# LilYau350/Variance-Aware-Weight

Hardware: AMD Instinct MI355X
Metric: training images/sec (higher is better)
Workload: dtype bf16; 1 GPU; DiT-B/4, 4x32x32 latents, 1000 classes; Trainer.train_step: q_sample + fwd + lambda-weighted MSE + bwd + AdamW + EMA; global batch 256 = 256 per GPU; global_batch=256, per_gpu_batch=256, parallelism=dp1, weight_type=lambda, hip_graph=False

## Files before the change

### include/vaw_hip.h

```cpp
#ifndef VAW_HIP_H
#define VAW_HIP_H
#include <stdint.h>

#ifdef __cplusplus
extern "C" {
#endif

typedef enum { VAW_OK = 0, VAW_ERR_INVALID = -1, VAW_ERR_LAUNCH = -2, VAW_ERR_UNSUPPORTED = -3 } vaw_status;
typedef enum { VAW_F32 = 0, VAW_BF16 = 1,
               VAW_FP8 = 2, VAW_BF8 = 3  } vaw_dtype;
typedef void* vaw_stream;

int vaw_version(void);
const char* vaw_last_error_string(void);


int vaw_qsample_fwd(const float* x0, const float* noise, const int64_t* t, const float* tab_a, const float* tab_s,
                    int num_timesteps, float* x_t, int B, int64_t per_sample, vaw_stream stream);

int vaw_mix_rows(const float* x, const float* y, const float* ca, const float* cb, float* out, int B,
                 int64_t per_sample, vaw_stream stream);

int vaw_wmse_fwd(const float* model_out, const float* x0, const float* noise, const float* ca, const float* cb,
                 const float* w, float* mse, int B, int64_t per_sample, vaw_stream stream);
int vaw_wmse_bwd(const float* model_out, const float* x0, const float* noise, const float* ca, const float* cb,
                 const float* w, const float* gmse, float* dout, int B, int64_t per_sample, vaw_stream stream);

int vaw_vb_fwd(const float* mean_out, const float* var_out, const float* x0, const float* x_t, const float* coef,
               int mean_mode, int var_mode, float scale, float* vb, int B, int64_t per_sample, vaw_stream stream);
int vaw_vb_bwd(const float* mean_out, const float* var_out, const float* x0, const float* x_t, const float* coef,
               int mean_mode, int var_mode, float scale, const float* gvb, float* d_mean, float* d_var, int B,
               int64_t per_sample, vaw_stream stream);

int vaw_sample_step(int kind, const float* mean_out, const float* var_out, const float* x, const float* noise,
                    const float* coef, int mean_mode, int var_mode, int clip_denoised, float eta, float* sample,
                    float* pred_xstart, float* mean, float* log_variance, int B, int64_t per_sample, vaw_stream stream);

int vaw_bpd_terms(const float* mean_out, const float* var_out, int64_t model_ld, const float* x0, const float* x_t,
                  const float* noise, const float* coef, int mean_mode, int var_mode, int clip_denoised, float* vb,
                  float* xstart_mse, float* mse, int64_t out_ld, int group, int B, int64_t per_sample, vaw_stream stream);

int vaw_prior_bpd(const float* x0, float sqrt_abar_last, float log_one_minus_abar_last, float* prior_bpd, int B,
                  int64_t per_sample, vaw_stream stream);

int vaw_ddim_reverse_step(const float* mean_out, int64_t model_ld, const float* x, const float* coef, int clip_denoised,
                          float* sample, float* pred_xstart, int B, int64_t per_sample, vaw_stream stream);

int vaw_guided_sample_step(int kind, const float* mean_cond, const float* mean_uncond, const float* var_cond,
                           const float* var_uncond, int64_t model_ld, float guidance_scale, const float* x, const float* noise,
                           const float* coef, int mean_mode, int var_mode, int clip_denoised, float eta, float* sample,
                           float* pred_xstart, float* mean, float* log_variance, int B, int64_t per_sample, vaw_stream stream);

int vaw_cfg_combine(const float* cond, const float* uncond, int64_t model_ld, float guidance_scale, float* out, int B,
                    int64_t per_sample, vaw_stream stream);

int vaw_finish_images(const void* src, int src_f64, uint8_t* dst, int B, int C, int H, int W, vaw_stream stream);


#define VAW_EDM_COLS 24
#define VAW_FLOW_COLS 16

int vaw_edm_input(const double* x, const double* noise, const double* coef, int row, int rows, double* x_hat, float* model_in,
                  float* model_in_dup, int B, int64_t per_sample, vaw_stream stream);

int vaw_edm_step(int kind, int pred_type, const float* cond, const float* uncond, int64_t model_ld, float guidance_scale,
                 const double* x_hat, double* d_cur, const double* coef, int row, int rows, double* x_out, float* model_in,
                 float* model_in_dup, int B, int64_t per_sample, vaw_stream stream);

int vaw_flow_step(int kind, int sde, int mean_type, const float* cond, const float* uncond, int64_t model_ld,
                  float guidance_scale, const float* x, const float* noise, const float* x_pred, float* f0, float* kick,
                  const float* coef, int row0, int row1, int rows, float* x_out, float* x_out_dup, int B, int64_t per_sample,
                  vaw_stream stream);


#define VAW_RESAMPLER_MAX_T 4096

int vaw_resampler_update(const int64_t* ts, const float* losses, int n, int T, int H, double* ring, int64_t* seen, int* bad,
                         vaw_stream stream);

// ... 82 lines not shown
    VAW_GV_GENERIC = 0,
    VAW_GV_T128_BK32 = 1,
    VAW_GV_T128_BK64 = 2,
    VAW_GV_RING256 = 3,
    VAW_GV_PERSISTENT = 4,
    VAW_GV_SMALL_M = 5,
    VAW_GV_PARKED_DRAIN = 6,
    VAW_GV_WARP_SPEC = 7
} vaw_gemm_variant;
typedef enum { VAW_GR_NONE = 0, VAW_GR_F32 = 1, VAW_GR_BF16 = 2, VAW_GR_F32_ROWSUM = 3 } vaw_gemm_reduce;
typedef enum { VAW_GS_NONE = 0, VAW_GS_FUSED = 1, VAW_GS_SEPARATE = 2 } vaw_gemm_rowsum_mode;
typedef enum { VAW_GC_NONE = 0, VAW_GC_FOLD = 1, VAW_GC_DEFERRED = 2, VAW_GC_SEPARATE = 3 } vaw_gemm_colsum_mode;
typedef struct {
    int variant;
    int ntw;
    int mb, nb, stages;
    int bkt;
    int epi_kind;
    int split;
    int xcd_parts;
    int grid_x, grid_y, grid_z, block;
    int64_t lds_bytes;
    int reduce;
    int rowsum_mode;
    int colsum_mode;
    int64_t colsum_rows;
    int64_t workspace_floats_used;
    int launches;
    int status;
} vaw_gemm_launch;
int vaw_gemm_plan(vaw_dtype dt, int a_kmajor, int b_kmajor, int64_t M, int64_t N, int64_t K, int64_t lda, int64_t ldb,
                  int64_t ldc, int64_t A, int64_t B, int64_t C, const vaw_epilogue* epi_host, int64_t workspace_floats,
                  const vaw_gemm_knobs* knobs, vaw_gemm_launch* out);

int64_t vaw_colsum_workspace_floats(int64_t M, int64_t N);
int vaw_colsum(vaw_dtype dt, const void* X, int64_t M, int64_t N, int64_t ldx, float* out, float beta,
               float* workspace, int64_t workspace_floats, vaw_stream stream);
int vaw_reduce_rows(const float* partial, int64_t R, int64_t N, float* out, float beta, vaw_stream stream);
typedef struct {
    const float* partial;
    float* out;
    int64_t R, N;
} vaw_reduce_job;
int64_t vaw_reduce_rows_batched_desc_bytes(int n_jobs);
int vaw_reduce_rows_batched(int n_jobs, const vaw_reduce_job* jobs, float beta, void* desc_dev, int upload, vaw_stream stream);


int vaw_ln_modulate_fwd(vaw_dtype dt, const float* x, const float* shift, const float* scale, int64_t mod_ld,
                        void* out, float* mean, float* rstd, int B, int T, int D, float eps, vaw_stream stream);
int vaw_ln_modulate_bwd(vaw_dtype dt, const void* dout, const float* x, const float* mean, const float* rstd,
                        const float* scale, int64_t mod_ld, const float* dres_in, float* dx, float* dshift,
                        float* dscale, int64_t dmod_ld, int B, int T, int D, float* workspace, int64_t workspace_floats,
                        vaw_stream stream);
int vaw_ln_modulate_fwd_fp8(const float* x, const float* shift, const float* scale, int64_t mod_ld, void* q_out, float* q_state,
                            vaw_dtype q_format, float* mean, float* rstd, int B, int T, int D, float eps, vaw_stream stream);
int vaw_gate_bwd_fp8(const float* dres, const void* y, const float* gate, int64_t mod_ld, void* dy_q, float* q_state,
                     vaw_dtype q_format, float* dgate, int64_t dmod_ld, float* dy_colsum_partial, int B, int T, int D,
                     float* workspace, int64_t workspace_floats, vaw_stream stream);
int64_t vaw_row_bwd_workspace_floats(int B, int T, int D);
typedef enum { VAW_ROW_LN_FWD = 0, VAW_ROW_LN_FWD_FP8 = 1, VAW_ROW_LN_BWD = 2, VAW_ROW_GATE_BWD = 3, VAW_ROW_GATE_BWD_FP8 = 4,
               VAW_ROW_LN_BWD_GATE = 5, VAW_ROW_LN_BWD_GATE_FP8 = 6, VAW_ROW_COLSUM = 7 } vaw_row_kind;
typedef enum {
    VAW_RV_LN_FWD = 0,
    VAW_RV_ROW_BWD = 1,
    VAW_RV_ROW_GATE = 2,
    VAW_RV_ROW_FUSE = 3,
    VAW_RV_ROW_FUSE8 = 4,
    VAW_RV_COLSUM_BF16X8 = 5, VAW_RV_COLSUM_VEC4 = 6, VAW_RV_COLSUM_SCALAR = 7
} vaw_row_variant;
typedef struct {
    int variant;
    int nv;
    int nc, rows_per_chunk;
    int grid_x, block;
    int64_t lds_bytes;
    int64_t workspace_floats;
} vaw_row_launch;
int vaw_row_plan(vaw_row_kind kind, vaw_dtype dt, int64_t B, int64_t T, int64_t D, int64_t ldx, int64_t base_addr,
                 int64_t workspace_floats, vaw_row_launch* out);
int vaw_gate_bwd(vaw_dtype dt, const float* dres, const void* y, const float* gate, int64_t mod_ld, void* dy,
                 float* dgate, int64_t dmod_ld, float* dy_colsum_partial, int B, int T, int D, float* workspace, int64_t workspace_floats, vaw_stream stream);
int vaw_ln_modulate_bwd_gate(vaw_dtype dt, const void* dout, const float* x, const float* mean, const float* rstd,
                             const float* scale, int64_t mod_ld, const float* dres_in, float* dx, float* dshift, float* dscale,
                             int64_t dmod_ld, const void* y_next, const float* gate_next, void* dy_next, float* dgate_next,
                             float* dy_colsum_partial, int B, int T, int D, float* workspace, int64_t workspace_floats, vaw_stream stream);
int vaw_ln_modulate_bwd_gate_fp8(const void* dout, const float* x, const float* mean, const float* rstd, const float* scale,
                                 int64_t mod_ld, const float* dres_in, float* dx, float* dshift, float* dscale, int64_t dmod_ld,
                                 const void* y_next, const float* gate_next, void* dy_q, float* q_state, vaw_dtype q_format,
                                 float* dgate_next, float* dy_colsum_partial, int B, int T, int D, float* workspace,
                                 int64_t workspace_floats, vaw_stream stream);

int vaw_patchify(vaw_dtype dt, const float* img, void* tok, int B, int C, int H, int W, int p, vaw_stream stream);
int vaw_patchify_bwd(const float* dtok, float* dimg, int B, int C, int H, int W, int p, vaw_stream stream);
int vaw_unpatchify(vaw_dtype dt, const float* tok, float* img, int B, int C, int H, int W, int p,
                   vaw_stream stream);
int vaw_unpatchify_bwd(vaw_dtype dt, const float* dimg, void* dtok, int B, int C, int H, int W, int p,
                       vaw_stream stream);

int vaw_timestep_embedding(vaw_dtype dt, const float* t, void* out, int B, int dim, float max_period,
                           vaw_stream stream);
int vaw_silu_fwd(vaw_dtype dt, const float* x, void* out, int64_t n, vaw_stream stream);
int vaw_silu_bwd(const float* x, const float* dy, float* dx, int64_t n, vaw_stream stream);
int vaw_add_embedding(const float* a, const float* table, const int64_t* idx, float* out, int B, int D,
                      int num_rows, vaw_stream stream);
int vaw_embedding_bwd(const float* dc, const int64_t* idx, float* dtable, int B, int D, int num_rows, float beta,
                      vaw_stream stream);

typedef struct {
    int B, H, T, hd;
    int64_t q_sb, q_sh, q_st, q_sd;
    int64_t o_sb, o_sh, o_st, o_sd;
    float scale;
} vaw_attn_desc;
int vaw_attn_fwd(vaw_dtype dt, const vaw_attn_desc* d_host, const void* q, const void* k, const void* v, void* o,
                 float* lse, vaw_stream stream);
int vaw_attn_bwd(vaw_dtype dt, const vaw_attn_desc* d_host, const void* q, const void* k, const void* v,
                 const void* o, const void* d_o, const float* lse, float* delta, void* dq, void* dk, void* dv,
                 vaw_stream stream);
int vaw_attn_bwd_colsum(vaw_dtype dt, const vaw_attn_desc* d, const void* q, const void* k, const void* v, const void* o,
                        const void* d_o, const float* lse, float* delta, void* dq, void* dk, void* dv, float* colsum_partial,
                        int64_t* rows_out, vaw_stream stream);

typedef enum { VAW_ATTN_DIR_FWD = 0, VAW_ATTN_DIR_BWD = 1, VAW_ATTN_DIR_BWD_COLSUM = 2 } vaw_attn_dir;
typedef enum {
    VAW_AV_ROWWISE = 0,
    VAW_AV_FWD_T64 = 1,
    VAW_AV_FWD_G1 = 2,
    VAW_AV_FWD_G2 = 3,
    VAW_AV_FWD_BIG = 4,
    VAW_AV_BWD_T64 = 5,
    VAW_AV_BWD_G1 = 6,
    VAW_AV_BWD_G2 = 7,
    VAW_AV_BWD_BIG_NT2 = 8,
    VAW_AV_BWD_BIG_NT4 = 9
} vaw_attn_variant;
typedef struct {
    int variant;
    int hd_image;
    int launches;
    int grid_x, grid_y, block;
    int64_t lds_bytes;
    int lds_cap_raised;
    int64_t colsum_rows;
    int status;
} vaw_attn_launch;
int vaw_attn_plan(int dir, vaw_dtype dt, const vaw_attn_desc* d, int64_t q, int64_t k, int64_t v, int64_t o_or_do, int64_t dq,
                  int64_t dk, int64_t dv, vaw_attn_launch* out);


int vaw_conv3x3_narrow(vaw_dtype dt, int mode, const void* in, const void* w, const float* bias, void* out, int B, int H,
                       int W, int Cn, int Cw, vaw_stream stream);

int64_t vaw_groupnorm_workspace_floats(int B, int HW, int C);
int vaw_groupnorm_fwd(vaw_dtype dt, const void* x, const float* gamma, const float* beta, const float* scale,
                      const float* shift, int64_t film_ld, int silu, void* y, float* mean, float* rstd, int B, int HW,
                      int C, int G, float eps, float* workspace, vaw_stream stream);
int vaw_groupnorm_apply(vaw_dtype dt, const void* x, const float* mean, const float* rstd, const float* gamma,
                        const float* beta, const float* scale, const float* shift, int64_t film_ld, int silu, void* y, int B,
                        int HW, int C, int G, vaw_stream stream);
int vaw_groupnorm_bwd(vaw_dtype dt, const void* dout, const void* x, const float* mean, const float* rstd,
                      const float* gamma, const float* beta, const float* scale, const float* shift, int64_t film_ld,
                      int silu, const void* dx_add, void* dx, float* dgamma, float* dbeta, float grad_beta, float* dscale,
                      float* dshift, int64_t dfilm_ld, int B, int HW, int C, int G, float* workspace, vaw_stream stream);
int vaw_im2col3x3(vaw_dtype dt, const void* x, void* col, int B, int H, int W, int C, vaw_stream stream);
int vaw_col2im3x3(vaw_dtype dt, const void* dcol, void* dx, int B, int H, int W, int C, vaw_stream stream);
int vaw_conv3x3(vaw_dtype dt, int mode, const void* act, const void* act2, const void* w, void* out, int B, int H, int W,
                int Ci, int Co, const vaw_epilogue* epi_host, float* workspace, int64_t workspace_floats, vaw_stream stream);
int64_t vaw_conv3x3_wgrad_small_workspace_floats(int B, int H, int W, int Ci, int Co);
int vaw_conv3x3_wgrad_small(vaw_dtype dt, const void* dy, const void* x, float* dw, float beta, int B, int H, int W, int Ci,
                            int Co, float* workspace, int64_t workspace_floats, vaw_stream stream);
int vaw_resample2(vaw_dtype dt, const void* in, void* out, int B, int Ho, int Wo, int C, int mode, float s,
                  vaw_stream stream);
int vaw_concat_channels(vaw_dtype dt, void* a, void* b, void* cat, int64_t M, int Ca, int Cb, int split,
                        vaw_stream stream);
int vaw_add_inplace(vaw_dtype dt, void* dst, const void* src, int64_t n, vaw_stream stream);
int vaw_mul(vaw_dtype dt, const void* a, const void* b, void* out, int64_t n, vaw_stream stream);
int vaw_subsample2(vaw_dtype dt, const void* in, void* out, int B, int Ho, int Wo, int C, int mode, vaw_stream stream);
int64_t vaw_dropout_bits_words(int64_t n);
int vaw_dropout_pack(vaw_dtype dt, const void* mask, void* bits, int64_t M, int C, vaw_stream stream);
int vaw_dropout_bits_fwd(vaw_dtype dt, const void* x, const void* bits, float keep_scale, void* y, int64_t n, vaw_stream stream);
int vaw_dropout_bits_bwd(vaw_dtype dt, const void* dy, const void* bits, float keep_scale, void* dx, int64_t n, vaw_stream stream);
int vaw_rowvec_add(vaw_dtype dt, void* h, const float* e, int64_t ld, int B, int HW, int C, vaw_stream stream);
int vaw_rowvec_sum(vaw_dtype dt, const void* dh, float* de, int64_t ld, int B, int HW, int C, float beta, vaw_stream stream);
int vaw_nchw_to_nhwc(vaw_dtype dt, const float* nchw, void* nhwc, int B, int C, int HW, vaw_stream stream);
int vaw_nhwc_to_nchw(vaw_dtype dt, const void* nhwc, float* nchw, int B, int C, int HW, vaw_stream stream);


int64_t vaw_sumsq_workspace_floats(void);
int vaw_sumsq(const float* g, int64_t n, float* sumsq_out, int accumulate, float* workspace, vaw_stream stream);
int vaw_adamw_ema_step(float* p, float* g, float* m, float* v, float* ema, void* shadow_bf16, int64_t n, float lr,
                       float beta1, float beta2, float eps, float weight_decay, float bc1, float bc2,
                       float ema_decay, const float* sumsq, float clip_max_norm, int zero_grad, vaw_stream stream);
int vaw_adamw_ema_step_dev(float* p, float* g, float* m, float* v, float* ema, void* shadow_bf16, int64_t n,
                           const float* hyper, float beta1, float beta2, float eps, float weight_decay, float ema_decay,
                           const float* sumsq, float clip_max_norm, int zero_grad, vaw_stream stream);
int vaw_ema_update(float* ema, const float* src, int64_t n, float decay, vaw_stream stream);
int vaw_cast_bf16(const float* src, void* dst, int64_t n, vaw_stream stream);
int vaw_uncast_bf16(const void* src, float* dst, int64_t n, float scale, vaw_stream stream);

typedef struct {
    int records;
    int colsum_sets;
    int own_dy;
    int Bk;
    int64_t block_bytes;
    int64_t block_stat_bytes;
    int64_t shared_bytes;
    int64_t colsum_bytes;
    int64_t scratch_bytes;
    int64_t cond_bytes;
    int64_t total;
} vaw_dit_ws_plan_t;
int vaw_dit_ws_plan(int dtype, int B, int T, int D, int Dm, int depth, int heads, int Kp, int No, int defer_wgrad, int checkpoint,
                    vaw_dit_ws_plan_t* out);

int vaw_comm_unique_id(void* out128);
int vaw_comm_init(const void* id128, int rank, int world);
int vaw_comm_world(void);
int vaw_comm_destroy(void);
int vaw_allreduce_bucket_start(void* buf, int64_t count, vaw_dtype dt, vaw_stream stream);
int vaw_reduce_scatter_bucket_start(void* buf, int64_t count, vaw_dtype dt, vaw_stream stream);
int vaw_allgather_bucket_start(void* buf, int64_t count, vaw_dtype dt, vaw_stream stream);
int vaw_allreduce_bucket_wait(vaw_stream stream);

#ifdef __cplusplus
}
#endif
#endif
```

### variance-aware-weight_amd/_lib.py

```python
import ctypes as C
import os

import torch

_HERE = os.path.dirname(os.path.abspath(__file__))
LIB_PATH = os.environ.get("VAW_HIP_LIB") or os.path.join(_HERE, "libvaw_hip.so")

F32, BF16, FP8, BF8 = 0, 1, 2, 3
TORCH_DTYPE = {F32: torch.float32, BF16: torch.bfloat16}

_p, _i, _l, _f = C.c_void_p, C.c_int, C.c_int64, C.c_float


class Epilogue(C.Structure):
    _fields_ = [("bias", _p), ("act", _i), ("aux_in", _p), ("aux_out", _p), ("gate", _p), ("gate_ld", _l),
                ("resid", _p), ("rowadd", _p), ("rows_per_batch", _i), ("alpha", _f), ("beta", _f), ("out_f32", _i),
                ("colsum_out", _p), ("colsum_beta", _f), ("resid_is_act", _i), ("rowsum_a_out", _p), ("rowsum_a_beta", _f),
                ("colsum_partial_out", _p), ("colsum_rows_out", C.POINTER(C.c_int64))]


class AttnDesc(C.Structure):
    _fields_ = [("B", _i), ("H", _i), ("T", _i), ("hd", _i), ("q_sb", _l), ("q_sh", _l), ("q_st", _l), ("q_sd", _l),
                ("o_sb", _l), ("o_sh", _l), ("o_st", _l), ("o_sd", _l), ("scale", _f)]


class RowLaunch(C.Structure):
    _fields_ = [("variant", _i), ("nv", _i), ("nc", _i), ("rows_per_chunk", _i), ("grid_x", _i), ("block", _i), ("lds_bytes", _l),
                ("workspace_floats", _l)]


class AttnLaunch(C.Structure):
    _fields_ = [("variant", _i), ("hd_image", _i), ("launches", _i), ("grid_x", _i), ("grid_y", _i), ("block", _i), ("lds_bytes", _l),
                ("lds_cap_raised", _i), ("colsum_rows", _l), ("status", _i)]


class GemmKnobs(C.Structure):
    _fields_ = [(n, _i) for n in ("tile", "force_generic", "bk", "pd", "ws", "xcdsplit", "sm_max_m", "sm_wide_m", "sm_nb", "sm_stages",
                                  "ws_loaders", "epi", "debug", "p8_nt", "nt_aux", "cus")]


class GemmLaunch(C.Structure):
    _fields_ = [("variant", _i), ("ntw", _i), ("mb", _i), ("nb", _i), ("stages", _i), ("bkt", _i), ("epi_kind", _i), ("split", _i),
                ("xcd_parts", _i), ("grid_x", _i), ("grid_y", _i), ("grid_z", _i), ("block", _i), ("lds_bytes", _l), ("reduce", _i),
                ("rowsum_mode", _i), ("colsum_mode", _i), ("colsum_rows", _l), ("workspace_floats_used", _l), ("launches", _i),
                ("status", _i)]


class DitWsPlan(C.Structure):
    _fields_ = [("records", _i), ("colsum_sets", _i), ("own_dy", _i), ("Bk", _i), ("block_bytes", _l), ("block_stat_bytes", _l),
                ("shared_bytes", _l), ("colsum_bytes", _l), ("scratch_bytes", _l), ("cond_bytes", _l), ("total", _l)]


ATTN_FWD, ATTN_BWD, ATTN_BWD_COLSUM = range(3)
(AV_ROWWISE, AV_FWD_T64, AV_FWD_G1, AV_FWD_G2, AV_FWD_BIG, AV_BWD_T64, AV_BWD_G1, AV_BWD_G2, AV_BWD_BIG_NT2,
 AV_BWD_BIG_NT4) = range(10)
AV_NAMES = ("rowwise", "fwd_t64", "fwd_g1", "fwd_g2", "fwd_big", "bwd_t64", "bwd_g1", "bwd_g2", "bwd_big_nt2", "bwd_big_nt4")

GV_GENERIC, GV_T128_BK32, GV_T128_BK64, GV_RING256, GV_PERSISTENT, GV_SMALL_M, GV_PARKED_DRAIN, GV_WARP_SPEC = range(8)
GV_NAMES = ("generic", "t128_bk32", "t128_bk64", "ring256", "persistent", "small_m", "parked_drain", "warp_spec")
GR_NONE, GR_F32, GR_BF16, GR_F32_ROWSUM = range(4)
GS_NONE, GS_FUSED, GS_SEPARATE = range(3)
GC_NONE, GC_FOLD, GC_DEFERRED, GC_SEPARATE = range(4)
P8_STORE, P8_GELU, P8_DGELU, P8_GATE, P8_SLAB, P8_ANY, P8_WGRAD, P8_RESID = range(8)

RESAMPLER_MAX_T = 4096

ROW_LN_FWD, ROW_LN_FWD_FP8, ROW_LN_BWD, ROW_GATE_BWD, ROW_GATE_BWD_FP8, ROW_LN_BWD_GATE, ROW_LN_BWD_GATE_FP8, ROW_COLSUM = range(8)
RV_LN_FWD, RV_ROW_BWD, RV_ROW_GATE, RV_ROW_FUSE, RV_ROW_FUSE8, RV_COLSUM_BF16X8, RV_COLSUM_VEC4, RV_COLSUM_SCALAR = range(8)

_PROTOS = {
    "vaw_qsample_fwd": [_p, _p, _p, _p, _p, _i, _p, _i, _l, _p],
    "vaw_mix_rows": [_p, _p, _p, _p, _p, _i, _l, _p],
    "vaw_wmse_fwd": [_p, _p, _p, _p, _p, _p, _p, _i, _l, _p],
    "vaw_wmse_bwd": [_p, _p, _p, _p, _p, _p, _p, _p, _i, _l, _p],
    "vaw_gemm": [_i, _i, _i, _l, _l, _l, _p, _l, _p, _l, _p, _l, C.POINTER(Epilogue), _p, _l, _p],
    "vaw_gemm_uses_bf16_mfma": [_i, _l, _l, _l, _p, _l, _p, _l],
    "vaw_colsum": [_i, _p, _l, _l, _l, _p, _f, _p, _l, _p],
    "vaw_ln_modulate_fwd": [_i, _p, _p, _p, _l, _p, _p, _p, _i, _i, _i, _f, _p],
    "vaw_ln_modulate_bwd": [_i, _p, _p, _p, _p, _p, _l, _p, _p, _p, _p, _l, _i, _i, _i, _p, _l, _p],
    "vaw_gate_bwd": [_i, _p, _p, _p, _l, _p, _p, _l, _p, _i, _i, _i, _p, _l, _p],
    "vaw_reduce_rows": [_p, _l, _l, _p, _f, _p],
    "vaw_reduce_rows_batched": [_i, _p, _f, _p, _i, _p],
    "vaw_ln_modulate_bwd_gate": [_i, _p, _p, _p, _p, _p, _l, _p, _p, _p, _p, _l, _p, _p, _p, _p, _p, _i, _i, _i, _p, _l, _p],
    "vaw_ln_modulate_bwd_gate_fp8": [_p, _p, _p, _p, _p, _l, _p, _p, _p, _p, _l, _p, _p, _p, _p, _i, _p, _p, _i, _i, _i, _p, _l, _p],
    "vaw_patchify": [_i, _p, _p, _i, _i, _i, _i, _i, _p],
    "vaw_patchify_bwd": [_p, _p, _i, _i, _i, _i, _i, _p],
    "vaw_unpatchify": [_i, _p, _p, _i, _i, _i, _i, _i, _p],
    "vaw_unpatchify_bwd": [_i, _p, _p, _i, _i, _i, _i, _i, _p],
    "vaw_timestep_embedding": [_i, _p, _p, _i, _i, _f, _p],
    "vaw_silu_fwd": [_i, _p, _p, _l, _p],
    "vaw_silu_bwd": [_p, _p, _p, _l, _p],
    "vaw_add_embedding": [_p, _p, _p, _p, _i, _i, _i, _p],
    "vaw_embedding_bwd": [_p, _p, _p, _i, _i, _i, _f, _p],
    "vaw_attn_fwd": [_i, C.POINTER(AttnDesc), _p, _p, _p, _p, _p, _p],
    "vaw_attn_bwd": [_i, C.POINTER(AttnDesc), _p, _p, _p, _p, _p, _p, _p, _p, _p, _p, _p],
    "vaw_attn_bwd_colsum": [_i, C.POINTER(AttnDesc), _p, _p, _p, _p, _p, _p, _p, _p, _p, _p, _p, C.POINTER(C.c_int64), _p],
    "vaw_comm_unique_id": [_p],
    "vaw_comm_init": [_p, _i, _i],
    "vaw_comm_world": [],
    "vaw_comm_destroy": [],
    "vaw_allreduce_bucket_start": [_p, _l, _i, _p],
    "vaw_reduce_scatter_bucket_start": [_p, _l, _i, _p],
    "vaw_allgather_bucket_start": [_p, _l, _i, _p],
# ... 1 lines not shown
    "vaw_groupnorm_fwd": [_i, _p, _p, _p, _p, _p, _l, _i, _p, _p, _p, _i, _i, _i, _i, _f, _p, _p],
    "vaw_groupnorm_apply": [_i, _p, _p, _p, _p, _p, _p, _p, _l, _i, _p, _i, _i, _i, _i, _p],
    "vaw_groupnorm_bwd": [_i, _p, _p, _p, _p, _p, _p, _p, _p, _l, _i, _p, _p, _p, _p, _f, _p, _p, _l, _i, _i, _i, _i, _p, _p],
    "vaw_im2col3x3": [_i, _p, _p, _i, _i, _i, _i, _p],
    "vaw_col2im3x3": [_i, _p, _p, _i, _i, _i, _i, _p],
    "vaw_conv3x3": [_i, _i, _p, _p, _p, _p, _i, _i, _i, _i, _i, C.POINTER(Epilogue), _p, _l, _p],
    "vaw_vb_fwd": [_p, _p, _p, _p, _p, _i, _i, _f, _p, _i, _l, _p],
    "vaw_vb_bwd": [_p, _p, _p, _p, _p, _i, _i, _f, _p, _p, _p, _i, _l, _p],
    "vaw_sample_step": [_i, _p, _p, _p, _p, _p, _i, _i, _i, _f, _p, _p, _p, _p, _i, _l, _p],
    "vaw_bpd_terms": [_p, _p, _l, _p, _p, _p, _p, _i, _i, _i, _p, _p, _p, _l, _i, _i, _l, _p],
    "vaw_guided_sample_step": [_i, _p, _p, _p, _p, _l, _f, _p, _p, _p, _i, _i, _i, _f, _p, _p, _p, _p, _i, _l, _p],
    "vaw_cfg_combine": [_p, _p, _l, _f, _p, _i, _l, _p],
    "vaw_finish_images": [_p, _i, _p, _i, _i, _i, _i, _p],
    "vaw_edm_input": [_p, _p, _p, _i, _i, _p, _p, _p, _i, _l, _p],
    "vaw_edm_step": [_i, _i, _p, _p, _l, _f, _p, _p, _p, _i, _i, _p, _p, _p, _i, _l, _p],
    "vaw_flow_step": [_i, _i, _i, _p, _p, _l, _f, _p, _p, _p, _p, _p, _p, _i, _i, _i, _p, _p, _i, _l, _p],
    "vaw_prior_bpd": [_p, _f, _f, _p, _i, _l, _p],
    "vaw_ddim_reverse_step": [_p, _l, _p, _p, _i, _p, _p, _i, _l, _p],
    "vaw_resampler_update": [_p, _p, _i, _i, _i, _p, _p, _p, _p],
    "vaw_resampler_draw": [_p, _p, _i, _i, C.c_double, _p, _i, _p, _p, _p, _p],
    "vaw_conv3x3_narrow": [_i, _i, _p, _p, _p, _p, _i, _i, _i, _i, _i, _p],
    "vaw_conv3x3_wgrad_small": [_i, _p, _p, _p, _f, _i, _i, _i, _i, _i, _p, _l, _p],
    "vaw_resample2": [_i, _p, _p, _i, _i, _i, _i, _i, _f, _p],
    "vaw_concat_channels": [_i, _p, _p, _p, _l, _i, _i, _i, _p],
    "vaw_add_inplace": [_i, _p, _p, _l, _p],
    "vaw_mul": [_i, _p, _p, _p, _l, _p],
    "vaw_subsample2": [_i, _p, _p, _i, _i, _i, _i, _i, _p],
    "vaw_dropout_pack": [_i, _p, _p, _l, _i, _p],
    "vaw_dropout_bits_fwd": [_i, _p, _p, _f, _p, _l, _p],
    "vaw_dropout_bits_bwd": [_i, _p, _p, _f, _p, _l, _p],
    "vaw_rowvec_add": [_i, _p, _p, _l, _i, _i, _i, _p],
    "vaw_rowvec_sum": [_i, _p, _p, _l, _i, _i, _i, _f, _p],
    "vaw_nchw_to_nhwc": [_i, _p, _p, _i, _i, _i, _p],
    "vaw_nhwc_to_nchw": [_i, _p, _p, _i, _i, _i, _p],
    "vaw_sumsq": [_p, _l, _p, _i, _p, _p],
    "vaw_adamw_ema_step_dev": [_p, _p, _p, _p, _p, _p, _l, _p, _f, _f, _f, _f, _f, _p, _f, _i, _p],
    "vaw_adamw_ema_step": [_p, _p, _p, _p, _p, _p, _l, _f, _f, _f, _f, _f, _f, _f, _f, _p, _f, _i, _p],
    "vaw_ema_update": [_p, _p, _l, _f, _p],
    "vaw_cast_bf16": [_p, _p, _l, _p],
    "vaw_uncast_bf16": [_p, _p, _l, _f, _p],
    "vaw_wgrad_grouped": [_i, _i, _p, _l, _f, _p, _i, _p, _l, _p],
    "vaw_fp8_quantize": [_i, _i, _p, _l, _l, _l, _p, _l, _p, _l, _p, _p, _l, _p],
    "vaw_fp8_quantize_delayed": [_i, _i, _p, _l, _l, _l, _p, _l, _p, _l, _p, _p],
    "vaw_fp8_scale_update": [_p, _l, _p],
    "vaw_fp8_quantize_delayed_batched": [_i, _p, _p, _i, _p],
    "vaw_gemm_fp8": [_i, _l, _l, _l, _p, _l, _p, _p, _l, _p, _p, _l, C.POINTER(Epilogue), _p, _i, _p, _l, _p],
    "vaw_fp8_transpose": [_p, _l, _l, _l, _p, _l, _p],
    "vaw_ln_modulate_fwd_fp8": [_p, _p, _p, _l, _p, _p, _i, _p, _p, _i, _i, _i, _f, _p],
    "vaw_gate_bwd_fp8": [_p, _p, _p, _l, _p, _p, _i, _p, _l, _p, _i, _i, _i, _p, _l, _p],
    "vaw_row_plan": [_i, _i, _l, _l, _l, _l, _l, _l, C.POINTER(RowLaunch)],
    "vaw_attn_plan": [_i, _i, C.POINTER(AttnDesc), _l, _l, _l, _l, _l, _l, _l, C.POINTER(AttnLaunch)],
    "vaw_gemm_plan": [_i, _i, _i, _l, _l, _l, _l, _l, _l, _l, _l, _l, C.POINTER(Epilogue), _l, C.POINTER(GemmKnobs), C.POINTER(GemmLaunch)],
    "vaw_dit_ws_plan": [_i, _i, _i, _i, _i, _i, _i, _i, _i, _i, _i, C.POINTER(DitWsPlan)],
}

_lib = None


class VawError(RuntimeError):
    pass


def lib():
    global _lib
    if _lib is None:
        if not os.path.exists(LIB_PATH):
            raise VawError(f"{LIB_PATH} not found: build it with `python -c 'import __graft_entry__ as g; g.build()'` "
                           "(there is no CPU fallback for the HIP path)")
        L = C.CDLL(LIB_PATH)
        for name, args in _PROTOS.items():
            if not hasattr(L, name) and os.environ.get("VAW_HIP_LIB"):
                continue
            fn = getattr(L, name)
            fn.argtypes = args
            fn.restype = _i
        L.vaw_version.restype = _i
        L.vaw_last_error_string.restype = C.c_char_p
        L.vaw_colsum_workspace_floats.argtypes = [_l, _l]
        L.vaw_colsum_workspace_floats.restype = _l
        L.vaw_row_bwd_workspace_floats.argtypes = [_i, _i, _i]
        L.vaw_row_bwd_workspace_floats.restype = _l
        L.vaw_conv3x3_wgrad_small_workspace_floats.argtypes = [_i, _i, _i, _i, _i]
        L.vaw_conv3x3_wgrad_small_workspace_floats.restype = _l
        L.vaw_groupnorm_workspace_floats.argtypes = [_i, _i, _i]
        L.vaw_groupnorm_workspace_floats.restype = _l
        if hasattr(L, "vaw_dropout_bits_words"):
            L.vaw_dropout_bits_words.argtypes = [_l]
            L.vaw_dropout_bits_words.restype = _l
        L.vaw_wgrad_grouped_desc_bytes.argtypes = [_i]
        L.vaw_wgrad_grouped_desc_bytes.restype = _l
        L.vaw_reduce_rows_batched_desc_bytes.argtypes = [_i]
        L.vaw_reduce_rows_batched_desc_bytes.restype = _l
        L.vaw_fp8_quantize_batched_desc_bytes.argtypes = [_i]
        L.vaw_fp8_quantize_batched_desc_bytes.restype = _l
        L.vaw_fp8_quantize_workspace_floats.argtypes = []
        L.vaw_fp8_quantize_workspace_floats.restype = _l
        L.vaw_sumsq_workspace_floats.argtypes = []
        L.vaw_sumsq_workspace_floats.restype = _l
        L.vaw_debug_force_rowwise_attention.argtypes = [_i]
        L.vaw_debug_force_rowwise_attention.restype = None
        L.vaw_debug_force_generic_gemm.argtypes = [_i]
        L.vaw_debug_force_generic_gemm.restype = None
        L.vaw_debug_gemm_tile.argtypes = [_i]
        L.vaw_debug_gemm_tile.restype = None
        if hasattr(L, "vaw_gemm_default_knobs"):
            L.vaw_gemm_default_knobs.argtypes = [C.POINTER(GemmKnobs)]
            L.vaw_gemm_default_knobs.restype = None
        for dbg in ("vaw_debug_gn_coop", "vaw_debug_gn_flat"):
            if hasattr(L, dbg):
                getattr(L, dbg).argtypes = [_i]
                getattr(L, dbg).restype = None
        L.vaw_p8_set_reserved_cus.argtypes = [_i]
        L.vaw_p8_set_reserved_cus.restype = None
        L.vaw_debug_cu_hog.argtypes = [_i, _i, _p]
        L.vaw_debug_cu_hog.restype = _i
        _lib = L
    return _lib


def exported_symbols():
    return sorted(list(_PROTOS) + ["vaw_version", "vaw_last_error_string", "vaw_colsum_workspace_floats",
                                   "vaw_sumsq_workspace_floats", "vaw_groupnorm_workspace_floats", "vaw_wgrad_grouped_desc_bytes",
                                   "vaw_conv3x3_wgrad_small_workspace_floats", "vaw_row_bwd_workspace_floats",
                                   "vaw_fp8_quantize_workspace_floats", "vaw_p8_set_reserved_cus", "vaw_reduce_rows_batched_desc_bytes", "vaw_fp8_quantize_batched_desc_bytes",
                                   "vaw_gemm_default_knobs", "vaw_dropout_bits_words"])


def check(rc, what):
    if rc != 0:
        raise VawError(f"{what} failed ({rc}): {lib().vaw_last_error_string().decode()}")


def stream_ptr():
    return torch.cuda.current_stream().cuda_stream


def ptr(t):
    return 0 if t is None else t.data_ptr()


def need_cuda(*tensors):
    for t in tensors:
        if t is not None and not t.is_cuda:
            raise VawError("vaw_amd runs on the GPU only: got a CPU tensor (no CPU fallback exists by design)")
```

### variance-aware-weight_amd/csrc/elementwise.hip

```cpp
#include "common.h"

static inline int stream_grid(int64_t work_items, int block) {
    int64_t g = (work_items + block - 1) / block;
    const int64_t cap = 256 * 8;
    return (int)(g < 1 ? 1 : (g > cap ? cap : g));
}

template <bool GATHER>
__global__ void mix_rows_kernel(const float* __restrict__ x, const float* __restrict__ y, const float* __restrict__ ca,
                                const float* __restrict__ cb, const int64_t* __restrict__ t, int T,
                                float* __restrict__ out, int64_t n) {
    const int b = blockIdx.y;
    float a, c;
    if (GATHER) {
        const int64_t tt = t[b];
        const bool ok = tt >= 0 && tt < T;
        a = ok ? ca[tt] : __builtin_nanf("");
        c = ok ? cb[tt] : __builtin_nanf("");
    } else {
        a = ca[b];
        c = cb[b];
    }
    const float* xr = x + (int64_t)b * n;
    const float* yr = y + (int64_t)b * n;
    float* orow = out + (int64_t)b * n;
    const int64_t n4 = ((n & 3) == 0) ? n / 4 : 0;
    for (int64_t i = blockIdx.x * (int64_t)blockDim.x + threadIdx.x; i < n4; i += (int64_t)gridDim.x * blockDim.x) {
        f32x4 xv = load4(xr + 4 * i), yv = load4(yr + 4 * i);
        store4(orow + 4 * i, a * xv + c * yv);
    }
    for (int64_t i = n4 * 4 + blockIdx.x * (int64_t)blockDim.x + threadIdx.x; i < n; i += (int64_t)gridDim.x * blockDim.x)
        orow[i] = a * xr[i] + c * yr[i];
}

extern "C" int vaw_qsample_fwd(const float* x0, const float* noise, const int64_t* t, const float* tab_a,
                               const float* tab_s, int num_timesteps, float* x_t, int B, int64_t per_sample,
                               vaw_stream stream) {
    VAW_CHECK_ARG(B > 0 && per_sample > 0 && num_timesteps > 0, "qsample: bad sizes B=%d n=%ld", B, (long)per_sample);
    int gx = stream_grid(per_sample / 4 + 1, 256);
    dim3 grid(gx > 64 ? 64 : gx, B);
    mix_rows_kernel<true><<<grid, 256, 0, (hipStream_t)stream>>>(x0, noise, tab_a, tab_s, t, num_timesteps, x_t, per_sample);
    VAW_CHECK_LAUNCH("qsample");
    return VAW_OK;
}

extern "C" int vaw_mix_rows(const float* x, const float* y, const float* ca, const float* cb, float* out, int B,
                            int64_t per_sample, vaw_stream stream) {
    VAW_CHECK_ARG(B > 0 && per_sample > 0, "mix_rows: bad sizes");
    int gx = stream_grid(per_sample / 4 + 1, 256);
    dim3 grid(gx > 64 ? 64 : gx, B);
    mix_rows_kernel<false><<<grid, 256, 0, (hipStream_t)stream>>>(x, y, ca, cb, nullptr, 0, out, per_sample);
    VAW_CHECK_LAUNCH("mix_rows");
    return VAW_OK;
}

__global__ void wmse_fwd_kernel(const float* __restrict__ o, const float* __restrict__ x0, const float* __restrict__ nz,
                                const float* __restrict__ ca, const float* __restrict__ cb, const float* __restrict__ w,
                                float* __restrict__ mse, int64_t n) {
    __shared__ float scratch[16];
    const int b = blockIdx.x;
    const float a = ca[b], c = cb[b];
    const float* orow = o + (int64_t)b * n;
    const float* xr = x0 + (int64_t)b * n;
    const float* nr = nz + (int64_t)b * n;
    float acc = 0.f;
    const int64_t n4 = ((n & 3) == 0) ? n / 4 : 0;
    for (int64_t i = threadIdx.x; i < n4; i += blockDim.x) {
        f32x4 d = a * load4(xr + 4 * i) + c * load4(nr + 4 * i) - load4(orow + 4 * i);
        acc += d[0] * d[0] + d[1] * d[1] + d[2] * d[2] + d[3] * d[3];
    }
    for (int64_t i = n4 * 4 + threadIdx.x; i < n; i += blockDim.x) {
        float d = a * xr[i] + c * nr[i] - orow[i];
        acc += d * d;
    }
    float tot = block_sum(acc, scratch);
    if (threadIdx.x == 0) mse[b] = w[b] * (tot / (float)n);
}

__global__ void wmse_bwd_kernel(const float* __restrict__ o, const float* __restrict__ x0, const float* __restrict__ nz,
                                const float* __restrict__ ca, const float* __restrict__ cb, const float* __restrict__ w,
                                const float* __restrict__ gmse, float* __restrict__ dout, int64_t n) {
    const int b = blockIdx.y;
    const float a = ca[b], c = cb[b];
    const float k = gmse[b] * w[b] * 2.f / (float)n;
    const float* orow = o + (int64_t)b * n;
    const float* xr = x0 + (int64_t)b * n;
    const float* nr = nz + (int64_t)b * n;
    float* dr = dout + (int64_t)b * n;
    const int64_t n4 = ((n & 3) == 0) ? n / 4 : 0;
    for (int64_t i = blockIdx.x * (int64_t)blockDim.x + threadIdx.x; i < n4; i += (int64_t)gridDim.x * blockDim.x)
        store4(dr + 4 * i, k * (load4(orow + 4 * i) - a * load4(xr + 4 * i) - c * load4(nr + 4 * i)));
    for (int64_t i = n4 * 4 + blockIdx.x * (int64_t)blockDim.x + threadIdx.x; i < n; i += (int64_t)gridDim.x * blockDim.x)
        dr[i] = k * (orow[i] - a * xr[i] - c * nr[i]);
}

extern "C" int vaw_wmse_fwd(const float* model_out, const float* x0, const float* noise, const float* ca,
                            const float* cb, const float* w, float* mse, int B, int64_t per_sample,
                            vaw_stream stream) {
    VAW_CHECK_ARG(B > 0 && per_sample > 0, "wmse_fwd: bad sizes");
    wmse_fwd_kernel<<<B, 1024, 0, (hipStream_t)stream>>>(model_out, x0, noise, ca, cb, w, mse, per_sample);
    VAW_CHECK_LAUNCH("wmse_fwd");
    return VAW_OK;
}

extern "C" int vaw_wmse_bwd(const float* model_out, const float* x0, const float* noise, const float* ca,
                            const float* cb, const float* w, const float* gmse, float* dout, int B,
                            int64_t per_sample, vaw_stream stream) {
    VAW_CHECK_ARG(B > 0 && per_sample > 0, "wmse_bwd: bad sizes");
    int gx = stream_grid(per_sample / 4 + 1, 256);
    dim3 grid(gx > 64 ? 64 : gx, B);
    wmse_bwd_kernel<<<grid, 256, 0, (hipStream_t)stream>>>(model_out, x0, noise, ca, cb, w, gmse, dout, per_sample);
    VAW_CHECK_LAUNCH("wmse_bwd");
    return VAW_OK;
}

#define VB_NCOEF 8
struct VbElem {
    float val;
    float d_lv;
    float d_mean;
};
__device__ __forceinline__ float vb_cdf(float z, float& dcdf) {
    const float k = 0.7978845608028654f;
    const float th = tanhf(k * (z + 0.044715f * (z * z * z)));
    dcdf = 0.5f * (1.f - th * th) * k * (1.f + 3.f * 0.044715f * z * z);
    return 0.5f * (1.f + th);
}
__device__ __forceinline__ VbElem vb_elem(float x0, float true_mean, float true_lv, float mean, float lv, bool t0) {
    VbElem r;
    if (!t0) {
        const float e2 = expf(-lv), d = true_mean - mean, ratio = expf(true_lv - lv);
        r.val = 0.5f * (-1.0f + lv - true_lv + ratio + (d * d) * e2);
        r.d_lv = 0.5f * (1.f - ratio - (d * d) * e2);
        r.d_mean = -d * e2;
        return r;
    }
    const float cx = x0 - mean, inv = expf(-(0.5f * lv));
    const float pin = inv * (cx + 1.0f / 255.0f), mnn = inv * (cx - 1.0f / 255.0f);
    float dp, dm;
    const float cp = vb_cdf(pin, dp), cm = vb_cdf(mnn, dm);
    float lp, g_pin = 0.f, g_min = 0.f;
    if (x0 < -0.999f) {
        lp = logf(fmaxf(cp, 1e-12f));
        if (cp >= 1e-12f) g_pin = dp / cp;
    } else if (x0 > 0.999f) {
        const float q = 1.f - cm;
        lp = logf(fmaxf(q, 1e-12f));
        if (q >= 1e-12f) g_min = -dm / q;
    } else {
        const float dl = cp - cm;
        lp = logf(fmaxf(dl, 1e-12f));
        if (dl >= 1e-12f) { g_pin = dp / dl; g_min = -dm / dl; }
    }
    r.val = -lp;
    r.d_lv = 0.5f * (g_pin * pin + g_min * mnn);
    r.d_mean = inv * (g_pin + g_min);
    return r;
}
__device__ __forceinline__ void vb_model(const float* c, int mean_mode, int var_mode, float xt, float m, float v, float& mean,
                                         float& lv) {
    mean = mean_mode == 1 ? m : c[0] * (c[4] * xt + c[5] * m) + c[1] * xt;
    if (var_mode == 1) lv = v;
    else if (var_mode == 2) { const float frac = (v + 1.f) / 2.f; lv = frac * c[3] + (1.f - frac) * c[2]; }
    else lv = c[3];
// ... 511 lines not shown

extern "C" int vaw_finish_images(const void* src, int src_f64, uint8_t* dst, int B, int C, int H, int W, vaw_stream stream) {
    VAW_CHECK_ARG(B > 0 && C > 0 && H > 0 && W > 0, "finish_images: bad sizes B=%d C=%d H=%d W=%d", B, C, H, W);
    VAW_CHECK_ARG(src && dst, "finish_images: null pointer");
    VAW_CHECK_ARG(src_f64 == 0 || src_f64 == 1, "finish_images: src_f64 must be 0 (f32) or 1 (f64), got %d", src_f64);
    VAW_CHECK_ARG(((uintptr_t)src & (src_f64 ? 7 : 3)) == 0, "finish_images: source not aligned to its element size");
    const int64_t HW = (int64_t)H * W;
    if (src_f64) finish_images_launch(static_cast<const double*>(src), dst, B, C, HW, (hipStream_t)stream);
    else finish_images_launch(static_cast<const float*>(src), dst, B, C, HW, (hipStream_t)stream);
    VAW_CHECK_LAUNCH("finish_images");
    return VAW_OK;
}

template <typename T>
__global__ void timestep_embedding_kernel(const float* __restrict__ t, T* __restrict__ out, int B, int dim,
                                          float neg_log_period) {
    const int half = dim / 2;
    for (int64_t idx = blockIdx.x * (int64_t)blockDim.x + threadIdx.x; idx < (int64_t)B * dim;
         idx += (int64_t)gridDim.x * blockDim.x) {
        const int b = (int)(idx / dim), j = (int)(idx % dim);
        float v = 0.f;
        if (j < 2 * half) {
            const int i = j < half ? j : j - half;
            const float f = expf(neg_log_period * (float)i / (float)half);
            const float ang = t[b] * f;
            v = j < half ? cosf(ang) : sinf(ang);
        }
        out[idx] = from_f32<T>(v);
    }
}

extern "C" int vaw_timestep_embedding(vaw_dtype dt, const float* t, void* out, int B, int dim, float max_period,
                                      vaw_stream stream) {
    VAW_CHECK_ARG(B > 0 && dim > 0, "timestep_embedding: bad sizes");
    const float nl = -logf(max_period);
    int grid = stream_grid((int64_t)B * dim, 256);
    if (dt == VAW_F32)
        timestep_embedding_kernel<float><<<grid, 256, 0, (hipStream_t)stream>>>(t, (float*)out, B, dim, nl);
    else
        timestep_embedding_kernel<bf16_t><<<grid, 256, 0, (hipStream_t)stream>>>(t, (bf16_t*)out, B, dim, nl);
    VAW_CHECK_LAUNCH("timestep_embedding");
    return VAW_OK;
}

template <typename T>
__global__ void silu_fwd_kernel(const float* __restrict__ x, T* __restrict__ out, int64_t n) {
    for (int64_t i = blockIdx.x * (int64_t)blockDim.x + threadIdx.x; i < n; i += (int64_t)gridDim.x * blockDim.x)
        out[i] = from_f32<T>(silu_f(x[i]));
}
__global__ void silu_bwd_kernel(const float* __restrict__ x, const float* __restrict__ dy, float* __restrict__ dx, int64_t n) {
    for (int64_t i = blockIdx.x * (int64_t)blockDim.x + threadIdx.x; i < n; i += (int64_t)gridDim.x * blockDim.x)
        dx[i] = dy[i] * silu_grad_f(x[i]);
}
extern "C" int vaw_silu_fwd(vaw_dtype dt, const float* x, void* out, int64_t n, vaw_stream stream) {
    VAW_CHECK_ARG(n > 0, "silu_fwd: n<=0");
    int grid = stream_grid(n, 256);
    if (dt == VAW_F32) silu_fwd_kernel<float><<<grid, 256, 0, (hipStream_t)stream>>>(x, (float*)out, n);
    else silu_fwd_kernel<bf16_t><<<grid, 256, 0, (hipStream_t)stream>>>(x, (bf16_t*)out, n);
    VAW_CHECK_LAUNCH("silu_fwd");
    return VAW_OK;
}
extern "C" int vaw_silu_bwd(const float* x, const float* dy, float* dx, int64_t n, vaw_stream stream) {
    VAW_CHECK_ARG(n > 0, "silu_bwd: n<=0");
    silu_bwd_kernel<<<stream_grid(n, 256), 256, 0, (hipStream_t)stream>>>(x, dy, dx, n);
    VAW_CHECK_LAUNCH("silu_bwd");
    return VAW_OK;
}

__global__ void add_embedding_kernel(const float* __restrict__ a, const float* __restrict__ table,
                                     const int64_t* __restrict__ idx, float* __restrict__ out, int B, int D, int rows) {
    for (int64_t i = blockIdx.x * (int64_t)blockDim.x + threadIdx.x; i < (int64_t)B * D; i += (int64_t)gridDim.x * blockDim.x) {
        const int b = (int)(i / D), d = (int)(i % D);
        const int64_t r = idx[b];
        out[i] = a[i] + ((r >= 0 && r < rows) ? table[r * D + d] : __builtin_nanf(""));
    }
}
__global__ void __launch_bounds__(256)
embedding_bwd_kernel(const float* __restrict__ dc, const int64_t* __restrict__ idx, float* __restrict__ dtable, int B, int D,
                     int rows, float beta) {
    __shared__ int s_idx[1024];
    const int r = blockIdx.x;
    constexpr int MAXC = 8;
    for (int d0 = 0; d0 < D; d0 += 256 * MAXC) {
        float acc[MAXC];
#pragma unroll
        for (int j = 0; j < MAXC; ++j) acc[j] = 0.f;
        for (int b0 = 0; b0 < B; b0 += 1024) {
            const int nb = B - b0 < 1024 ? B - b0 : 1024;
            __syncthreads();
            for (int i = threadIdx.x; i < nb; i += 256) s_idx[i] = (int)idx[b0 + i];
            __syncthreads();
            for (int i = 0; i < nb; ++i) {
                if (s_idx[i] != r) continue;
                const float* src = dc + (int64_t)(b0 + i) * D + d0;
#pragma unroll
                for (int j = 0; j < MAXC; ++j) {
                    const int d = threadIdx.x + 256 * j;
                    if (d0 + d < D) acc[j] += src[d];
                }
            }
        }
#pragma unroll
        for (int j = 0; j < MAXC; ++j) {
            const int d = d0 + threadIdx.x + 256 * j;
            if (d < D) {
                float* o = dtable + (int64_t)r * D + d;
                *o = (beta != 0.f ? beta * *o : 0.f) + acc[j];
            }
        }
    }
}
extern "C" int vaw_add_embedding(const float* a, const float* table, const int64_t* idx, float* out, int B, int D,
                                 int num_rows, vaw_stream stream) {
    VAW_CHECK_ARG(B > 0 && D > 0 && num_rows > 0, "add_embedding: bad sizes");
    add_embedding_kernel<<<stream_grid((int64_t)B * D, 256), 256, 0, (hipStream_t)stream>>>(a, table, idx, out, B, D, num_rows);
    VAW_CHECK_LAUNCH("add_embedding");
    return VAW_OK;
}
extern "C" int vaw_embedding_bwd(const float* dc, const int64_t* idx, float* dtable, int B, int D, int num_rows,
                                 float beta, vaw_stream stream) {
    VAW_CHECK_ARG(B > 0 && D > 0 && num_rows > 0, "embedding_bwd: bad sizes");
    embedding_bwd_kernel<<<num_rows, 256, 0, (hipStream_t)stream>>>(dc, idx, dtable, B, D, num_rows, beta);
    VAW_CHECK_LAUNCH("embedding_bwd");
    return VAW_OK;
}

template <typename T, bool CONV_ORDER, bool TO_TOKENS>
__global__ void patch_shuffle_kernel(const float* __restrict__ img_in, float* __restrict__ img_out,
                                     const float* __restrict__ tok_in_f32, T* __restrict__ tok_out, int B, int C, int H,
                                     int W, int p) {
    const int hp = H / p, wp = W / p;
    const int64_t total = (int64_t)B * C * H * W;
    const int K = C * p * p;
    for (int64_t e = blockIdx.x * (int64_t)blockDim.x + threadIdx.x; e < total; e += (int64_t)gridDim.x * blockDim.x) {
        int x = (int)(e % W);
        int64_t r = e / W;
        int y = (int)(r % H);
        r /= H;
        int c = (int)(r % C);
        int b = (int)(r / C);
        const int ty = y / p, i = y % p, tx = x / p, j = x % p;
        const int64_t row = ((int64_t)b * hp + ty) * wp + tx;
        const int col = CONV_ORDER ? (c * p + i) * p + j : (i * p + j) * C + c;
        if (TO_TOKENS) tok_out[row * K + col] = from_f32<T>(img_in[e]);
        else img_out[e] = tok_in_f32[row * K + col];
    }
}

extern "C" int vaw_patchify(vaw_dtype dt, const float* img, void* tok, int B, int C, int H, int W, int p,
                            vaw_stream stream) {
    VAW_CHECK_ARG(B > 0 && C > 0 && p > 0 && H % p == 0 && W % p == 0, "patchify: bad sizes");
    int grid = stream_grid((int64_t)B * C * H * W, 256);
    if (dt == VAW_F32)
        patch_shuffle_kernel<float, true, true><<<grid, 256, 0, (hipStream_t)stream>>>(img, nullptr, nullptr, (float*)tok, B, C, H, W, p);
    else
        patch_shuffle_kernel<bf16_t, true, true><<<grid, 256, 0, (hipStream_t)stream>>>(img, nullptr, nullptr, (bf16_t*)tok, B, C, H, W, p);
    VAW_CHECK_LAUNCH("patchify");
    return VAW_OK;
}
extern "C" int vaw_patchify_bwd(const float* dtok, float* dimg, int B, int C, int H, int W, int p, vaw_stream stream) {
    VAW_CHECK_ARG(B > 0 && C > 0 && p > 0 && H % p == 0 && W % p == 0, "patchify_bwd: bad sizes");
    int grid = stream_grid((int64_t)B * C * H * W, 256);
    patch_shuffle_kernel<float, true, false><<<grid, 256, 0, (hipStream_t)stream>>>(nullptr, dimg, dtok, nullptr, B, C, H, W, p);
    VAW_CHECK_LAUNCH("patchify_bwd");
// ... 165 lines not shown
                                      vaw_stream stream) {
    VAW_CHECK_ARG(n > 0 && hyper, "adamw_dev: n<=0 or no hyper buffer");
    VAW_CHECK_ARG((((uintptr_t)p | (uintptr_t)g | (uintptr_t)m | (uintptr_t)v | (uintptr_t)ema) & 15) == 0 &&
                      ((uintptr_t)shadow_bf16 & 7) == 0, "adamw_dev: buffers must be 16-byte aligned");
    VAW_CHECK_ARG(clip_max_norm <= 0.f || sumsq != nullptr, "adamw_dev: clip needs sumsq");
    AdamArgs a{0.f, beta1, beta2, eps, weight_decay, 1.f, 1.f, ema_decay, clip_max_norm, zero_grad};
    adamw_ema_kernel<<<adam_grid(n), 256, 0, (hipStream_t)stream>>>(p, g, m, v, ema, (bf16_t*)shadow_bf16, n, sumsq, a, hyper);
    VAW_CHECK_LAUNCH("adamw_ema_dev");
    return VAW_OK;
}

__global__ void ema_kernel(float* __restrict__ ema, const float* __restrict__ src, int64_t n, float d) {
    for (int64_t i = blockIdx.x * (int64_t)blockDim.x + threadIdx.x; i < n; i += (int64_t)gridDim.x * blockDim.x)
        ema[i] = ema[i] * d + src[i] * (1.f - d);
}
extern "C" int vaw_ema_update(float* ema, const float* src, int64_t n, float decay, vaw_stream stream) {
    VAW_CHECK_ARG(n > 0, "ema: n<=0");
    ema_kernel<<<stream_grid(n, 256), 256, 0, (hipStream_t)stream>>>(ema, src, n, decay);
    VAW_CHECK_LAUNCH("ema");
    return VAW_OK;
}

__global__ void cast_bf16_kernel(const float* __restrict__ src, bf16_t* __restrict__ dst, int64_t n) {
    const int64_t n4 = n / 4;
    for (int64_t i = blockIdx.x * (int64_t)blockDim.x + threadIdx.x; i < n4; i += (int64_t)gridDim.x * blockDim.x)
        store4(dst + 4 * i, load4(src + 4 * i));
    for (int64_t i = n4 * 4 + blockIdx.x * (int64_t)blockDim.x + threadIdx.x; i < n; i += (int64_t)gridDim.x * blockDim.x)
        dst[i] = (bf16_t)src[i];
}
extern "C" int vaw_cast_bf16(const float* src, void* dst, int64_t n, vaw_stream stream) {
    VAW_CHECK_ARG(n > 0 && ((uintptr_t)src & 15) == 0 && ((uintptr_t)dst & 7) == 0, "cast_bf16: n<=0 or unaligned");
    cast_bf16_kernel<<<stream_grid(n / 4 + 1, 256), 256, 0, (hipStream_t)stream>>>(src, (bf16_t*)dst, n);
    VAW_CHECK_LAUNCH("cast_bf16");
    return VAW_OK;
}

__global__ void uncast_bf16_kernel(const bf16_t* __restrict__ src, float* __restrict__ dst, int64_t n, float scale) {
    const int64_t n8 = n / 8;
    for (int64_t i = blockIdx.x * (int64_t)blockDim.x + threadIdx.x; i < n8; i += (int64_t)gridDim.x * blockDim.x) {
        const bf16x8 v = reinterpret_cast<const bf16x8*>(src)[i];
        f32x4 a = {(float)v[0], (float)v[1], (float)v[2], (float)v[3]}, b = {(float)v[4], (float)v[5], (float)v[6], (float)v[7]};
        reinterpret_cast<f32x4*>(dst)[2 * i] = a * scale;
        reinterpret_cast<f32x4*>(dst)[2 * i + 1] = b * scale;
    }
    for (int64_t i = n8 * 8 + blockIdx.x * (int64_t)blockDim.x + threadIdx.x; i < n; i += (int64_t)gridDim.x * blockDim.x)
        dst[i] = scale * (float)src[i];
}
extern "C" int vaw_uncast_bf16(const void* src, float* dst, int64_t n, float scale, vaw_stream stream) {
    VAW_CHECK_ARG(n > 0 && ((uintptr_t)src & 15) == 0 && ((uintptr_t)dst & 15) == 0, "uncast_bf16: n<=0 or unaligned");
    uncast_bf16_kernel<<<stream_grid(n / 8 + 1, 256), 256, 0, (hipStream_t)stream>>>((const bf16_t*)src, dst, n, scale);
    VAW_CHECK_LAUNCH("uncast_bf16");
    return VAW_OK;
}
```

### variance-aware-weight_amd/csrc/gemm.hip

```cpp
#include "common.h"
#include <type_traits>

#include "gemm_plan.h"

#define BM 128
#define BN 128
#define BK 64
#define CS_LD 132
#define CS_BYTES (64 * CS_LD * 4)
#define CP_BYTES (4 * 128 * 4)

template <int BKT> struct FastCfg {
    static constexpr int tile_bytes = 128 * BKT * 2;
    static constexpr int stage_bytes = 2 * tile_bytes;
    static constexpr int main_bytes = 2 * stage_bytes;
    static constexpr int lds_bytes = (main_bytes > CS_BYTES ? main_bytes : CS_BYTES) + CP_BYTES;
};

typedef __attribute__((address_space(3))) void* lds_ptr_t;
typedef const __attribute__((address_space(1))) void* gbl_ptr_t;

template <int BKT>
__device__ __forceinline__ int kmaj_swz(int row) { return BKT == 64 ? ((row >> 1) & 7) : ((-(row >> 2)) & 3); }
template <int BKT>
// ... 443 lines not shown
            for (int i = 0; i < 4; ++i)
#pragma unroll
                for (int j = 0; j < 4; ++j)
#pragma unroll
                    for (int r = 0; r < 4; ++r)
                        cs[(16 * i + 4 * (lane >> 4) + r) * BIG_CS_LD + 64 * wx + 16 * j + (lane & 15)] =
                            acc[4 * (quarter & 1) + i][j][r];
        }
        __syncthreads();
#pragma unroll
        for (int pass = 0; pass < 4; ++pass) {
            const int row = pass * 16 + r0;
            if (!col_ok || 64 * quarter + row >= mvalid) continue;
            const float* src = cs + row * BIG_CS_LD + c8;
            const int64_t m = m0 + 64 * quarter + row;
            if (n_split > 1) {
                float* dst = e.slab + (int64_t)blockIdx.y * e.M * e.N + m * e.N + n0 + c8;
                store4(dst, load4(src));
                store4(dst + 4, load4(src + 4));
            } else {
                f32x4 v0 = load4(src), v1 = load4(src + 4);
                epi_row8(e, (unsigned)m, n0 + c8, v0, v1, b0, b1);
                s0 += v0;
                s1 += v1;
            }
        }
    }
    if (e.colpart && n_split == 1) {
#pragma unroll
        for (int j = 0; j < 4; ++j) {
            s0[j] += __shfl_xor(s0[j], 32, 64);
            s1[j] += __shfl_xor(s1[j], 32, 64);
        }
        float* cp = reinterpret_cast<float*>(smem + BIG_NSTAGE * BIG_STAGE);
        if (lane < 32) {
            store4(cp + wid * 256 + c8, s0);
            store4(cp + wid * 256 + c8 + 4, s1);
        }
        __syncthreads();
        if ((int)threadIdx.x < nvalid && threadIdx.x < 256) {
            float t = 0.f;
#pragma unroll
            for (int w8 = 0; w8 < 8; ++w8) t += cp[w8 * 256 + threadIdx.x];
            e.colpart[(int64_t)tm * e.N + n0 + threadIdx.x] = t;
        }
    }
}

template <typename TO>
__global__ void splitk_reduce_kernel(const float* __restrict__ slab, int S, int64_t M, int64_t N, int64_t ldc,
                                     void* __restrict__ C, float alpha, float beta, int out_f32,
                                     const float* __restrict__ rowpart = nullptr, float* __restrict__ rowsum_out = nullptr,
                                     float rowsum_beta = 0.f) {
    if (rowpart && blockIdx.x == gridDim.x - 1) {
        for (int64_t m = threadIdx.x; m < M; m += blockDim.x) {
            float t = 0.f;
            for (int sidx = 0; sidx < S; ++sidx) t += rowpart[(int64_t)sidx * M + m];
            rowsum_out[m] = (rowsum_beta != 0.f ? rowsum_beta * rowsum_out[m] : 0.f) + t;
        }
    }
    const int64_t total4 = M * N / 4;
    for (int64_t i = blockIdx.x * (int64_t)blockDim.x + threadIdx.x; i < total4; i += (int64_t)gridDim.x * blockDim.x) {
        const int64_t m = (4 * i) / N, n = (4 * i) % N;
        f32x4 acc = {0, 0, 0, 0};
        int sidx = 0;
        for (; sidx + 8 <= S; sidx += 8) {
            f32x4 v[8];
#pragma unroll
            for (int u = 0; u < 8; ++u) v[u] = load4(slab + (int64_t)(sidx + u) * M * N + 4 * i);
#pragma unroll
            for (int u = 0; u < 8; ++u) acc += v[u];
        }
        for (; sidx < S; ++sidx) acc += load4(slab + (int64_t)sidx * M * N + 4 * i);
        acc *= alpha;
        const int64_t off = m * ldc + n;
        if (out_f32) {
            float* c = (float*)C + off;
            if (beta != 0.f) acc += beta * load4(c);
            store4(c, acc);
        } else {
            store4((TO*)C + off, acc);
        }
    }
}

#define GBM 128
#define GBN 128
#define GBK 16
#define GLD 144

template <typename T, bool KMAJOR>
__device__ __forceinline__ void generic_stage(const T* __restrict__ g, int64_t ld, int64_t r0, int64_t rows, int64_t k0,
                                              int64_t K, float* tile, int tid) {
#pragma unroll
    for (int i = 0; i < (GBM * GBK) / 256; ++i) {
        const int e = tid + 256 * i;
        int r, k;
        if (KMAJOR) { r = e / GBK; k = e % GBK; } else { k = e / GBM; r = e % GBM; }
        const int64_t gr = r0 + r, gk = k0 + k;
        float v = 0.f;
        if (gr < rows && gk < K) v = to_f32(KMAJOR ? g[gr * ld + gk] : g[gk * ld + gr]);
        tile[k * GLD + r] = v;
    }
}

template <typename T, bool AK, bool BKM>
__global__ void __launch_bounds__(256)
gemm_generic_kernel(const T* __restrict__ A, int64_t lda, const T* __restrict__ B, int64_t ldb, int64_t K, int64_t kchunk,
                    EpiDev e) {
    __shared__ float As[GBK * GLD];
// ... 261 lines not shown
```

### variance-aware-weight_amd/csrc/layernorm.hip

```cpp
#include <stdio.h>
#include <stdlib.h>

#include "common.h"

template <typename T, int NV>
__global__ void __launch_bounds__(256)
ln_modulate_fwd_kernel(const float* __restrict__ x, const float* __restrict__ shift, const float* __restrict__ scale,
                       int64_t mod_ld, T* __restrict__ out, float* __restrict__ mean_out, float* __restrict__ rstd_out,
                       int64_t M, int Tt, int D, float eps, unsigned char* __restrict__ q_out = nullptr,
                       float* __restrict__ q_state = nullptr, int q_e5m2 = 0) {
    const int lane = threadIdx.x & 63;
    const float q_inv = q_out ? 1.f / q_state[0] : 1.f;
    float am = 0.f;
    const int wave = __builtin_amdgcn_readfirstlane(threadIdx.x >> 6);
    const int64_t row0 = (int64_t)blockIdx.x * 4 + wave, rstep = (int64_t)gridDim.x * 4;
    unsigned colc[NV];
#pragma unroll
    for (int i = 0; i < NV; ++i) {
        const unsigned c = (unsigned)(i * 64 + lane) * 4u;
        colc[i] = c < (unsigned)D ? c : 0u;
    }
    f32x4 nx[NV];
    if (row0 < M) {
#pragma unroll
// ... 19 lines not shown
        for (int i = 0; i < NV; ++i) {
            const int c = (i * 64 + lane) * 4;
            if (c < D) {
                f32x4 d = v[i] - mean;
                q += d[0] * d[0] + d[1] * d[1] + d[2] * d[2] + d[3] * d[3];
            }
        }
        const float rstd = rsqrtf(wave_sum(q) / (float)D + eps);
        if (lane == 0) {
            mean_out[row] = mean;
            rstd_out[row] = rstd;
        }
        const float* sh = shift + (int64_t)b * mod_ld;
        const float* sc = scale + (int64_t)b * mod_ld;
        if (q_out) {
#pragma unroll
            for (int i = 0; i < NV; ++i) {
                const int c = (i * 64 + lane) * 4;
                if (c < D) {
                    f32x4 xh = (v[i] - mean) * rstd;
                    *reinterpret_cast<unsigned*>(q_out + row * D + c) = fp8_word_of_bf16(xh * (1.f + load4(sc + c)) + load4(sh + c), q_inv, q_e5m2, am);
                }
            }
            continue;
        }
        T* orow = out + row * D;
#pragma unroll
        for (int i = 0; i < NV; ++i) {
            const int c = (i * 64 + lane) * 4;
            if (c < D) {
                f32x4 xh = (v[i] - mean) * rstd;
                store4(orow + c, xh * (1.f + load4(sc + c)) + load4(sh + c));
            }
        }
    }
    if (q_out) {
        __shared__ float wmax[4];
        am = wave_max(am);
        if (lane == 0) wmax[threadIdx.x >> 6] = am;
        __syncthreads();
        if (threadIdx.x < 64) fp8_amax_commit(fmaxf(fmaxf(wmax[0], wmax[1]), fmaxf(wmax[2], wmax[3])), q_state + 1, lane);
    }
}

template <typename T, int NV, bool GATE_ONLY, bool QOUT = false, bool FUSE = false>
__global__ void __launch_bounds__((FUSE && NV > 3) ? 512 : 1024)
row_bwd_kernel(const T* __restrict__ dout, const float* __restrict__ x, const float* __restrict__ mean,
               const float* __restrict__ rstd, const float* __restrict__ scale, int64_t mod_ld,
               const float* __restrict__ dres_in, float* __restrict__ dx, float* __restrict__ dshift,
               float* __restrict__ dscale, int64_t dmod_ld, int Tt, int D,
               const float* __restrict__ dres, const T* __restrict__ y, const float* __restrict__ gate,
               T* __restrict__ dy, float* __restrict__ dgate, float* __restrict__ dy_colpart,
               int rows_per_chunk, float* __restrict__ part,
               unsigned char* __restrict__ q_out = nullptr, float* __restrict__ q_state = nullptr, int q_e5m2 = 0) {
    static_assert(!(FUSE && GATE_ONLY), "FUSE extends the LayerNorm mode");
    constexpr int NQ = FUSE ? 4 : 2;
    extern __shared__ __attribute__((aligned(16))) float lds[];
    const float q_inv = ((GATE_ONLY || FUSE) && QOUT) ? 1.f / q_state[0] : 1.f;
    float q_am = 0.f;
    const int lane = threadIdx.x & 63, wid = threadIdx.x >> 6, nw = blockDim.x >> 6;
    const int b = blockIdx.x;
    const int t_begin = blockIdx.y * rows_per_chunk;
    const int t_end = t_begin + rows_per_chunk < Tt ? t_begin + rows_per_chunk : Tt;
    f32x4 acc0[NV], acc1[NV], sc[NV];
    f32x4 acc2[FUSE ? NV : 1], acc3[FUSE ? NV : 1];
    float* const sc_lds = lds + NQ * D;
    float* const gsc_lds = sc_lds + D;
#pragma unroll
    for (int i = 0; i < NV; ++i) {
        acc0[i] = f32x4{0, 0, 0, 0};
        acc1[i] = f32x4{0, 0, 0, 0};
        const int c = (i * 64 + lane) * 4;
        const float* src = GATE_ONLY ? gate : scale;
        sc[i] = c < D ? load4(src + (int64_t)b * mod_ld + c) : f32x4{0, 0, 0, 0};
        if (FUSE) {
            acc2[i] = acc3[i] = f32x4{0, 0, 0, 0};
            if (wid == 0 && c < D) {
                store4(sc_lds + c, 1.f + sc[i]);
                store4(gsc_lds + c, load4(gate + (int64_t)b * mod_ld + c));
            }
        }
    }
    if (FUSE) __syncthreads();
    for (int t = t_begin + wid; t < t_end; t += nw) {
        const int64_t row = (int64_t)b * Tt + t;
        if (GATE_ONLY) {
#pragma unroll
            for (int i = 0; i < NV; ++i) {
                const int c = (i * 64 + lane) * 4;
                if (c < D) {
                    f32x4 g = load4(dres + row * D + c);
                    f32x4 yv = load4(y + row * D + c);
                    f32x4 d = g * sc[i];
                    if (QOUT) *reinterpret_cast<unsigned*>(q_out + row * D + c) = fp8_word_of_bf16(d, q_inv, q_e5m2, q_am);
                    else store4(dy + row * D + c, d);
                    acc0[i] += g * yv;
                    f32x4 dr = {to_f32(from_f32<T>(d[0])), to_f32(from_f32<T>(d[1])), to_f32(from_f32<T>(d[2])), to_f32(from_f32<T>(d[3]))};
                    acc1[i] += dr;
                }
            }
        } else {
            const float mu = mean[row], rs = rstd[row];
            f32x4 g[NV], xh[NV];
            float s1 = 0.f, s2 = 0.f;
#pragma unroll
            for (int i = 0; i < NV; ++i) {
                const int c = (i * 64 + lane) * 4;
                if (c < D) {
                    f32x4 d = load4(dout + row * D + c);
                    xh[i] = (load4(x + row * D + c) - mu) * rs;
                    acc0[i] += d;
                    acc1[i] += d * xh[i];
                    g[i] = d * (FUSE ? load4(sc_lds + c) : 1.f + sc[i]);
                    s1 += g[i][0] + g[i][1] + g[i][2] + g[i][3];
                    f32x4 gx = g[i] * xh[i];
                    s2 += gx[0] + gx[1] + gx[2] + gx[3];
                } else {
                    g[i] = xh[i] = f32x4{0, 0, 0, 0};
                }
            }
            const float c1 = wave_sum(s1) / (float)D, c2 = wave_sum(s2) / (float)D;
#pragma unroll
            for (int i = 0; i < NV; ++i) {
                const int c = (i * 64 + lane) * 4;
                if (c < D) {
                    f32x4 r = (g[i] - c1 - xh[i] * c2) * rs;
                    if (dres_in) r += load4(dres_in + row * D + c);
                    store4(dx + row * D + c, r);
                    if (FUSE) {
                        const f32x4 yv = load4(y + row * D + c);
                        const f32x4 d = r * load4(gsc_lds + c);
                        if (QOUT) *reinterpret_cast<unsigned*>(q_out + row * D + c) = fp8_word_of_bf16(d, q_inv, q_e5m2, q_am);
                        else store4(dy + row * D + c, d);
                        acc2[i] += r * yv;
                        f32x4 dr = {to_f32(from_f32<T>(d[0])), to_f32(from_f32<T>(d[1])), to_f32(from_f32<T>(d[2])), to_f32(from_f32<T>(d[3]))};
                        acc3[i] += dr;
                    }
                }
            }
        }
    }
    if ((GATE_ONLY || FUSE) && QOUT) fp8_amax_commit(q_am, q_state + 1, lane);
    float* s0 = lds;
    float* s1p = lds + D;
    for (int i = threadIdx.x; i < NQ * D; i += blockDim.x) lds[i] = 0.f;
    __syncthreads();
    for (int w = 0; w < nw; ++w) {
        if (wid == w) {
#pragma unroll
            for (int i = 0; i < NV; ++i) {
                const int c = (i * 64 + lane) * 4;
                if (c < D) {
                    store4(s0 + c, load4(s0 + c) + acc0[i]);
                    store4(s1p + c, load4(s1p + c) + acc1[i]);
                    if (FUSE) {
                        store4(lds + 2 * D + c, load4(lds + 2 * D + c) + acc2[i]);
                        store4(lds + 3 * D + c, load4(lds + 3 * D + c) + acc3[i]);
                    }
                }
            }
        }
        __syncthreads();
    }
    if (part) {
        float* dst = part + ((int64_t)blockIdx.y * gridDim.x + b) * NQ * D;
        for (int c = threadIdx.x; c < NQ * D; c += blockDim.x) dst[c] = lds[c];
        return;
    }
    for (int c = threadIdx.x; c < D; c += blockDim.x) {
        if (GATE_ONLY) {
            dgate[(int64_t)b * dmod_ld + c] = s0[c];
            if (dy_colpart) dy_colpart[(int64_t)b * D + c] = s1p[c];
        } else {
            dshift[(int64_t)b * dmod_ld + c] = s0[c];
            dscale[(int64_t)b * dmod_ld + c] = s1p[c];
            if (FUSE) {
                dgate[(int64_t)b * dmod_ld + c] = lds[2 * D + c];
                if (dy_colpart) dy_colpart[(int64_t)b * D + c] = lds[3 * D + c];
            }
        }
    }
// ... 249 lines not shown
        case 6: { constexpr int NV = 6; CALL; } break;              \
        default: { constexpr int NV = 8; CALL; } break;             \
    }

#define ROW_PLAN(kind, dt, B, T, D, ldx, base, wsf)                                      \
    vaw_row_launch plan;                                                               \
    {                                                                                  \
        const int rc_ = vaw_row_plan(kind, dt, B, T, D, ldx, base, wsf, &plan);        \
        if (rc_ != VAW_OK) return rc_;                                                 \
    }

extern "C" int vaw_ln_modulate_fwd(vaw_dtype dt, const float* x, const float* shift, const float* scale, int64_t mod_ld,
                                   void* out, float* mean, float* rstd, int B, int T, int D, float eps,
                                   vaw_stream stream) {
    VAW_CHECK_ARG(B > 0 && T > 0 && D > 0 && D % 4 == 0 && D <= 2048 && mod_ld % 4 == 0,
                  "ln_modulate_fwd: need D%%4==0, D<=2048, mod_ld%%4==0 (D=%d)", D);
    ROW_PLAN(VAW_ROW_LN_FWD, dt, B, T, D, 0, 0, 0);
    const int64_t M = (int64_t)B * T;
    static int per_cu[2][9] = {};
    const int nvk = plan.nv, ti = dt == VAW_F32 ? 0 : 1;
    if (!per_cu[ti][nvk]) {
        int nb = 0;
        if (dt == VAW_F32) { DISPATCH_NV(nvk, (void)hipOccupancyMaxActiveBlocksPerMultiprocessor(&nb, ln_modulate_fwd_kernel<float, NV>, 256, 0)); }
        else { DISPATCH_NV(nvk, (void)hipOccupancyMaxActiveBlocksPerMultiprocessor(&nb, ln_modulate_fwd_kernel<bf16_t, NV>, 256, 0)); }
        per_cu[ti][nvk] = nb > 0 && nb <= 8 ? nb : 8;
    }
    const int64_t cap = 256LL * per_cu[ti][nvk];
    const int grid = (int)(plan.grid_x < cap ? plan.grid_x : cap);
    hipStream_t s = (hipStream_t)stream;
    if (dt == VAW_F32) {
        DISPATCH_NV(nvk, (ln_modulate_fwd_kernel<float, NV><<<grid, plan.block, 0, s>>>(x, shift, scale, mod_ld, (float*)out, mean, rstd, M, T, D, eps)));
    } else {
        DISPATCH_NV(nvk, (ln_modulate_fwd_kernel<bf16_t, NV><<<grid, plan.block, 0, s>>>(x, shift, scale, mod_ld, (bf16_t*)out, mean, rstd, M, T, D, eps)));
    }
    VAW_CHECK_LAUNCH("ln_modulate_fwd");
    return VAW_OK;
}

extern "C" int vaw_ln_modulate_fwd_fp8(const float* x, const float* shift, const float* scale, int64_t mod_ld, void* q_out,
                                       float* q_state, vaw_dtype q_format, float* mean, float* rstd, int B, int T, int D, float eps,
                                       vaw_stream stream) {
    VAW_CHECK_ARG(B > 0 && T > 0 && D > 0 && D % 4 == 0 && D <= 2048 && mod_ld % 4 == 0 && q_out && q_state,
                  "ln_modulate_fwd_fp8: need D%%4==0, D<=2048, mod_ld%%4==0 (D=%d)", D);
    VAW_CHECK_ARG(q_format == VAW_FP8 || q_format == VAW_BF8, "ln_modulate_fwd_fp8: q_format");
    ROW_PLAN(VAW_ROW_LN_FWD_FP8, VAW_BF16, B, T, D, 0, 0, 0);
    const int64_t M = (int64_t)B * T;
    hipStream_t s = (hipStream_t)stream;
    DISPATCH_NV(plan.nv, (ln_modulate_fwd_kernel<bf16_t, NV><<<plan.grid_x, plan.block, 0, s>>>(x, shift, scale, mod_ld, nullptr, mean, rstd, M, T, D, eps,
                                                                                             (unsigned char*)q_out, q_state, q_format == VAW_BF8)));
    VAW_CHECK_LAUNCH("ln_modulate_fwd_fp8");
    return VAW_OK;
}

extern "C" int vaw_ln_modulate_bwd(vaw_dtype dt, const void* dout, const float* x, const float* mean, const float* rstd,
                                   const float* scale, int64_t mod_ld, const float* dres_in, float* dx, float* dshift,
                                   float* dscale, int64_t dmod_ld, int B, int T, int D, float* workspace,
                                   int64_t workspace_floats, vaw_stream stream) {
    VAW_CHECK_ARG(B > 0 && T > 0 && D > 0 && D % 4 == 0 && D <= 2048 && mod_ld % 4 == 0,
                  "ln_modulate_bwd: need D%%4==0, D<=2048, mod_ld%%4==0 (D=%d)", D);
    ROW_PLAN(VAW_ROW_LN_BWD, dt, B, T, D, 0, 0, workspace ? workspace_floats : 0);
    hipStream_t s = (hipStream_t)stream;
    const int nc = plan.nc, rpc = plan.rows_per_chunk, block = plan.block;
    float* part = nc > 1 ? workspace : nullptr;
    const size_t lds = plan.lds_bytes;
    dim3 grid(B, nc);
    if (dt == VAW_F32) {
        DISPATCH_NV(plan.nv, (row_bwd_kernel<float, NV, false><<<grid, block, lds, s>>>((const float*)dout, x, mean, rstd, scale, mod_ld, dres_in, dx, dshift, dscale, dmod_ld, T, D, nullptr, nullptr, nullptr, nullptr, nullptr, nullptr, rpc, part)));
    } else {
        DISPATCH_NV(plan.nv, (row_bwd_kernel<bf16_t, NV, false><<<grid, block, lds, s>>>((const bf16_t*)dout, x, mean, rstd, scale, mod_ld, dres_in, dx, dshift, dscale, dmod_ld, T, D, nullptr, nullptr, nullptr, nullptr, nullptr, nullptr, rpc, part)));
    }
    if (nc > 1) row_bwd_finish_kernel<<<ceil_div((int64_t)B * D, 256), 256, 0, s>>>(part, nc, B, D, dshift, dmod_ld, dscale, dmod_ld);
    VAW_CHECK_LAUNCH("ln_modulate_bwd");
    return VAW_OK;
}

extern "C" int vaw_ln_modulate_bwd_gate(vaw_dtype dt, const void* dout, const float* x, const float* mean, const float* rstd,
                                        const float* scale, int64_t mod_ld, const float* dres_in, float* dx, float* dshift,
                                        float* dscale, int64_t dmod_ld, const void* y_next, const float* gate_next, void* dy_next,
                                        float* dgate_next, float* dy_colsum_partial, int B, int T, int D, float* workspace,
                                        int64_t workspace_floats, vaw_stream stream) {
    VAW_CHECK_ARG(B > 0 && T > 0 && D > 0 && D % 4 == 0 && D <= 2048 && mod_ld % 4 == 0,
                  "ln_modulate_bwd_gate: need D%%4==0, D<=2048, mod_ld%%4==0 (D=%d)", D);
    VAW_CHECK_ARG(y_next && gate_next && dy_next && dgate_next, "ln_modulate_bwd_gate: the gate operands are required");
    ROW_PLAN(VAW_ROW_LN_BWD_GATE, dt, B, T, D, 0, 0, workspace ? workspace_floats : 0);
    hipStream_t s = (hipStream_t)stream;
    const int nc = plan.nc, rpc = plan.rows_per_chunk, block = plan.block;
    float* part = nc > 1 ? workspace : nullptr;
    const size_t lds = plan.lds_bytes;
    dim3 grid(B, nc);
    if (plan.variant == VAW_RV_ROW_FUSE8) {
#define LAUNCH_FUSE8(NVv)                                                                                                              \
    row_bwd_fuse8_kernel<NVv, false><<<grid, block, row_fuse8_lds<NVv, false>(D, block), s>>>(                                          \
        (const bf16_t*)dout, x, mean, rstd, scale, mod_ld, dres_in, dx, dshift, dscale, dmod_ld, T, D, (const bf16_t*)y_next, gate_next, \
        (bf16_t*)dy_next, dgate_next, dy_colsum_partial, rpc, part, nullptr, nullptr, 0)
        const int nv = plan.nv;
        if (nv == 1) LAUNCH_FUSE8(1); else if (nv == 2) LAUNCH_FUSE8(2); else if (nv == 3) LAUNCH_FUSE8(3); else if (nv == 4) LAUNCH_FUSE8(4); else LAUNCH_FUSE8(5);
    } else if (dt == VAW_F32) {
        DISPATCH_NV(plan.nv, (row_bwd_kernel<float, NV, false, false, true><<<grid, block, lds, s>>>((const float*)dout, x, mean, rstd, scale, mod_ld, dres_in, dx, dshift, dscale, dmod_ld, T, D, nullptr, (const float*)y_next, gate_next, (float*)dy_next, dgate_next, dy_colsum_partial, rpc, part)));
    } else {
        DISPATCH_NV(plan.nv, (row_bwd_kernel<bf16_t, NV, false, false, true><<<grid, block, lds, s>>>((const bf16_t*)dout, x, mean, rstd, scale, mod_ld, dres_in, dx, dshift, dscale, dmod_ld, T, D, nullptr, (const bf16_t*)y_next, gate_next, (bf16_t*)dy_next, dgate_next, dy_colsum_partial, rpc, part)));
    }
    if (nc > 1)
        row_bwd_finish_kernel<<<ceil_div((int64_t)B * D, 256), 256, 0, s>>>(part, nc, B, D, dshift, dmod_ld, dscale, dmod_ld, 4, dgate_next, dmod_ld,
                                                                             dy_colsum_partial, D);
    VAW_CHECK_LAUNCH("ln_modulate_bwd_gate");
    return VAW_OK;
}

extern "C" int vaw_ln_modulate_bwd_gate_fp8(const void* dout, const float* x, const float* mean, const float* rstd, const float* scale,
                                            int64_t mod_ld, const float* dres_in, float* dx, float* dshift, float* dscale, int64_t dmod_ld,
                                            const void* y_next, const float* gate_next, void* dy_q, float* q_state, vaw_dtype q_format,
                                            float* dgate_next, float* dy_colsum_partial, int B, int T, int D, float* workspace,
                                            int64_t workspace_floats, vaw_stream stream) {
    VAW_CHECK_ARG(B > 0 && T > 0 && D > 0 && D % 4 == 0 && D <= 2048 && mod_ld % 4 == 0,
                  "ln_modulate_bwd_gate_fp8: need D%%4==0, D<=2048, mod_ld%%4==0 (D=%d)", D);
    VAW_CHECK_ARG(y_next && gate_next && dy_q && q_state && dgate_next, "ln_modulate_bwd_gate_fp8: the gate operands are required");
    VAW_CHECK_ARG(q_format == VAW_FP8 || q_format == VAW_BF8, "ln_modulate_bwd_gate_fp8: q_format");
    ROW_PLAN(VAW_ROW_LN_BWD_GATE_FP8, VAW_BF16, B, T, D, 0, 0, workspace ? workspace_floats : 0);
    hipStream_t s = (hipStream_t)stream;
    const int nc = plan.nc, rpc = plan.rows_per_chunk, block = plan.block;
    float* part = nc > 1 ? workspace : nullptr;
    const size_t lds = plan.lds_bytes;
    dim3 grid(B, nc);
    if (plan.variant == VAW_RV_ROW_FUSE8) {
#define LAUNCH_FUSE8Q(NVv)                                                                                                             \
    row_bwd_fuse8_kernel<NVv, true><<<grid, block, row_fuse8_lds<NVv, true>(D, block), s>>>(                                            \
// ... 221 lines not shown
```

### variance-aware-weight_amd/dit.py

```python
import os

import numpy as np
import torch
import torch.nn as nn

from . import _lib as L
from . import ops
from ._lib import BF16, F32, ptr
from .flat import FlatModule

__all__ = ["DiT", "DiT_S", "DiT_B", "DiT_L", "DiT_XL", "DiT_models"]


def _sincos_1d(dim, pos):
    omega = 1.0 / 10000 ** (np.arange(dim // 2, dtype=np.float64) / (dim / 2.0))
    ang = np.einsum("m,d->md", pos.reshape(-1), omega)
    return np.concatenate([np.sin(ang), np.cos(ang)], axis=1)


def get_2d_sincos_pos_embed(dim, grid_size):
    gh = np.arange(grid_size, dtype=np.float32)
    gw = np.arange(grid_size, dtype=np.float32)
    grid = np.stack(np.meshgrid(gw, gh), axis=0).reshape([2, 1, grid_size, grid_size])
    return np.concatenate([_sincos_1d(dim // 2, grid[0]), _sincos_1d(dim // 2, grid[1])], axis=1)
# ... 115 lines not shown
            fmts = [L.FP8] * 4 + [gf] * 4
            self.fp8_states = ops.fp8_states(fmts * Lyr, dev, m.fp8_margin)
            self.calib_fwd = self.calib_bwd = False
            self.d_fwd = self.d_bwd = False
            for l, b in enumerate(self.blk):
                F = lambda i, cols: ops.Fp8(M, cols, dev, transposed=True, plain=False, fmt=fmts[i], state=self.fp8_states[8 * l + i])
                b.update(f_xm=F(0, D), f_ao=F(1, D), f_xm2=F(2, D), f_a=F(3, m.Dm), f_dy2=F(4, D), f_dhid=F(5, m.Dm), f_dy1=F(6, D),
                         f_dqkv=F(7, 3 * D))
        elif plan.own_dy:
            for b in self.blk[:plan.records]:
                b.update(dy2=e(M, D), dDm=e(M, m.Dm), dy1=e(M, D), dqkv=e(M, 3 * D))
        self.wgrad_groups = {}
        self.bias_groups = {}

        def cp_set():
            cps = dict(fc2=ops.ColsumPartial(B, D, dev), proj=ops.ColsumPartial(B, D, dev),
                       fc1=ops.ColsumPartial((M + 63) // 64, m.Dm, dev), qkv=ops.ColsumPartial(max(B, M // 64), 3 * D, dev))
            cps["fc2"].rows.value = cps["proj"].rows.value = B
            self._bufs += [c.buf for c in cps.values()]
            return cps

        self.cp = [cp_set()] * Lyr if ckpt else [cp_set() for _ in range(Lyr)]
        if not (ckpt and plan.own_dy):
            self.dyb = e(M, D)
        self.delta = e(B * m.num_heads * T, dtype=f32)
        self.dmod, self.dmod_a = e(B, m.mod_cols, dtype=f32), z(m.mod_cols)
        self.dcs, self.dc, self.dc_a = e(B, D, dtype=f32), e(B, D, dtype=f32), z(D)
        self.dh1s, self.dh1, self.dh1_a = e(B, D, dtype=f32), e(B, D, dtype=f32), z(D)
        self.dxp = e(M, m.Kp, dtype=f32)
        if not self.fp8 and self.nbytes() != plan.total:
            raise L.VawError(f"DiT workspace: allocated {self.nbytes()} bytes, vaw_dit_ws_plan says {plan.total}")

    def nbytes(self):
        return sum(t.numel() * t.element_size() for t in self._bufs)


class _DiTFn(torch.autograd.Function):
    @staticmethod
    def forward(ctx, anchor, model, x, t, y):
        out = model._forward_impl(x, t, y)
        ctx.model, ctx.gen, ctx.need_dx = model, model._ws_cur.gen, x.requires_grad
        ctx.x_shape = x.shape
        return out

    @staticmethod
    def backward(ctx, dout):
        m = ctx.model
        if m._ws_cur.gen != ctx.gen:
            raise L.VawError("DiT backward: activations were overwritten by a later forward of the same batch size")
        if m._ws_cur.ckpt != bool(m.activation_checkpointing):
            raise L.VawError("DiT backward: activation_checkpointing was switched between this forward and its backward "
                             "(the workspace of the forward was laid out for the other mode)")
        dx = m._backward_impl(dout.contiguous(), ctx.need_dx)
        return torch.zeros_like(m._anchor), None, dx, None, None


class DiT(FlatModule):
    def __init__(self, image_size=32, patch_size=2, in_channels=4, hidden_size=1152, depth=28, num_heads=16,
                 mlp_ratio=4.0, class_dropout_prob=0.1, num_classes=1000, learn_sigma=False, learn_align=False,
                 encoder_depth=8, z_dims=768, projector_dim=2048, compute_dtype="bf16", activation_checkpointing=False):
        super().__init__()
        if learn_align:
            raise NotImplementedError("learn_align (REPA feature alignment) is outside the hot path (SURVEY §2.1 row 12)")
        assert hidden_size % num_heads == 0 and hidden_size % 4 == 0
        self.learn_sigma, self.learn_align = learn_sigma, learn_align
        self.in_channels = in_channels
        self.out_channels = in_channels * 2 if learn_sigma else in_channels
        self.patch_size, self.num_heads, self.depth = patch_size, num_heads, depth
        self.image_size = image_size
        self.encoder_depth = encoder_depth
        self.x_embedder = _PatchEmbed(image_size, patch_size, in_channels, hidden_size)
        self.t_embedder = _TimestepEmbedder(hidden_size)
        self.y_embedder = _LabelEmbedder(num_classes, hidden_size, class_dropout_prob)
        self.pos_embed = nn.Parameter(torch.zeros(1, self.x_embedder.num_patches, hidden_size), requires_grad=False)
        self.blocks = nn.ModuleList([_Block(hidden_size, num_heads, mlp_ratio) for _ in range(depth)])
        self.projectors = None
        self.final_layer = _FinalLayer(hidden_size, patch_size, self.out_channels)
        self.initialize_weights()
        self.D, self.T = hidden_size, self.x_embedder.num_patches
        self.Dm = int(hidden_size * mlp_ratio)
        self.Kp = in_channels * patch_size * patch_size
        self.No = patch_size * patch_size * self.out_channels
        self.mod_cols = (6 * depth + 2) * hidden_size
        self.fp8_grad_format = "e5m2"
        self.fp8_scaling, self.fp8_margin = "delayed", 2.0
        self.fp8_fuse_epilogue = os.environ.get("VAW_FP8_FUSE", "1") != "0"
        self.fp8_fuse_rows = os.environ.get("VAW_FP8_FUSE_ROWS", "1") != "0"
        self._fp8_w, self._fp8_epoch, self._fp8_wstates, self._fp8_wgroup = {}, None, None, None
        self.activation_checkpointing = False
        self.set_compute_dtype(compute_dtype)
        self._anchor = torch.zeros(1, requires_grad=True)
        self._ws, self._ws_cur = {}, None
        self.set_activation_checkpointing(activation_checkpointing)
        self._ckpt_debug_hook = None
        self.grad_ready_hook = None
        self.defer_wgrad = True

    def initialize_weights(self):
        def basic(mod):
            if isinstance(mod, nn.Linear):
                nn.init.xavier_uniform_(mod.weight)
                if mod.bias is not None:
                    nn.init.constant_(mod.bias, 0)
        self.apply(basic)
        pe = get_2d_sincos_pos_embed(self.pos_embed.shape[-1], int(self.x_embedder.num_patches ** 0.5))
        self.pos_embed.data.copy_(torch.from_numpy(pe).float().unsqueeze(0))
        w = self.x_embedder.proj.weight.data
# ... 212 lines not shown
        mo = ptr(ws.mod) + 4 * (6 * l * D)
        xin, xmid = ptr(ws.xres[2 * l]), ptr(ws.xres[2 * l + 1])
        if xout is None:
            xout = ptr(ws.xres[2 * l + 2])
        fuse_rows = ws.fp8 and ws.d_fwd and self.fp8_fuse_epilogue and self.fp8_fuse_rows and M % 64 == 0 and D % 128 == 0
        if fuse_rows:
            ops.ln_modulate_fwd_fp8(xin, mo, mo + 4 * D, ld, b["f_xm"], ptr(b["mean1"]), ptr(b["rstd1"]), B, T, D)
        else:
            ops.ln_modulate_fwd(dt, xin, mo, mo + 4 * D, ld, ptr(b["xm"]), ptr(b["mean1"]), ptr(b["rstd1"]), B, T, D)
        self._linear_fwd(ws, b, "f_xm", None if fuse_rows else b["xm"], pre + "attn.qkv.", M, 3 * D, D, ptr(b["qkv"]), 3 * D)
        q = ptr(b["qkv"])
        es = self._wsize
        ops.attn_fwd(dt, self._attn_desc(B), q, q + es * D, q + 2 * es * D, ptr(b["ao"]), ptr(b["lse"]))
        self._linear_fwd(ws, b, "f_ao", b["ao"], pre + "attn.proj.", M, D, D, xmid, D, aux_out=ptr(b["y1"]), gate=mo + 4 * 2 * D,
                         gate_ld=ld, resid=xin, rows_per_batch=T, out_f32=True)
        if fuse_rows:
            ops.ln_modulate_fwd_fp8(xmid, mo + 4 * 3 * D, mo + 4 * 4 * D, ld, b["f_xm2"], ptr(b["mean2"]), ptr(b["rstd2"]), B, T, D)
        else:
            ops.ln_modulate_fwd(dt, xmid, mo + 4 * 3 * D, mo + 4 * 4 * D, ld, ptr(b["xm2"]), ptr(b["mean2"]), ptr(b["rstd2"]), B, T, D)
        fuse_a = ws.fp8 and ws.d_fwd and self.fp8_fuse_epilogue and M % 64 == 0
        self._linear_fwd(ws, b, "f_xm2", None if fuse_rows else b["xm2"], pre + "mlp.fc1.", M, Dm, D, b["f_a"].epilogue_target() if fuse_a else ptr(b["a"]), Dm,
                         act=1, aux_out=ptr(b["hpre"]), **({"out_fp8": b["f_a"]} if fuse_a else {}))
        self._linear_fwd(ws, b, "f_a", None if fuse_a else b["a"], pre + "mlp.fc2.", M, D, Dm, xout, D, aux_out=ptr(b["y2"]),
                         gate=mo + 4 * 5 * D, gate_ld=ld, resid=xmid, rows_per_batch=T, out_f32=True)

    def _linear_fwd(self, ws, b, fkey, x, name, M, N, K, out, ldc, **epi):
        if not ws.fp8:
            ops.gemm(self._dt, 1, 1, M, N, K, ptr(x), K, self._w(name + "weight"), K, out, ldc, bias=self._p32(name + "bias"), **epi)
            return
        f = b[fkey].quantize(x, delayed=ws.d_fwd) if x is not None else b[fkey].transpose_from_q()
        w = self._fp8_w[name + "weight"]
        ops.gemm_fp8(M, N, K, f.last_q, K, ptr(f.scale), ptr(w.q), K, ptr(w.scale), out, ldc, bias=self._p32(name + "bias"), **epi)

    def _linear_dgrad(self, ws, b, fkey, dy, name, M, N, K, out, **epi):
        if not ws.fp8:
            ops.gemm(self._dt, 1, 0, M, K, N, ptr(dy) if isinstance(dy, torch.Tensor) else dy, N, self._w(name + "weight"), K, out, K, **epi)
            return
        f = b[fkey].quantize(dy, src_dt=BF16, delayed=ws.d_bwd) if dy is not None else b[fkey].transpose_from_q()
        w = self._fp8_w[name + "weight"]
        ops.gemm_fp8(M, K, N, f.last_q, N, ptr(f.scale), ptr(w.qt), N, ptr(w.scale), out, K, a_format=f.fmt, **epi)

    def _attn_desc(self, B):
        d = getattr(self, "_adesc", None)
        if d is None or d.B != B:
            d = self._adesc = ops.attn_desc_token_major(B, self.num_heads, self.T, self.D // self.num_heads)
        return d

    def _wgrad(self, dt, name, dy, x, Nw, Kw, M, beta, bias=True):
        ops.gemm(dt, 0, 0, Nw, Kw, M, dy, Nw, x, Kw, self._g(name + "weight"), Kw, beta=beta, out_f32=True,
                 rowsum_a_out=self._g(name + "bias") if bias else None, rowsum_a_beta=beta)

    def _adaln_wgrad(self, dt, ws, r0, nrows, B, beta):
        D, ld = self.D, self.mod_cols
        if dt == BF16:
            ops.cast_bf16(ws.dmod, ws.dmod_a)
            dmod_a, es = ptr(ws.dmod_a), 2
        else:
            dmod_a, es = ptr(ws.dmod), 4
        ops.gemm(dt, 0, 0, nrows, D, ws.Bk, dmod_a + es * r0, ld, ptr(ws.cs), D, self._g("blocks.0.adaLN_modulation.1.weight") + 4 * r0 * D,
                 D, beta=beta, out_f32=True)
        ops.colsum(dt, dmod_a + es * r0, B, nrows, ld, self._g("blocks.0.adaLN_modulation.1.bias") + 4 * r0, beta)
        return dmod_a

    def _backward_impl(self, dout, need_dx):
        ws = self._ws_cur
        B = ws.B
        dt, D, T, Dm, Lyr, ld = self._dt, self.D, self.T, self.Dm, self.depth, self.mod_cols
        M, lib, st = B * T, L.lib(), L.stream_ptr()
        H = W = self.image_size
        beta = 1.0 if self.grads_live() else 0.0
        self._gbase = self.flat_grads().data_ptr()
        hook = self.grad_ready_hook
        ada_half = self._ada_split_block() if hook else None
        dres, dD, dDm, dmod = ptr(ws.dres), ptr(ws.dD), ptr(ws.dDm), ptr(ws.dmod)
        mod = ptr(ws.mod)
        es = self._wsize
        defer = ws.defer and dt == BF16
        fp8 = ws.fp8
        own_dy = defer and not fp8
        ckpt = ws.ckpt
        fuse_rows = fp8 and ws.d_bwd and self.fp8_fuse_epilogue and self.fp8_fuse_rows and M % 64 == 0 and D % 128 == 0

        def ln_bwd_and_gate(dout_p, x_p, mean_p, rstd_p, scale_p, dres_in, dsh, dsc, nxt):
            if nxt is None:
                ops.ln_modulate_bwd(dt, dout_p, x_p, mean_p, rstd_p, scale_p, ld, dres_in, dres, dsh, dsc, ld, B, T, D)
                return
            l2, which = nxt
            nb = ws.blk[l2]
            mo2, dmo2 = mod + 4 * (6 * l2 * D), dmod + 4 * (6 * l2 * D)
            gcol = 5 if which == "mlp" else 2
            y, cp = (nb["y2"], ws.cp[l2]["fc2"]) if which == "mlp" else (nb["y1"], ws.cp[l2]["proj"])
            if fuse_rows:
                ops.ln_modulate_bwd_gate_fp8(dout_p, x_p, mean_p, rstd_p, scale_p, ld, dres_in, dres, dsh, dsc, ld, ptr(y),
                                             mo2 + 4 * gcol * D, nb["f_dy2" if which == "mlp" else "f_dy1"], dmo2 + 4 * gcol * D,
                                             B, T, D, cp.buf.data_ptr())
            else:
                dy = ptr(nb["dy2" if which == "mlp" else "dy1"]) if own_dy else ptr(ws.dyb)
                ops.ln_modulate_bwd_gate(dt, dout_p, x_p, mean_p, rstd_p, scale_p, ld, dres_in, dres, dsh, dsc, ld, ptr(y),
                                         mo2 + 4 * gcol * D, dy, dmo2 + 4 * gcol * D, B, T, D, cp.buf.data_ptr())

        L.check(lib.vaw_unpatchify_bwd(dt, ptr(dout), ptr(ws.dotok), B, self.out_channels, H, W, self.patch_size, st), "unpatchify_bwd")
        self._wgrad(dt, "final_layer.linear.", ptr(ws.dotok), ptr(ws.xf), self.No, D, M, beta)
        ops.gemm(dt, 1, 0, M, D, self.No, ptr(ws.dotok), self.No, self._w("final_layer.linear.weight"), D, dD, D)
        mo, dmo = mod + 4 * (6 * Lyr * D), dmod + 4 * (6 * Lyr * D)
        ln_bwd_and_gate(dD, ptr(ws.xres[2 * Lyr]), ptr(ws.meanf), ptr(ws.rstdf), mo + 4 * D, 0, dmo, dmo + 4 * D,
                        (Lyr - 1, "mlp") if (Lyr and not ckpt) else None)
        if hook:
            hook(Lyr + 1)
        pending = []
        group_cut = Lyr // 2 if (hook and Lyr >= 4) else 0

        def fold_bias(blocks, qkv_too):
            key = (blocks[0], blocks[-1], self._gbase, qkv_too)
            cps = []
            for l in blocks:
                cp, pre = ws.cp[l], f"blocks.{l}."
                names = [("fc2", "mlp.fc2."), ("fc1", "mlp.fc1."), ("proj", "attn.proj.")] + ([("qkv", "attn.qkv.")] if qkv_too else [])
                cps += [(cp[key_cp], pre + nm) for key_cp, nm in names]
            rows = tuple(int(cp.rows.value) for cp, _ in cps)
            ent = ws.bias_groups.get(key)
            if ent is None or ent[1] != rows:
                jobs = [(cp.buf.data_ptr(), self._g(nm + "bias"), r, cp.N) for (cp, nm), r in zip(cps, rows)]
                ent = ws.bias_groups[key] = (ops.ReduceGroup(jobs, dout.device), rows)
            grp = ent[0]
            grp.launch(beta)

        def flush():
            if not pending:
                return
            key = (pending[0], pending[-1], self._gbase)
            grp = ws.wgrad_groups.get(key)
            if grp is None:
                probs = []
                for l in pending:
                    b, pre = ws.blk[l], f"blocks.{l}."
                    if fp8:
                        for name, fdy, fx, Nw, Kw in ((pre + "mlp.fc2.", b["f_dy2"], b["f_a"], D, Dm), (pre + "mlp.fc1.", b["f_dhid"], b["f_xm2"], Dm, D),
                                                      (pre + "attn.proj.", b["f_dy1"], b["f_ao"], D, D), (pre + "attn.qkv.", b["f_dqkv"], b["f_xm"], 3 * D, D)):
                            probs.append((ptr(fdy.qt), ptr(fx.qt), self._g(name + "weight"), Nw, Kw, M, M, Kw, 0.0, 0, ptr(fdy.scale), ptr(fx.scale)))
                        continue
                    for name, dy, x, Nw, Kw in ((pre + "mlp.fc2.", b["dy2"], b["a"], D, Dm), (pre + "mlp.fc1.", b["dDm"], b["xm2"], Dm, D),
                                                (pre + "attn.proj.", b["dy1"], b["ao"], D, D), (pre + "attn.qkv.", b["dqkv"], b["xm"], 3 * D, D)):
                        probs.append((ptr(dy), ptr(x), self._g(name + "weight"), Nw, Kw, Nw, Kw, Kw))
                grp = ws.wgrad_groups[key] = ops.WgradGroup(probs, M, dout.device)
            grp.launch((L.BF8 if self.fp8_grad_format == "e5m2" else L.FP8) if fp8 else dt, beta)
            fold_bias(list(pending), True)
            if hook:
                for l in pending:
                    hook(l + 1)
            pending.clear()

        for l in reversed(range(Lyr)):
            b, cp, pre = ws.blk[l], ws.cp[l], f"blocks.{l}."
            mo, dmo = mod + 4 * (6 * l * D), dmod + 4 * (6 * l * D)
            xin, xmid = ptr(ws.xres[2 * l]), ptr(ws.xres[2 * l + 1])
            dy2, dhid, dy1, dq = ((ptr(b["dy2"]), ptr(b["dDm"]), ptr(b["dy1"]), ptr(b["dqkv"])) if own_dy
                                  else (ptr(ws.dyb), dDm, ptr(ws.dyb), ptr(ws.dqkv)))
            if ckpt:
                self._block_fwd(ws, l, xout=ptr(ws.xscr))
                if self._ckpt_debug_hook is not None:
                    self._ckpt_debug_hook(l, b)
                ops.gate_bwd(dt, dres, ptr(b["y2"]), mo + 4 * 5 * D, ld, dy2, dmo + 4 * 5 * D, ld, B, T, D, cp["fc2"].buf.data_ptr())
            if not defer:
                self._wgrad(dt, pre + "mlp.fc2.", dy2, ptr(b["a"]), D, Dm, M, beta, bias=False)
            fuse_dh = fp8 and ws.d_bwd and self.fp8_fuse_epilogue and M % 64 == 0
            self._linear_dgrad(ws, b, "f_dy2", None if fuse_rows else dy2, pre + "mlp.fc2.", M, D, Dm, b["f_dhid"].epilogue_target() if fuse_dh else dhid, act=2,
                               aux_in=ptr(b["hpre"]), colsum_partial=cp["fc1"], **({"out_fp8": b["f_dhid"]} if fuse_dh else {}))
            if not defer:
                self._wgrad(dt, pre + "mlp.fc1.", dhid, ptr(b["xm2"]), Dm, D, M, beta, bias=False)
            self._linear_dgrad(ws, b, "f_dhid", None if (fp8 and fuse_dh) else dhid, pre + "mlp.fc1.", M, Dm, D, dD)
            ln_bwd_and_gate(dD, xmid, ptr(b["mean2"]), ptr(b["rstd2"]), mo + 4 * 4 * D, dres, dmo + 4 * 3 * D, dmo + 4 * 4 * D, (l, "attn"))
            if not defer:
                self._wgrad(dt, pre + "attn.proj.", dy1, ptr(b["ao"]), D, D, M, beta, bias=False)
            self._linear_dgrad(ws, b, "f_dy1", None if fuse_rows else dy1, pre + "attn.proj.", M, D, D, ptr(ws.dao))
            q = ptr(b["qkv"])
            qkv_bias_folded = False
            if defer:
                qkv_bias_folded = ops.attn_bwd_colsum(dt, self._attn_desc(B), q, q + es * D, q + 2 * es * D, ptr(b["ao"]), ptr(ws.dao),
                                                      ptr(b["lse"]), ptr(ws.delta), dq, dq + es * D, dq + 2 * es * D, cp["qkv"])
            if not qkv_bias_folded:
                ops.attn_bwd(dt, self._attn_desc(B), q, q + es * D, q + 2 * es * D, ptr(b["ao"]), ptr(ws.dao), ptr(b["lse"]),
                             ptr(ws.delta), dq, dq + es * D, dq + 2 * es * D)
                if defer:
                    ops.colsum(dt, dq, M, 3 * D, 3 * D, cp["qkv"].buf.data_ptr(), 0.0, device=dout.device)
                    cp["qkv"].rows.value = 1
                else:
                    self._wgrad(dt, pre + "attn.qkv.", dq, ptr(b["xm"]), 3 * D, D, M, beta)
            self._linear_dgrad(ws, b, "f_dqkv", dq, pre + "attn.qkv.", M, 3 * D, D, dD)
            ln_bwd_and_gate(dD, xin, ptr(b["mean1"]), ptr(b["rstd1"]), mo + 4 * D, dres, dmo, dmo + 4 * D,
                            (l - 1, "mlp") if (l and not ckpt) else None)
            if defer:
                pending.append(l)
                if ckpt or l == group_cut:
                    pending.reverse()
                    flush()
            else:
                fold_bias([l], False)
            if hook:
                if not defer:
                    hook(l + 1)
                if l == ada_half:
                    r0 = 6 * l * D
                    self._adaln_wgrad(dt, ws, r0, ld - r0, B, beta)
                    hook("ada_hi")
        pending.reverse()
        flush()
        if dt == BF16:
            ops.cast_bf16(ws.dres, ws.dD)
            dx0 = dD
        else:
            dx0 = dres
        self._wgrad(dt, "x_embedder.proj.", dx0, ptr(ws.xp), D, self.Kp, M, beta)
        dx = None
        if need_dx:
            ops.gemm(dt, 1, 0, M, self.Kp, D, dx0, D, self._w("x_embedder.proj.weight"), self.Kp, ptr(ws.dxp), self.Kp, out_f32=True)
            dx = torch.empty(B, self.in_channels, H, W, device=dout.device, dtype=torch.float32)
            L.check(lib.vaw_patchify_bwd(ptr(ws.dxp), ptr(dx), B, self.in_channels, H, W, self.patch_size, st), "patchify_bwd")
        rows = ld if ada_half is None else 6 * ada_half * D
        dmod_a = self._adaln_wgrad(dt, ws, 0, rows, B, beta)
        ops.gemm(dt, 1, 0, B, D, ld, dmod_a, ld, self._w("blocks.0.adaLN_modulation.1.weight"), D, ptr(ws.dcs), D, out_f32=True)
        L.check(lib.vaw_silu_bwd(ptr(ws.c), ptr(ws.dcs), ptr(ws.dc), B * D, st), "silu_bwd")
        ye = self.y_embedder.embedding_table
        L.check(lib.vaw_embedding_bwd(ptr(ws.dc), ptr(ws.y), self._g("y_embedder.embedding_table.weight"), B, D,
                                      ye.num_embeddings, beta, st), "embedding_bwd")
        if dt == BF16:
            ops.cast_bf16(ws.dc, ws.dc_a)
            dc_a = ptr(ws.dc_a)
        else:
            dc_a = ptr(ws.dc)
        self._wgrad(dt, "t_embedder.mlp.2.", dc_a, ptr(ws.h1s), D, D, ws.Bk, beta)
        ops.gemm(dt, 1, 0, B, D, D, dc_a, D, self._w("t_embedder.mlp.2.weight"), D, ptr(ws.dh1s), D, out_f32=True)
        L.check(lib.vaw_silu_bwd(ptr(ws.h1), ptr(ws.dh1s), ptr(ws.dh1), B * D, st), "silu_bwd")
        if dt == BF16:
            ops.cast_bf16(ws.dh1, ws.dh1_a)
            dh1_a = ptr(ws.dh1_a)
        else:
            dh1_a = ptr(ws.dh1)
        self._wgrad(dt, "t_embedder.mlp.0.", dh1_a, ptr(ws.tfreq), D, 256, ws.Bk, beta)
        self.attach_grads()
        if fp8:
            ws.calib_bwd = True
        if hook:
            hook(0)
        return dx


_PRESETS = {"DiT-S": (384, 12, 6), "DiT-B": (768, 12, 12), "DiT-L": (1024, 24, 16), "DiT-XL": (1152, 28, 16)}


def _make(name):
    hidden, depth, heads = _PRESETS[name]

    def build(image_size, patch_size, in_channels, class_dropout_prob, num_classes, learn_sigma, **kwargs):
        return DiT(image_size=image_size, patch_size=patch_size, in_channels=in_channels, hidden_size=hidden,
                   depth=depth, num_heads=heads, class_dropout_prob=class_dropout_prob, num_classes=num_classes,
                   learn_sigma=learn_sigma, **kwargs)
    build.__name__ = name.replace("-", "_")
    return build


DiT_S, DiT_B, DiT_L, DiT_XL = (_make(n) for n in ("DiT-S", "DiT-B", "DiT-L", "DiT-XL"))
DiT_models = {"DiT-S": DiT_S, "DiT-B": DiT_B, "DiT-L": DiT_L, "DiT-XL": DiT_XL}
```

### variance-aware-weight_amd/gaussian_diffusion.py

```python
import enum
import math

import numpy as np
import torch

from . import ops


class ModelMeanType(enum.Enum):
    PREVIOUS_X = enum.auto()
    START_X = enum.auto()
    EPSILON = enum.auto()
    VELOCITY = enum.auto()
    VECTOR = enum.auto()
    SCORE = enum.auto()


class ModelVarType(enum.Enum):
    LEARNED = enum.auto()
    FIXED_SMALL = enum.auto()
    FIXED_LARGE = enum.auto()
    LEARNED_RANGE = enum.auto()


# ... 406 lines not shown
        return self._reverse_step(3, model, x, t, clip_denoised, denoised_fn, None, model_kwargs)

    def ddim_reverse_sample_loop_progressive(self, model, x_start, clip_denoised=True, model_kwargs=None, progress=False):
        indices = list(range(self.num_timesteps))
        if progress:
            from tqdm.auto import tqdm
            indices = tqdm(indices)
        x = x_start
        for i in indices:
            t = torch.full((x.shape[0],), i, device=x.device, dtype=torch.long)
            with torch.no_grad():
                out = self.ddim_reverse_sample(model, x, t, clip_denoised=clip_denoised, model_kwargs=model_kwargs)
                yield out
                x = out["sample"]

    def ddim_reverse_sample_loop(self, model, x_start, clip_denoised=True, model_kwargs=None, progress=False):
        final = None
        for final in self.ddim_reverse_sample_loop_progressive(model, x_start, clip_denoised, model_kwargs, progress):
            pass
        return final["sample"]

    def _vb_terms_bpd(self, mean_out, var_out, x_start, x_t, t, scale=1.0):
        self._refuse_unsupported_mean_type()
        mt, vt = self.model_mean_type, self.model_var_type
        var_mode = {ModelVarType.LEARNED: 1, ModelVarType.LEARNED_RANGE: 2}.get(vt, 0)
        coef = self._tables(x_start.device)["vb"][t]
        return ops.vb_terms(mean_out, var_out, x_start, x_t, coef, 1 if mt == ModelMeanType.PREVIOUS_X else 0, var_mode, scale)

    def _scale_timesteps(self, t):
        if self.rescale_timesteps:
            return t.float() * (1000.0 / self.num_timesteps)
        return t

    def q_sample(self, x_start, t, noise=None):
        if noise is None:
            noise = torch.randn_like(x_start)
        assert noise.shape == x_start.shape
        tb = self._tables(x_start.device)
        return ops.qsample(x_start.contiguous(), noise.contiguous(), t, tb["a"], tb["s"])

    def sample_t(self, x_start):
        if self.args.time_dist[0] == "uniform":
            return torch.randint(0, self.num_timesteps, (x_start.shape[0],), device=x_start.device)
        raise NotImplementedError(f"Unknown time_dist: {self.args.time_dist}")

    def compute_target(self, x_start, noise, t, alpha=None, sigma=None):
        tb = self._tables(x_start.device)
        if self.model_mean_type == ModelMeanType.START_X:
            return x_start
        if self.model_mean_type == ModelMeanType.EPSILON:
            return noise
        return ops.mix_rows(x_start.contiguous(), noise.contiguous(), tb["ca"][t], tb["cb"][t])

    def training_losses(self, model, x_start, features=None, t=None, model_kwargs=None, noise=None):
        if model_kwargs is None:
            model_kwargs = {}
        if noise is None:
            noise = torch.randn_like(x_start)
        if t is None:
            t = self.sample_t(x_start)
        kl_loss = self.loss_type in (LossType.KL, LossType.RESCALED_KL)
        if not kl_loss and self.loss_type not in (LossType.MSE, LossType.RESCALED_MSE):
            raise NotImplementedError(self.loss_type)
        if getattr(self.args, "learn_align", False):
            raise NotImplementedError("learn_align: feature-alignment teachers are out of scope (SURVEY.md §2.1 row 12)")
        x_start = x_start.contiguous()
        noise = noise.contiguous()
        tb = self._tables(x_start.device)
        x_t = ops.qsample(x_start, noise, t, tb["a"], tb["s"])
        raw_output = model(x_t, self._scale_timesteps(t), **model_kwargs)
        model_output = raw_output[0] if isinstance(raw_output, tuple) else raw_output
        learned = self.model_var_type in (ModelVarType.LEARNED, ModelVarType.LEARNED_RANGE)
        var_values = None
        if learned:
            B, C = x_t.shape[:2]
            assert model_output.shape == (B, C * 2, *x_t.shape[2:])
            model_output, var_values = torch.split(model_output, C, dim=1)
        if kl_loss:
            scale = float(self.num_timesteps) if self.loss_type == LossType.RESCALED_KL else 1.0
            return {"loss": self._vb_terms_bpd(model_output, var_values, x_start, x_t, t, scale)}
        terms = {}
        if learned:
            scale = self.num_timesteps / 1000.0 if self.loss_type == LossType.RESCALED_MSE else 1.0
            terms["vb"] = self._vb_terms_bpd(model_output.detach(), var_values, x_start, x_t, t, scale)
        assert model_output.shape == x_start.shape
        terms["mse"] = ops.weighted_mse(model_output, x_start, noise, tb["ca"][t], tb["cb"][t], tb["w"][t])
        terms["loss"] = terms["mse"] + terms["vb"] if "vb" in terms else terms["mse"]
        return terms


class FlowMatching:

    def __init__(self, *, args, model_mean_type, device="cuda"):
        self.args = args
        self.model_mean_type = model_mean_type
        self.mse_loss_weight_type = args.weight_type
        self.path_type = args.path_type
        self.sampler_type = getattr(args, "sampler_type", "ode")
        self.p2_gamma = args.p2_gamma
        self.p2_k = args.p2_k
        self.gamma = args.gamma
        self.learn_sigma = args.learn_sigma

    def expand_t_like_x(self, t, x):
        if t.dim() == 0:
            t = t.expand(x.shape[0])
        return t.view(t.size(0), *([1] * (len(x.size()) - 1))).to(x)

    def interpolant(self, t):
        if self.path_type == "linear":
            return 1 - t, t, torch.full_like(t, -1.0), torch.full_like(t, 1.0)
        if self.path_type == "cosine":
            return (torch.cos(t * np.pi / 2), torch.sin(t * np.pi / 2), -np.pi / 2 * torch.sin(t * np.pi / 2),
                    np.pi / 2 * torch.cos(t * np.pi / 2))
        if self.path_type == "linear_logsnr":
            lam = 10 + t * (-10.0 - 10)
            alpha_t, sigma_t = torch.sigmoid(0.5 * lam), torch.sigmoid(-0.5 * lam)
            d_alpha_t = -10.0 * alpha_t * sigma_t
            return alpha_t, sigma_t, d_alpha_t, -d_alpha_t
        raise NotImplementedError()

    def sample_t(self, x_start):
        td = self.args.time_dist
        if td[0] == "uniform":
            return torch.rand(x_start.shape[0], device=x_start.device)
        if td[0] == "lognorm":
            mu, sigma = float(td[-2]), float(td[-1])
            return torch.sigmoid(torch.randn(x_start.shape[0], device=x_start.device) * sigma + mu)
        raise NotImplementedError(f"Unknown time_dist: {td}")

    def q_sample(self, x_start, noise, t):
        alpha_t, sigma_t, _, _ = self.interpolant(t.float())
        return ops.mix_rows(x_start.contiguous(), noise.contiguous(), alpha_t.contiguous(), sigma_t.contiguous())

    def _target_coefs(self, alpha_t, sigma_t, d_alpha_t, d_sigma_t):
        mt = self.model_mean_type
        one, zero = torch.ones_like(alpha_t), torch.zeros_like(alpha_t)
        if mt == ModelMeanType.START_X:
            return one, zero
        if mt == ModelMeanType.EPSILON:
            return zero, one
        if mt == ModelMeanType.VELOCITY:
            return -sigma_t, alpha_t
        if mt == ModelMeanType.VECTOR:
            return d_alpha_t, d_sigma_t
        if mt == ModelMeanType.SCORE:
            return zero, -1.0 / sigma_t
        raise KeyError(mt)

    def compute_target(self, x_start, noise, t, alpha_t=None, sigma_t=None, d_alpha_t=None, d_sigma_t=None):
        if alpha_t is None or sigma_t is None or d_alpha_t is None or d_sigma_t is None:
            alpha_t, sigma_t, d_alpha_t, d_sigma_t = self.interpolant(t)
        ca, cb = self._target_coefs(alpha_t, sigma_t, d_alpha_t, d_sigma_t)
        return ops.mix_rows(x_start.contiguous(), noise.contiguous(), ca.float().contiguous(), cb.float().contiguous())

    def training_losses(self, model, x_start, features=None, t=None, model_kwargs=None, noise=None):
        if model_kwargs is None:
            model_kwargs = {}
        if noise is None:
            noise = torch.randn_like(x_start)
        if t is None:
            t = self.sample_t(x_start)
        if getattr(self.args, "learn_align", False):
            raise NotImplementedError("learn_align: feature-alignment teachers are out of scope (SURVEY.md §2.1 row 12)")
        x_start, noise = x_start.contiguous(), noise.contiguous()
        alpha_t, sigma_t, d_alpha_t, d_sigma_t = self.interpolant(t)
        x_t = ops.mix_rows(x_start, noise, alpha_t.contiguous(), sigma_t.contiguous())
        ca, cb = self._target_coefs(alpha_t, sigma_t.clone(), d_alpha_t, d_sigma_t)
        w = compute_mse_loss_weight(self.model_mean_type, self.mse_loss_weight_type, t, alpha_t, sigma_t, self.p2_k,
                                    self.p2_gamma)
        raw_output = model(x_t, t, **model_kwargs)
        model_output = raw_output[0] if isinstance(raw_output, tuple) else raw_output
        assert model_output.shape == x_start.shape
        terms = {"mse": ops.weighted_mse(model_output, x_start, noise, ca.float().contiguous(), cb.float().contiguous(),
                                         w.float().contiguous())}
        terms["loss"] = terms["mse"]
        return terms
```

### variance-aware-weight_amd/ops.py

```python
import ctypes as C

import torch

from . import _lib as L
from ._lib import BF16, F32, AttnDesc, Epilogue, check, need_cuda, ptr, stream_ptr


def dt_of(t):
    if t.dtype == torch.float32:
        return F32
    if t.dtype == torch.bfloat16:
        return BF16
    raise L.VawError(f"unsupported activation dtype {t.dtype}")


def _f32c(*ts):
    for t in ts:
        if t is not None and (t.dtype != torch.float32 or not t.is_contiguous()):
            raise L.VawError(f"expected a contiguous float32 tensor, got {t.dtype} contiguous={t.is_contiguous()}")


def qsample(x0, noise, t, tab_a, tab_s):
    need_cuda(x0, noise, t, tab_a, tab_s)
    _f32c(x0, noise, tab_a, tab_s)
    assert noise.shape == x0.shape and t.dtype == torch.int64 and t.shape == (x0.shape[0],)
    out = torch.empty_like(x0)
    B = x0.shape[0]
    check(L.lib().vaw_qsample_fwd(ptr(x0), ptr(noise), ptr(t), ptr(tab_a), ptr(tab_s), tab_a.numel(), ptr(out), B,
                                  x0.numel() // B, stream_ptr()), "vaw_qsample_fwd")
    return out


def mix_rows(x, y, ca, cb):
    need_cuda(x, y, ca, cb)
    _f32c(x, y, ca, cb)
    assert x.shape == y.shape and ca.shape == cb.shape == (x.shape[0],)
    out = torch.empty_like(x)
    B = x.shape[0]
    check(L.lib().vaw_mix_rows(ptr(x), ptr(y), ptr(ca), ptr(cb), ptr(out), B, x.numel() // B, stream_ptr()), "vaw_mix_rows")
    return out


class _WeightedMSE(torch.autograd.Function):
    @staticmethod
    def forward(ctx, model_out, x0, noise, ca, cb, w):
        need_cuda(model_out, x0, noise, ca, cb, w)
        model_out = model_out.contiguous()
        _f32c(model_out, x0, noise, ca, cb, w)
        B = x0.shape[0]
        assert model_out.shape == x0.shape == noise.shape and ca.shape == cb.shape == w.shape == (B,)
        mse = torch.empty(B, device=x0.device, dtype=torch.float32)
        check(L.lib().vaw_wmse_fwd(ptr(model_out), ptr(x0), ptr(noise), ptr(ca), ptr(cb), ptr(w), ptr(mse), B,
                                   x0.numel() // B, stream_ptr()), "vaw_wmse_fwd")
        ctx.save_for_backward(model_out, x0, noise, ca, cb, w)
        return mse

    @staticmethod
    def backward(ctx, gmse):
        model_out, x0, noise, ca, cb, w = ctx.saved_tensors
        gmse = gmse.contiguous().float()
        dout = torch.empty_like(model_out)
        B = x0.shape[0]
        check(L.lib().vaw_wmse_bwd(ptr(model_out), ptr(x0), ptr(noise), ptr(ca), ptr(cb), ptr(w), ptr(gmse), ptr(dout),
                                   B, x0.numel() // B, stream_ptr()), "vaw_wmse_bwd")
        return dout, None, None, None, None, None


def weighted_mse(model_out, x0, noise, ca, cb, w):
    return _WeightedMSE.apply(model_out, x0, noise, ca, cb, w)


class _VbTerms(torch.autograd.Function):

    @staticmethod
    def forward(ctx, mean_out, var_out, x0, x_t, coef, mean_mode, var_mode, scale):
        need_cuda(mean_out, x0, x_t, coef)
        _f32c(mean_out, x0, x_t, coef)
        B = x0.shape[0]
        assert mean_out.shape == x0.shape == x_t.shape and coef.shape == (B, 8)
        if var_out is not None:
            need_cuda(var_out)
            _f32c(var_out)
            assert var_out.shape == x0.shape
        vb = torch.empty(B, device=x0.device, dtype=torch.float32)
        check(L.lib().vaw_vb_fwd(ptr(mean_out), ptr(var_out) if var_out is not None else None, ptr(x0), ptr(x_t), ptr(coef),
                                 mean_mode, var_mode, scale, ptr(vb), B, x0.numel() // B, stream_ptr()), "vaw_vb_fwd")
        ctx.save_for_backward(mean_out, var_out, x0, x_t, coef)
        ctx.modes = (mean_mode, var_mode, scale)
        return vb

    @staticmethod
    def backward(ctx, gvb):
        mean_out, var_out, x0, x_t, coef = ctx.saved_tensors
        mean_mode, var_mode, scale = ctx.modes
        gvb = gvb.contiguous().float()
        d_mean = torch.empty_like(mean_out) if ctx.needs_input_grad[0] else None
        d_var = torch.empty_like(var_out) if (var_out is not None and ctx.needs_input_grad[1]) else None
        B = x0.shape[0]
        if d_mean is not None or d_var is not None:
            check(L.lib().vaw_vb_bwd(ptr(mean_out), ptr(var_out) if var_out is not None else None, ptr(x0), ptr(x_t), ptr(coef),
                                     mean_mode, var_mode, scale, ptr(gvb), ptr(d_mean) if d_mean is not None else None,
                                     ptr(d_var) if d_var is not None else None, B, x0.numel() // B, stream_ptr()), "vaw_vb_bwd")
        return d_mean, d_var, None, None, None, None, None, None


def vb_terms(mean_out, var_out, x0, x_t, coef, mean_mode, var_mode, scale=1.0):
    return _VbTerms.apply(mean_out.contiguous(), None if var_out is None else var_out.contiguous(), x0, x_t, coef,
                          int(mean_mode), int(var_mode), float(scale))


def _step_outputs(kind, x, want_all):
    res = {"pred_xstart": torch.empty_like(x)}
    if kind:
        res["sample"] = torch.empty_like(x)
    if want_all:
        res["mean"], res["log_variance"] = torch.empty_like(x), torch.empty_like(x)
    return res


def sample_step(kind, mean_out, var_out, x, noise, coef, mean_mode, var_mode, clip_denoised, eta=0.0, want_all=False):
    need_cuda(mean_out, x, coef)
    x = x.contiguous().float()
# ... 517 lines not shown
    _f32c(bias, gate, resid, rowadd)
    gemm(dt, a_kmajor, b_kmajor, M, N, K, ptr(A), A.shape[1], ptr(B), B.shape[1], ptr(out), N, bias=ptr(bias), act=act,
         aux_in=ptr(aux_in), aux_out=ptr(aux), gate=ptr(gate), gate_ld=(gate.shape[-1] if gate is not None else 0),
         resid=ptr(resid), rowadd=ptr(rowadd), rows_per_batch=rows_per_batch, alpha=alpha, beta=beta,
         out_f32=(out.dtype == torch.float32), colsum_out=ptr(colsum_out), colsum_beta=colsum_beta,
         rowsum_a_out=ptr(rowsum_a_out), rowsum_a_beta=rowsum_a_beta)
    return (out, aux) if want_aux else out


_scratch = {}


def scratch_f32(device, n):
    t = _scratch.get(device)
    if t is None or t.numel() < n:
        t = _scratch[device] = torch.empty(max(n, 1 << 26), device=device, dtype=torch.float32)
    return t


def colsum(dt, X, M, N, ldx, out, beta=0.0, device=None):
    need = L.lib().vaw_colsum_workspace_floats(M, N)
    ws = scratch_f32(device or torch.device("cuda", torch.cuda.current_device()), need)
    check(L.lib().vaw_colsum(dt, X, M, N, ldx, out, beta, ptr(ws), ws.numel(), stream_ptr()), "vaw_colsum")


def ln_modulate_fwd(dt, x, shift, scale, mod_ld, out, mean, rstd, B, T, D, eps=1e-6):
    check(L.lib().vaw_ln_modulate_fwd(dt, x, shift, scale, mod_ld, out, mean, rstd, B, T, D, eps, stream_ptr()),
          "vaw_ln_modulate_fwd")


def ln_modulate_fwd_fp8(x, shift, scale, mod_ld, f8, mean, rstd, B, T, D, eps=1e-6, pool=2):
    q = f8.epilogue_target(pool)
    check(L.lib().vaw_ln_modulate_fwd_fp8(x, shift, scale, mod_ld, q, f8.state.data_ptr(), f8.fmt, mean, rstd, B, T, D, eps, stream_ptr()),
          "vaw_ln_modulate_fwd_fp8")


def gate_bwd_fp8(dres, y, gate, mod_ld, f8, dgate, dmod_ld, B, T, D, dy_colpart=0, pool=2):
    ws = _row_ws(B, T, D)
    q = f8.epilogue_target(pool)
    check(L.lib().vaw_gate_bwd_fp8(dres, y, gate, mod_ld, q, f8.state.data_ptr(), f8.fmt, dgate, dmod_ld, dy_colpart or None, B, T, D,
                                   ws.data_ptr(), ws.numel(), stream_ptr()), "vaw_gate_bwd_fp8")


def row_plan(kind, dt, B, T, D, workspace_floats=0, ldx=0, base_addr=0):
    p = L.RowLaunch()
    check(L.lib().vaw_row_plan(kind, dt, B, T, D, ldx, base_addr, workspace_floats, C.byref(p)), "vaw_row_plan")
    return p


def _row_ws(B, T, D):
    return scratch_f32(torch.device("cuda", torch.cuda.current_device()), L.lib().vaw_row_bwd_workspace_floats(B, T, D))


def ln_modulate_bwd(dt, dout, x, mean, rstd, scale, mod_ld, dres_in, dx, dshift, dscale, dmod_ld, B, T, D):
    ws = _row_ws(B, T, D)
    check(L.lib().vaw_ln_modulate_bwd(dt, dout, x, mean, rstd, scale, mod_ld, dres_in or None, dx, dshift, dscale,
                                      dmod_ld, B, T, D, ws.data_ptr(), ws.numel(), stream_ptr()), "vaw_ln_modulate_bwd")


def ln_modulate_bwd_gate(dt, dout, x, mean, rstd, scale, mod_ld, dres_in, dx, dshift, dscale, dmod_ld, y_next, gate_next, dy_next,
                         dgate_next, B, T, D, dy_colpart=0):
    if D > 1280:
        ln_modulate_bwd(dt, dout, x, mean, rstd, scale, mod_ld, dres_in, dx, dshift, dscale, dmod_ld, B, T, D)
        gate_bwd(dt, dx, y_next, gate_next, mod_ld, dy_next, dgate_next, dmod_ld, B, T, D, dy_colpart)
        return
    ws = _row_ws(B, T, D)
    check(L.lib().vaw_ln_modulate_bwd_gate(dt, dout, x, mean, rstd, scale, mod_ld, dres_in or None, dx, dshift, dscale, dmod_ld,
                                           y_next, gate_next, dy_next, dgate_next, dy_colpart or None, B, T, D, ws.data_ptr(),
                                           ws.numel(), stream_ptr()), "vaw_ln_modulate_bwd_gate")


def ln_modulate_bwd_gate_fp8(dout, x, mean, rstd, scale, mod_ld, dres_in, dx, dshift, dscale, dmod_ld, y_next, gate_next, f8,
                             dgate_next, B, T, D, dy_colpart=0, pool=2):
    if D > 1280:
        ln_modulate_bwd(BF16, dout, x, mean, rstd, scale, mod_ld, dres_in, dx, dshift, dscale, dmod_ld, B, T, D)
        gate_bwd_fp8(dx, y_next, gate_next, mod_ld, f8, dgate_next, dmod_ld, B, T, D, dy_colpart, pool)
        return
    ws = _row_ws(B, T, D)
    q = f8.epilogue_target(pool)
    check(L.lib().vaw_ln_modulate_bwd_gate_fp8(dout, x, mean, rstd, scale, mod_ld, dres_in or None, dx, dshift, dscale, dmod_ld,
                                               y_next, gate_next, q, f8.state.data_ptr(), f8.fmt, dgate_next, dy_colpart or None,
                                               B, T, D, ws.data_ptr(), ws.numel(), stream_ptr()), "vaw_ln_modulate_bwd_gate_fp8")


class ColsumPartial:

    def __init__(self, max_rows, N, device):
        self.buf = torch.empty(max_rows, N, device=device, dtype=torch.float32)
        self.N = int(N)
        self.rows = C.c_int64(0)


class ReduceJob(C.Structure):
    _fields_ = [("partial", C.c_void_p), ("out", C.c_void_p), ("R", C.c_int64), ("N", C.c_int64)]


class ReduceGroup:

    def __init__(self, jobs, device):
        self.n = len(jobs)
        self.table = (ReduceJob * self.n)(*[ReduceJob(*j) for j in jobs])
        self.desc = torch.empty(L.lib().vaw_reduce_rows_batched_desc_bytes(self.n), device=device, dtype=torch.uint8)
        self.uploaded = False

    def launch(self, beta):
        check(L.lib().vaw_reduce_rows_batched(self.n, C.cast(self.table, C.c_void_p), float(beta), self.desc.data_ptr(),
                                              0 if self.uploaded else 1, stream_ptr()), "vaw_reduce_rows_batched")
        self.uploaded = True
# ... 38 lines not shown
def attn_fwd(dt, desc, q, k, v, o, lse):
    check(L.lib().vaw_attn_fwd(dt, C.byref(desc), q, k, v, o, lse, stream_ptr()), "vaw_attn_fwd")


def attn_bwd(dt, desc, q, k, v, o, d_o, lse, delta, dq, dk, dv):
    check(L.lib().vaw_attn_bwd(dt, C.byref(desc), q, k, v, o, d_o, lse, delta, dq, dk, dv, stream_ptr()), "vaw_attn_bwd")


def attn_bwd_colsum(dt, desc, q, k, v, o, d_o, lse, delta, dq, dk, dv, partial):
    partial.rows.value = partial.buf.shape[0]
    rc = L.lib().vaw_attn_bwd_colsum(dt, C.byref(desc), q, k, v, o, d_o, lse, delta, dq, dk, dv, partial.buf.data_ptr(),
                                     C.byref(partial.rows), stream_ptr())
    if rc == -3:
        return False
    check(rc, "vaw_attn_bwd_colsum")
    return True


def timestep_embedding(t, dim, dtype=torch.float32, max_period=10000.0):
    need_cuda(t)
    t = t.float().contiguous()
    out = torch.empty(t.shape[0], dim, device=t.device, dtype=dtype)
    check(L.lib().vaw_timestep_embedding(dt_of(out), ptr(t), ptr(out), t.shape[0], dim, max_period, stream_ptr()),
          "vaw_timestep_embedding")
    return out


def sumsq(g, out, accumulate=False):
    ws = scratch_f32(g.device, L.lib().vaw_sumsq_workspace_floats())
    check(L.lib().vaw_sumsq(ptr(g), g.numel(), ptr(out), 1 if accumulate else 0, ptr(ws), stream_ptr()), "vaw_sumsq")


def adamw_ema_step(p, g, m, v, ema, shadow, lr, beta1, beta2, eps, wd, step, ema_decay, sumsq_t, clip, zero_grad, hyper=None):
    if hyper is not None:
        check(L.lib().vaw_adamw_ema_step_dev(ptr(p), ptr(g), ptr(m), ptr(v), ptr(ema), ptr(shadow), p.numel(), ptr(hyper), beta1,
                                             beta2, eps, wd, ema_decay, ptr(sumsq_t), clip or 0.0, 1 if zero_grad else 0,
                                             stream_ptr()), "vaw_adamw_ema_step_dev")
        return
    bc1 = 1.0 - beta1 ** step
    bc2 = 1.0 - beta2 ** step
    check(L.lib().vaw_adamw_ema_step(ptr(p), ptr(g), ptr(m), ptr(v), ptr(ema), ptr(shadow), p.numel(), lr, beta1, beta2,
                                     eps, wd, bc1, bc2, ema_decay, ptr(sumsq_t), clip or 0.0, 1 if zero_grad else 0,
                                     stream_ptr()), "vaw_adamw_ema_step")


def ema_update(ema, src, decay):
    check(L.lib().vaw_ema_update(ptr(ema), ptr(src), ema.numel(), decay, stream_ptr()), "vaw_ema_update")


def cast_bf16(src, dst):
    check(L.lib().vaw_cast_bf16(ptr(src), ptr(dst), src.numel(), stream_ptr()), "vaw_cast_bf16")


def uncast_bf16(src, dst, scale=1.0):
    check(L.lib().vaw_uncast_bf16(ptr(src), ptr(dst), src.numel(), float(scale), stream_ptr()), "vaw_uncast_bf16")


def groupnorm_apply(dt, x, mean, rstd, gamma, beta, scale, shift, film_ld, silu, y, B, HW, C, G=32):
    check(L.lib().vaw_groupnorm_apply(dt, x, mean, rstd, gamma, beta, scale or None, shift or None, film_ld, 1 if silu else 0, y,
                                      B, HW, C, G, stream_ptr()), "vaw_groupnorm_apply")


def dropout_pack(dt, mask, M, C):
    bits = torch.empty(L.lib().vaw_dropout_bits_words(M * C), device=mask.device, dtype=torch.int32)
    check(L.lib().vaw_dropout_pack(dt, ptr(mask), ptr(bits), M, C, stream_ptr()), "vaw_dropout_pack")
    return bits


def dropout_bits(dt, x, bits, keep_scale, y, n, backward=False):
    fn = L.lib().vaw_dropout_bits_bwd if backward else L.lib().vaw_dropout_bits_fwd
    check(fn(dt, x, ptr(bits), keep_scale, y, n, stream_ptr()), "vaw_dropout_bits_bwd" if backward else "vaw_dropout_bits_fwd")
```

### variance-aware-weight_amd/respace.py

```python
import numpy as np
import torch

from .gaussian_diffusion import GaussianDiffusion


def _ddim_stride(num_timesteps, count):
    stride = -(-num_timesteps // count) if count > 0 else 0
    if not (1 <= stride < num_timesteps) or -(-num_timesteps // stride) != count:
        raise ValueError(f"cannot create exactly {num_timesteps} steps with an integer stride")
    return stride


def space_timesteps(num_timesteps, section_counts):
    if isinstance(section_counts, str):
        if section_counts.startswith("ddim"):
            return set(range(0, num_timesteps, _ddim_stride(num_timesteps, int(section_counts[4:]))))
        section_counts = [int(tok) for tok in section_counts.split(",")]
    counts = np.asarray(section_counts, dtype=np.int64)
    sizes = np.full(len(counts), num_timesteps // len(counts), dtype=np.int64)
    sizes[: num_timesteps % len(counts)] += 1
    short = np.nonzero(sizes < counts)[0]
    if short.size:
        raise ValueError(f"cannot divide section of {int(sizes[short[0]])} steps into {int(counts[short[0]])}")
    firsts = np.cumsum(sizes) - sizes
    kept = set()
    for first, size, count in zip(firsts.tolist(), sizes.tolist(), counts.tolist()):
        if count <= 0:
            continue
        step = 1.0 if count == 1 else (size - 1) / (count - 1)
        offsets = np.concatenate(([0.0], np.cumsum(np.full(count - 1, step, dtype=np.float64))))
        kept.update((first + np.rint(offsets).astype(np.int64)).tolist())
    return kept


class SpacedDiffusion(GaussianDiffusion):

    def __init__(self, use_timesteps, **kwargs):
        base_betas = np.asarray(kwargs["betas"], dtype=np.float64)
        self.original_num_steps = int(base_betas.shape[0])
        self.use_timesteps = set(use_timesteps)
        keep = np.array(sorted(k for k in self.use_timesteps if 0 <= k < self.original_num_steps), dtype=np.int64)
        self.timestep_map = keep.tolist()
        abar = np.cumprod(1.0 - base_betas, axis=0)[keep]
        kwargs["betas"] = 1 - abar / np.concatenate(([1.0], abar[:-1]))
        super().__init__(**kwargs)

    def _reverse_step(self, kind, model, *args, **kwargs):
        return super()._reverse_step(kind, self._respaced(model), *args, **kwargs)

    def training_losses(self, model, *args, **kwargs):
        return super().training_losses(self._respaced(model), *args, **kwargs)

    def calc_bpd_loop(self, model, *args, **kwargs):
        return super().calc_bpd_loop(self._respaced(model), *args, **kwargs)

    def _scale_timesteps(self, t):
        return t

    def _host_model_time(self, i):
        k = self.timestep_map[i]
        return float(np.float32(k) * np.float32(1000.0 / self.original_num_steps)) if self.rescale_timesteps else float(k)

    def _kept_steps_on(self, like):
        cache = self.__dict__.setdefault("_kept_cache", {})
        key = (like.device, like.dtype)
        if key not in cache:
            cache[key] = torch.as_tensor(self.timestep_map, device=like.device, dtype=like.dtype)
        return cache[key]

    def _respaced(self, model):
        if getattr(model, "_vaw_respaced_by", None) is self:
            return model
        factor = 1000.0 / self.original_num_steps if self.rescale_timesteps else None

        def original(j):
            k = self._kept_steps_on(j).index_select(0, j.reshape(-1)).reshape(j.shape)
            return k.float() * factor if factor is not None else k

        def call(x, j, **kwargs):
            return model(x, original(j), **kwargs)

        call._vaw_respaced_by = self
        if hasattr(model, "guided_halves"):
            call.guided_halves = lambda x, j, t_mean=None, **kwargs: model.guided_halves(x, original(j), t_mean=t_mean, **kwargs)
            call.unguided = lambda x, j, **kwargs: model.unguided(x, original(j), **kwargs)
            call.combine, call.guidance_scale = model.combine, model.guidance_scale
        if hasattr(model, "parameters"):
            call.parameters = model.parameters
        return call
```

### variance-aware-weight_amd/trainer.py

```python
from contextlib import nullcontext

import torch
import torch.nn as nn

from . import dist_util, ops
from .flat import FlatModule
from .optim import FusedAdamW


def ema(source, target, decay):
    s, t = getattr(source, "module", source), getattr(target, "module", target)
    with torch.no_grad():
        if isinstance(s, FlatModule) and isinstance(t, FlatModule):
            s.ensure_flat(); t.ensure_flat()
            if s._flat_offsets == t._flat_offsets and s._flat.is_cuda and not list(s.buffers()):
                ops.ema_update(t._flat, s._flat, decay)
                t.mark_weights_changed()
                return
        src, dst = source.state_dict(), target.state_dict()
        for k in src:
            dst[k].data.copy_(dst[k].data * decay + src[k].data * (1 - decay))
        if isinstance(t, FlatModule) and getattr(t, "_flat", None) is not None:
            t.mark_weights_changed()


def sample_from_latent(latent, latent_scale=1.0, cpu_rng=False):
    mean, std = torch.chunk(latent, 2, dim=1)
    eps = torch.randn(mean.shape).to(mean.device) if cpu_rng else torch.randn_like(mean)
    return (mean + std * eps) * latent_scale


class Trainer:
    def __init__(self, args, device, model, ema_model, optimizer, scheduler, diffusion, train_loader, pbar=None):
        if getattr(args, "learn_align", False):
            raise NotImplementedError("learn_align needs network-fetched teacher encoders: out of scope (SURVEY.md §2.1 row 12)")
        self.args, self.device = args, device
        self.model, self.ema_model = model, ema_model
        self.optimizer, self.scheduler, self.diffusion = optimizer, scheduler, diffusion
        self.train_loader = train_loader
        self.datalooper = iter(train_loader)
        self.pbar = pbar
        self.scaler = None
        inner = getattr(model, "module", model)
        if hasattr(inner, "set_compute_dtype"):
            low = getattr(args, "amp_dtype", None) or (inner.compute_dtype if inner.compute_dtype in ("bf16", "fp8") else "bf16")
            want = low if args.amp else "fp32"
            if inner.compute_dtype != want:
                inner.set_compute_dtype(want)
        ckpt = getattr(args, "activation_checkpointing", None)
        if ckpt is not None and hasattr(inner, "set_activation_checkpointing"):
            if inner.activation_checkpointing != bool(ckpt):
                inner.set_activation_checkpointing(ckpt)
        elif ckpt:
            raise ValueError(f"args.activation_checkpointing: {type(inner).__name__} has no activation recomputation (the DiT and UNet models do)")
        if hasattr(inner, "host_dropout_rng"):
            inner.host_dropout_rng = bool(getattr(args, "cpu_rng", False))
        self._fused = isinstance(optimizer, FusedAdamW)
        self._zero = self._fused and getattr(optimizer, "zero", None) is not None
        if getattr(inner, "_zero", None) is not None and not self._zero:
            raise ValueError("the model was wrapped with shard_optimizer=True: it needs a vaw_amd.FusedAdamW built after the wrap "
                             f"(got {type(optimizer).__name__}{' built before the wrap' if self._fused else ''})")
        if self._zero:
            if getattr(args, "ema_decay", None) is not None:
                optimizer.attach_ema_sharded(args.ema_decay, ema_model)
        elif self._fused and ema_model is not None and dist_util.is_main_process():
            optimizer.attach_ema(ema_model, args.ema_decay)
        self.last_mse = None
        self._cpu_rng = bool(getattr(args, "cpu_rng", False))
        self.schedule_sampler, self._device_sampler = None, False
        name = getattr(args, "schedule_sampler", None)
        if name and name != "uniform":
            from .resample import create_named_schedule_sampler
            self.schedule_sampler = create_named_schedule_sampler(name, diffusion, device=device)
            self._device_sampler = hasattr(self.schedule_sampler, "ring")
            if getattr(args, "hip_graph", False) and not self._device_sampler:
                raise ValueError("args.schedule_sampler updates its history on the host every step: not with args.hip_graph")
        self._graph, self._graph_calls, self._gin, self._gout = None, 0, None, None
        hg = getattr(args, "hip_graph", False)
        self._graph_auto = hg == "auto"
        self._use_graph = bool(hg)
        if self._use_graph:
            why = ("needs vaw_amd.FusedAdamW" if not self._fused else "not with DDP (args.parallel)" if args.parallel else
                   "not with grad_accumulation > 1" if max(1, args.grad_accumulation) > 1 else
                   "not with args.cpu_rng" if self._cpu_rng else "needs a CUDA device" if torch.device(device).type != "cuda" else
                   "the model draws its label-drop mask on the host every step (UNet drop_label_prob > 0)"
                   if getattr(inner, "host_rng_in_forward", False) else None)
            if why and self._graph_auto:
                self._use_graph = False
            elif why:
                raise ValueError(f"args.hip_graph: {why}")
            else:
                optimizer.enable_device_hyper()

    def _get_next_batch(self):
        try:
            images, labels = next(self.datalooper)
        except StopIteration:
            self.datalooper = iter(self.train_loader)
            return self._get_next_batch()
        return (images.to(self.device, non_blocking=True),
                labels.to(self.device, non_blocking=True) if self.args.class_cond else None)

    def _compute_loss(self, images, labels, features):
        model_kwargs = {"y": labels} if self.args.class_cond else {}
        if self._cpu_rng and not self._device_sampler:
            noise = torch.randn(images.shape).to(images.device)
            t = torch.randint(0, self.diffusion.num_timesteps, (images.shape[0],)).to(images.device)
            return self.diffusion.training_losses(self.model, images, features, t=t, model_kwargs=model_kwargs, noise=noise)
        if self.schedule_sampler is not None:
            noise = torch.randn(images.shape).to(images.device) if self._cpu_rng else None
            t, w = self.schedule_sampler.sample(images.shape[0], images.device)
            terms = self.diffusion.training_losses(self.model, images, features, t=t, model_kwargs=model_kwargs, noise=noise)
            self.schedule_sampler.update_with_local_losses(t, terms["loss"].detach())
            terms = dict(terms)
            terms["loss"] = terms["loss"] * w
            return terms
        return self.diffusion.training_losses(self.model, images, features, model_kwargs=model_kwargs)

    def _apply_gradient_clipping(self):
        if self.args.grad_clip:
            if self._fused:
                self.optimizer.max_grad_norm = float(self.args.grad_clip)
            else:
                nn.utils.clip_grad_norm_(self.model.parameters(), self.args.grad_clip)

    def consolidate(self):
        if self._zero:
            self.optimizer.consolidate()
            if getattr(self.optimizer, "_ema_shard", None) is not None:
                self.optimizer.consolidate_ema(self.ema_model)

    def _update_ema(self):
        if self._zero:
            return
        if dist_util.is_main_process() and self.ema_model is not None:
            if self._fused and getattr(self.optimizer, "ema_done_in_step", False):
                return
            ema(self.model, self.ema_model, self.args.ema_decay)

    def _graph_body(self, images, labels):
        a = self.args
        if a.in_chans == 4:
            images = sample_from_latent(images, a.latent_scale, False)
        loss_dict = self._compute_loss(images, labels, None)
        loss = loss_dict["loss"].mean()
        loss.backward()
        self._apply_gradient_clipping()
        self.optimizer.step()
        self.optimizer.zero_grad()
        return loss.detach(), (loss_dict["mse"].detach().mean() if "mse" in loss_dict else torch.zeros_like(loss.detach()))

    def eager_from_now_on(self):
        if self._use_graph:
            self._graph, self._gin, self._gout = None, None, None
            self._graph_calls = -(1 << 60)

    def _train_step_graph(self, step):
        a = self.args
        self.model.train()
        images, labels = self._get_next_batch()
        self.optimizer.prepare_step()
        self._graph_calls += 1
        if self._graph is None and self._graph_calls <= 2:
            if self._graph_auto and self._graph_calls == 2:
                import time
                e0, e1 = torch.cuda.Event(enable_timing=True), torch.cuda.Event(enable_timing=True)
                torch.cuda.synchronize()
                t0 = time.perf_counter()
                e0.record()
                total, mse = self._graph_body(images, labels)
                e1.record()
                host_ms = 1e3 * (time.perf_counter() - t0)
                torch.cuda.synchronize()
                self.graph_decision = dict(host_ms=host_ms, gpu_ms=e0.elapsed_time(e1))
                if host_ms < 0.7 * self.graph_decision["gpu_ms"]:
                    self._graph_calls = -(1 << 60)
            else:
                total, mse = self._graph_body(images, labels)
        elif self._graph_calls < 0:
            total, mse = self._graph_body(images, labels)
        else:
            if self._graph is None:
                self._gin = (images.clone(), None if labels is None else labels.clone())
                torch.cuda.synchronize()
                g = torch.cuda.CUDAGraph()
                with torch.cuda.graph(g):
                    self._gout = self._graph_body(*self._gin)
                self._graph = g
            else:
                self._gin[0].copy_(images, non_blocking=True)
                if labels is not None:
                    self._gin[1].copy_(labels, non_blocking=True)
            self._graph.replay()
            total, mse = self._gout
        self.scheduler.step()
        if dist_util.is_main_process():
            self._update_ema()
        self.last_mse = mse
        if dist_util.is_main_process() and self.pbar is not None:
            self.pbar.update(1)
        if getattr(a, "defer_loss_sync", False):
            return total
        total_f = float(total.item())
        if dist_util.is_main_process() and self.pbar is not None:
            self.pbar.set_postfix(mse=f"{float(mse.item()):.4f}")
        return total_f

    def train_step(self, step):
        if self._use_graph:
            return self._train_step_graph(step)
        a = self.args
        self.model.train()
        if a.parallel:
            self.train_loader.sampler.set_epoch(step)
        accum = max(1, a.grad_accumulation)
        total, mse_avg = None, None
        for i in range(accum):
            images, labels = self._get_next_batch()
            if a.in_chans == 4:
                images = sample_from_latent(images, a.latent_scale, self._cpu_rng)
            if a.parallel and accum > 1 and i < accum - 1:
                ctx = self.model.no_sync()
            else:
                ctx = nullcontext()
            with ctx:
                loss_dict = self._compute_loss(images, labels, None)
                loss = loss_dict["loss"].mean() / accum
                loss.backward()
            ld = loss.detach()
            md = loss_dict["mse"].detach().mean() / accum if "mse" in loss_dict else torch.zeros_like(ld)
            total = ld if total is None else total + ld
            mse_avg = md if mse_avg is None else mse_avg + md
            if (i + 1) % accum == 0:
                self._apply_gradient_clipping()
                self.optimizer.step()
                self.optimizer.zero_grad()
        self.scheduler.step()
        if dist_util.is_main_process():
            self._update_ema()
        self.last_mse = mse_avg
        if getattr(a, "defer_loss_sync", False):
            if dist_util.is_main_process() and self.pbar is not None:
                self.pbar.update(1)
            return total
        total_f = float(total.item())
        if dist_util.is_main_process() and self.pbar is not None:
            self.pbar.update(1)
            self.pbar.set_postfix(mse=f"{float(mse_avg.item()):.4f}")
        return total_f
```

Before: 20410 images/sec.

## Fuse latent sampling, q_sample, weighted MSE and mean into step-level kernels

Adds a fused training-step path, on by default through an environment flag. Latent sampling and q_sample become one kernel, and the weighted MSE gathers its coefficients by timestep on the device and produces the batch mean directly, which removes several small elementwise launches and extra passes over memory. It also adds backward kernels that write a bf16 copy alongside the fp32 result (SiLU bwd, LN-modulate bwd, cast+colsum), and it rewrites the embedding backward to find matching rows with ballot masks instead of a serial scan. The trade-off is more code paths and dispatch logic in the trainer, and some of the new kernels may only be wired up in parts of the code that are not shown.

```diff
diff --git a/include/vaw_hip.h b/include/vaw_hip.h
--- a/include/vaw_hip.h
+++ b/include/vaw_hip.h
@@ -25,6 +25,16 @@
                  const float* w, float* mse, int B, int64_t per_sample, vaw_stream stream);
 int vaw_wmse_bwd(const float* model_out, const float* x0, const float* noise, const float* ca, const float* cb,
                  const float* w, const float* gmse, float* dout, int B, int64_t per_sample, vaw_stream stream);
+
+int vaw_latent_qsample(const float* latent, const float* eps, const float* noise, const int64_t* t, const float* tab_a,
+                       const float* tab_s, int num_timesteps, float latent_scale, float t_scale, float* x0, float* x_t,
+                       float* t_float, int B, int64_t per_sample, vaw_stream stream);
+int vaw_wmse_fwd_t(const float* model_out, const float* x0, const float* noise, const int64_t* t, const float* ca, const float* cb,
+                   const float* w, int num_timesteps, float* mse, float* mean_out, float accum, int B, int64_t per_sample,
+                   vaw_stream stream);
+int vaw_wmse_bwd_t(const float* model_out, const float* x0, const float* noise, const int64_t* t, const float* ca, const float* cb,
+                   const float* w, int num_timesteps, const float* g, float inv_count, float* dout, int B, int64_t per_sample,
+                   vaw_stream stream);
 
 int vaw_vb_fwd(const float* mean_out, const float* var_out, const float* x0, const float* x_t, const float* coef,
                int mean_mode, int var_mode, float scale, float* vb, int B, int64_t per_sample, vaw_stream stream);
@@ -213,6 +223,10 @@
                         const float* scale, int64_t mod_ld, const float* dres_in, float* dx, float* dshift,
                         float* dscale, int64_t dmod_ld, int B, int T, int D, float* workspace, int64_t workspace_floats,
                         vaw_stream stream);
+int vaw_ln_modulate_bwd_cast(vaw_dtype dt, const void* dout, const float* x, const float* mean, const float* rstd,
+                             const float* scale, int64_t mod_ld, const float* dres_in, float* dx, float* dshift,
+                             float* dscale, int64_t dmod_ld, int B, int T, int D, float* workspace, int64_t workspace_floats,
+                             void* dx_act, vaw_stream stream);
 int vaw_ln_modulate_fwd_fp8(const float* x, const float* shift, const float* scale, int64_t mod_ld, void* q_out, float* q_state,
                             vaw_dtype q_format, float* mean, float* rstd, int B, int T, int D, float eps, vaw_stream stream);
 int vaw_gate_bwd_fp8(const float* dres, const void* y, const float* gate, int64_t mod_ld, void* dy_q, float* q_state,
@@ -262,6 +276,7 @@
                            vaw_stream stream);
 int vaw_silu_fwd(vaw_dtype dt, const float* x, void* out, int64_t n, vaw_stream stream);
 int vaw_silu_bwd(const float* x, const float* dy, float* dx, int64_t n, vaw_stream stream);
+int vaw_silu_bwd_cast(const float* x, const float* dy, float* dx, void* dx_bf16, int64_t n, vaw_stream stream);
 int vaw_add_embedding(const float* a, const float* table, const int64_t* idx, float* out, int B, int D,
                       int num_rows, vaw_stream stream);
 int vaw_embedding_bwd(const float* dc, const int64_t* idx, float* dtable, int B, int D, int num_rows, float beta,
@@ -357,6 +372,15 @@
                            const float* sumsq, float clip_max_norm, int zero_grad, vaw_stream stream);
 int vaw_ema_update(float* ema, const float* src, int64_t n, float decay, vaw_stream stream);
 int vaw_cast_bf16(const float* src, void* dst, int64_t n, vaw_stream stream);
+typedef struct {
+    int grid_x, block;
+    int rows_per_lane;
+    int64_t bytes_read, bytes_written;
+} vaw_cast_colsum_launch;
+int vaw_cast_colsum_plan(int64_t M, int64_t N, int64_t ld_src, int64_t ld_dst, int64_t src_addr, int64_t dst_addr,
+                         int64_t colsum_addr, vaw_cast_colsum_launch* out);
+int vaw_cast_colsum_bf16(const float* src, int64_t ld_src, void* dst, int64_t ld_dst, int64_t M, int64_t N, float* colsum,
+                         float beta, vaw_stream stream);
 int vaw_uncast_bf16(const void* src, float* dst, int64_t n, float scale, vaw_stream stream);
 
 typedef struct {
diff --git a/variance-aware-weight_amd/_lib.py b/variance-aware-weight_amd/_lib.py
--- a/variance-aware-weight_amd/_lib.py
+++ b/variance-aware-weight_amd/_lib.py
@@ -49,6 +49,10 @@
 class DitWsPlan(C.Structure):
     _fields_ = [("records", _i), ("colsum_sets", _i), ("own_dy", _i), ("Bk", _i), ("block_bytes", _l), ("block_stat_bytes", _l),
                 ("shared_bytes", _l), ("colsum_bytes", _l), ("scratch_bytes", _l), ("cond_bytes", _l), ("total", _l)]
+
+
+class CastColsumLaunch(C.Structure):
+    _fields_ = [("grid_x", _i), ("block", _i), ("rows_per_lane", _i), ("bytes_read", _l), ("bytes_written", _l)]
 
 
 ATTN_FWD, ATTN_BWD, ATTN_BWD_COLSUM = range(3)
@@ -156,6 +160,13 @@
     "vaw_attn_plan": [_i, _i, C.POINTER(AttnDesc), _l, _l, _l, _l, _l, _l, _l, C.POINTER(AttnLaunch)],
     "vaw_gemm_plan": [_i, _i, _i, _l, _l, _l, _l, _l, _l, _l, _l, _l, C.POINTER(Epilogue), _l, C.POINTER(GemmKnobs), C.POINTER(GemmLaunch)],
     "vaw_dit_ws_plan": [_i, _i, _i, _i, _i, _i, _i, _i, _i, _i, _i, C.POINTER(DitWsPlan)],
+    "vaw_latent_qsample": [_p, _p, _p, _p, _p, _p, _i, _f, _f, _p, _p, _p, _i, _l, _p],
+    "vaw_wmse_fwd_t": [_p, _p, _p, _p, _p, _p, _p, _i, _p, _p, _f, _i, _l, _p],
+    "vaw_wmse_bwd_t": [_p, _p, _p, _p, _p, _p, _p, _i, _p, _f, _p, _i, _l, _p],
+    "vaw_ln_modulate_bwd_cast": [_i, _p, _p, _p, _p, _p, _l, _p, _p, _p, _p, _l, _i, _i, _i, _p, _l, _p, _p],
+    "vaw_silu_bwd_cast": [_p, _p, _p, _p, _l, _p],
+    "vaw_cast_colsum_plan": [_l, _l, _l, _l, _l, _l, _l, C.POINTER(CastColsumLaunch)],
+    "vaw_cast_colsum_bf16": [_p, _l, _p, _l, _l, _l, _p, _f, _p],
 }
 
 _lib = None
@@ -230,6 +241,9 @@
                                    "vaw_gemm_default_knobs", "vaw_dropout_bits_words"])
 
 
+STEP_FUSED = os.environ.get("VAW_STEP_FUSED", "1") != "0"
+
+
 def check(rc, what):
     if rc != 0:
         raise VawError(f"{what} failed ({rc}): {lib().vaw_last_error_string().decode()}")
diff --git a/variance-aware-weight_amd/csrc/elementwise.hip b/variance-aware-weight_amd/csrc/elementwise.hip
--- a/variance-aware-weight_amd/csrc/elementwise.hip
+++ b/variance-aware-weight_amd/csrc/elementwise.hip
@@ -4,6 +4,14 @@
     int64_t g = (work_items + block - 1) / block;
     const int64_t cap = 256 * 8;
     return (int)(g < 1 ? 1 : (g > cap ? cap : g));
+}
+
+__device__ __forceinline__ void gather_mix_coef(const float* __restrict__ ca, const float* __restrict__ cb, const int64_t* __restrict__ t,
+                                                int T, int b, float& a, float& c) {
+    const int64_t tt = t[b];
+    const bool ok = tt >= 0 && tt < T;
+    a = ok ? ca[tt] : __builtin_nanf("");
+    c = ok ? cb[tt] : __builtin_nanf("");
 }
 
 template <bool GATHER>
@@ -13,10 +21,7 @@
     const int b = blockIdx.y;
     float a, c;
     if (GATHER) {
-        const int64_t tt = t[b];
-        const bool ok = tt >= 0 && tt < T;
-        a = ok ? ca[tt] : __builtin_nanf("");
-        c = ok ? cb[tt] : __builtin_nanf("");
+        gather_mix_coef(ca, cb, t, T, b, a, c);
     } else {
         a = ca[b];
         c = cb[b];
@@ -54,12 +59,20 @@
     return VAW_OK;
 }
 
-__global__ void wmse_fwd_kernel(const float* __restrict__ o, const float* __restrict__ x0, const float* __restrict__ nz,
-                                const float* __restrict__ ca, const float* __restrict__ cb, const float* __restrict__ w,
-                                float* __restrict__ mse, int64_t n) {
+struct WmseCoef { float a, c, w; };
+__device__ __forceinline__ WmseCoef wmse_coef(const float* ca, const float* cb, const float* w, const int64_t* t, int T, int b) {
+    if (!t) return WmseCoef{ca[b], cb[b], w[b]};
+    const int64_t tt = t[b];
+    const float nan = __builtin_nanf("");
+    return (tt >= 0 && tt < T) ? WmseCoef{ca[tt], cb[tt], w[tt]} : WmseCoef{nan, nan, nan};
+}
+__global__ void wmse_fwd_t_kernel(const float* __restrict__ o, const float* __restrict__ x0, const float* __restrict__ nz,
+                                  const float* __restrict__ ca, const float* __restrict__ cb, const float* __restrict__ w,
+                                  const int64_t* __restrict__ t, int T, float* __restrict__ mse, int64_t n) {
     __shared__ float scratch[16];
     const int b = blockIdx.x;
-    const float a = ca[b], c = cb[b];
+    const WmseCoef k = wmse_coef(ca, cb, w, t, T, b);
+    const float a = k.a, c = k.c;
     const float* orow = o + (int64_t)b * n;
     const float* xr = x0 + (int64_t)b * n;
     const float* nr = nz + (int64_t)b * n;
@@ -74,15 +87,17 @@
         acc += d * d;
     }
     float tot = block_sum(acc, scratch);
-    if (threadIdx.x == 0) mse[b] = w[b] * (tot / (float)n);
-}
-
-__global__ void wmse_bwd_kernel(const float* __restrict__ o, const float* __restrict__ x0, const float* __restrict__ nz,
-                                const float* __restrict__ ca, const float* __restrict__ cb, const float* __restrict__ w,
-                                const float* __restrict__ gmse, float* __restrict__ dout, int64_t n) {
+    if (threadIdx.x == 0) mse[b] = k.w * (tot / (float)n);
+}
+__global__ void wmse_bwd_t_kernel(const float* __restrict__ o, const float* __restrict__ x0, const float* __restrict__ nz,
+                                  const float* __restrict__ ca, const float* __restrict__ cb, const float* __restrict__ w,
+                                  const int64_t* __restrict__ t, int T, const float* __restrict__ g, int g_per_row, float inv_count,
+                                  float* __restrict__ dout, int64_t n) {
     const int b = blockIdx.y;
-    const float a = ca[b], c = cb[b];
-    const float k = gmse[b] * w[b] * 2.f / (float)n;
+    const WmseCoef kc = wmse_coef(ca, cb, w, t, T, b);
+    const float a = kc.a, c = kc.c;
+    const float gm = g_per_row ? g[b] : g[0] * inv_count;
+    const float k = gm * kc.w * 2.f / (float)n;
     const float* orow = o + (int64_t)b * n;
     const float* xr = x0 + (int64_t)b * n;
     const float* nr = nz + (int64_t)b * n;
@@ -93,12 +108,19 @@
     for (int64_t i = n4 * 4 + blockIdx.x * (int64_t)blockDim.x + threadIdx.x; i < n; i += (int64_t)gridDim.x * blockDim.x)
         dr[i] = k * (orow[i] - a * xr[i] - c * nr[i]);
 }
+__global__ void __launch_bounds__(256) batch_mean_kernel(const float* __restrict__ v, int B, float accum, float* __restrict__ out) {
+    __shared__ float scratch[4];
+    float acc = 0.f;
+    for (int i = threadIdx.x; i < B; i += 256) acc += v[i];
+    const float tot = block_sum(acc, scratch);
+    if (threadIdx.x == 0) out[0] = (tot / (float)B) / accum;
+}
 
 extern "C" int vaw_wmse_fwd(const float* model_out, const float* x0, const float* noise, const float* ca,
                             const float* cb, const float* w, float* mse, int B, int64_t per_sample,
                             vaw_stream stream) {
     VAW_CHECK_ARG(B > 0 && per_sample > 0, "wmse_fwd: bad sizes");
-    wmse_fwd_kernel<<<B, 1024, 0, (hipStream_t)stream>>>(model_out, x0, noise, ca, cb, w, mse, per_sample);
+    wmse_fwd_t_kernel<<<B, 1024, 0, (hipStream_t)stream>>>(model_out, x0, noise, ca, cb, w, nullptr, 0, mse, per_sample);
     VAW_CHECK_LAUNCH("wmse_fwd");
     return VAW_OK;
 }
@@ -109,7 +131,7 @@
     VAW_CHECK_ARG(B > 0 && per_sample > 0, "wmse_bwd: bad sizes");
     int gx = stream_grid(per_sample / 4 + 1, 256);
     dim3 grid(gx > 64 ? 64 : gx, B);
-    wmse_bwd_kernel<<<grid, 256, 0, (hipStream_t)stream>>>(model_out, x0, noise, ca, cb, w, gmse, dout, per_sample);
+    wmse_bwd_t_kernel<<<grid, 256, 0, (hipStream_t)stream>>>(model_out, x0, noise, ca, cb, w, nullptr, 0, gmse, 1, 1.f, dout, per_sample);
     VAW_CHECK_LAUNCH("wmse_bwd");
     return VAW_OK;
 }
@@ -727,6 +749,14 @@
     for (int64_t i = blockIdx.x * (int64_t)blockDim.x + threadIdx.x; i < n; i += (int64_t)gridDim.x * blockDim.x)
         dx[i] = dy[i] * silu_grad_f(x[i]);
 }
+__global__ void silu_bwd_cast_kernel(const float* __restrict__ x, const float* __restrict__ dy, float* __restrict__ dx,
+                                     bf16_t* __restrict__ dx_act, int64_t n) {
+    for (int64_t i = blockIdx.x * (int64_t)blockDim.x + threadIdx.x; i < n; i += (int64_t)gridDim.x * blockDim.x) {
+        const float v = dy[i] * silu_grad_f(x[i]);
+        dx[i] = v;
+        dx_act[i] = (bf16_t)v;
+    }
+}
 extern "C" int vaw_silu_fwd(vaw_dtype dt, const float* x, void* out, int64_t n, vaw_stream stream) {
     VAW_CHECK_ARG(n > 0, "silu_fwd: n<=0");
     int grid = stream_grid(n, 256);
@@ -753,7 +783,7 @@
 __global__ void __launch_bounds__(256)
 embedding_bwd_kernel(const float* __restrict__ dc, const int64_t* __restrict__ idx, float* __restrict__ dtable, int B, int D,
                      int rows, float beta) {
-    __shared__ int s_idx[1024];
+    __shared__ unsigned long long s_mask[16];
     const int r = blockIdx.x;
     constexpr int MAXC = 8;
     for (int d0 = 0; d0 < D; d0 += 256 * MAXC) {
@@ -763,15 +793,24 @@
         for (int b0 = 0; b0 < B; b0 += 1024) {
             const int nb = B - b0 < 1024 ? B - b0 : 1024;
             __syncthreads();
-            for (int i = threadIdx.x; i < nb; i += 256) s_idx[i] = (int)idx[b0 + i];
+#pragma unroll
+            for (int k = 0; k < 4; ++k) {
+                const int i = threadIdx.x + 256 * k;
+                const unsigned long long m = __ballot(i < nb && idx[b0 + (i < nb ? i : 0)] == (int64_t)r);
+                if ((threadIdx.x & 63) == 0) s_mask[4 * k + (threadIdx.x >> 6)] = m;
+            }
             __syncthreads();
-            for (int i = 0; i < nb; ++i) {
-                if (s_idx[i] != r) continue;
-                const float* src = dc + (int64_t)(b0 + i) * D + d0;
-#pragma unroll
-                for (int j = 0; j < MAXC; ++j) {
-                    const int d = threadIdx.x + 256 * j;
-                    if (d0 + d < D) acc[j] += src[d];
+            for (int w = 0; w < 16; ++w) {
+                unsigned long long m = s_mask[w];
+                while (m) {
+                    const int i = 64 * w + __builtin_ctzll(m);
+                    m &= m - 1;
+                    const float* src = dc + (int64_t)(b0 + i) * D + d0;
+#pragma unroll
+                    for (int j = 0; j < MAXC; ++j) {
+                        const int d = threadIdx.x + 256 * j;
+                        if (d0 + d < D) acc[j] += src[d];
+                    }
                 }
             }
         }
@@ -785,6 +824,14 @@
         }
     }
 }
+extern "C" int vaw_silu_bwd_cast(const float* x, const float* dy, float* dx, void* dx_bf16, int64_t n, vaw_stream stream) {
+    if (!dx_bf16) return vaw_silu_bwd(x, dy, dx, n, stream);
+    VAW_CHECK_ARG(n > 0, "silu_bwd_cast: n<=0");
+    silu_bwd_cast_kernel<<<stream_grid(n, 256), 256, 0, (hipStream_t)stream>>>(x, dy, dx, (bf16_t*)dx_bf16, n);
+    VAW_CHECK_LAUNCH("silu_bwd_cast");
+    return VAW_OK;
+}
+
 extern "C" int vaw_add_embedding(const float* a, const float* table, const int64_t* idx, float* out, int B, int D,
                                  int num_rows, vaw_stream stream) {
     VAW_CHECK_ARG(B > 0 && D > 0 && num_rows > 0, "add_embedding: bad sizes");
@@ -1056,3 +1103,140 @@
     VAW_CHECK_LAUNCH("uncast_bf16");
     return VAW_OK;
 }
+
+__global__ void latent_qsample_kernel(const float* __restrict__ latent, const float* __restrict__ eps, const float* __restrict__ noise,
+                                      const int64_t* __restrict__ t, const float* __restrict__ tab_a, const float* __restrict__ tab_s,
+                                      int T, float scale, float t_scale, float* __restrict__ x0, float* __restrict__ x_t,
+                                      float* __restrict__ tf, int64_t n) {
+    const int b = blockIdx.y;
+    float a, c;
+    gather_mix_coef(tab_a, tab_s, t, T, b, a, c);
+    if (tf && blockIdx.x == 0 && threadIdx.x == 0) tf[b] = (float)t[b] * t_scale;
+    const float* mr = latent + (int64_t)b * 2 * n;
+    const float* sr = mr + n;
+    const float* er = eps + (int64_t)b * n;
+    const float* nr = noise + (int64_t)b * n;
+    float* xr = x0 + (int64_t)b * n;
+    float* orow = x_t + (int64_t)b * n;
+    const int64_t n4 = ((n & 3) == 0) ? n / 4 : 0;
+    for (int64_t i = blockIdx.x * (int64_t)blockDim.x + threadIdx.x; i < n4; i += (int64_t)gridDim.x * blockDim.x) {
+        const f32x4 x = (load4(mr + 4 * i) + load4(sr + 4 * i) * load4(er + 4 * i)) * scale;
+        store4(xr + 4 * i, x);
+        store4(orow + 4 * i, a * x + c * load4(nr + 4 * i));
+    }
+    for (int64_t i = n4 * 4 + blockIdx.x * (int64_t)blockDim.x + threadIdx.x; i < n; i += (int64_t)gridDim.x * blockDim.x) {
+        const float x = (mr[i] + sr[i] * er[i]) * scale;
+        xr[i] = x;
+        orow[i] = a * x + c * nr[i];
+    }
+}
+
+extern "C" int vaw_latent_qsample(const float* latent, const float* eps, const float* noise, const int64_t* t, const float* tab_a,
+                                  const float* tab_s, int num_timesteps, float latent_scale, float t_scale, float* x0, float* x_t,
+                                  float* t_float, int B, int64_t per_sample, vaw_stream stream) {
+    VAW_CHECK_ARG(B > 0 && B <= 65535 && per_sample > 0 && num_timesteps > 0, "latent_qsample: bad sizes B=%d n=%ld", B, (long)per_sample);
+    VAW_CHECK_ARG(latent && eps && noise && t && tab_a && tab_s && x0 && x_t, "latent_qsample: null pointer");
+    VAW_CHECK_ARG(per_sample % 4 != 0 || ((((uintptr_t)latent | (uintptr_t)eps | (uintptr_t)noise | (uintptr_t)x0 | (uintptr_t)x_t) & 15) == 0),
+                  "latent_qsample: tensors must be 16-byte aligned");
+    int gx = stream_grid(per_sample / 4 + 1, 256);
+    dim3 grid(gx > 64 ? 64 : gx, B);
+    latent_qsample_kernel<<<grid, 256, 0, (hipStream_t)stream>>>(latent, eps, noise, t, tab_a, tab_s, num_timesteps, latent_scale, t_scale,
+                                                                x0, x_t, t_float, per_sample);
+    VAW_CHECK_LAUNCH("latent_qsample");
+    return VAW_OK;
+}
+
+extern "C" int vaw_wmse_fwd_t(const float* model_out, const float* x0, const float* noise, const int64_t* t, const float* ca,
+                              const float* cb, const float* w, int num_timesteps, float* mse, float* mean_out, float accum, int B,
+                              int64_t per_sample, vaw_stream stream) {
+    VAW_CHECK_ARG(B > 0 && per_sample > 0 && (!t || num_timesteps > 0) && accum >= 1.f, "wmse_fwd_t: bad sizes");
+    VAW_CHECK_ARG(model_out && x0 && noise && ca && cb && w && mse, "wmse_fwd_t: null pointer");
+    wmse_fwd_t_kernel<<<B, 1024, 0, (hipStream_t)stream>>>(model_out, x0, noise, ca, cb, w, t, num_timesteps, mse, per_sample);
+    if (mean_out) batch_mean_kernel<<<1, 256, 0, (hipStream_t)stream>>>(mse, B, accum, mean_out);
+    VAW_CHECK_LAUNCH("wmse_fwd_t");
+    return VAW_OK;
+}
+
+extern "C" int vaw_wmse_bwd_t(const float* model_out, const float* x0, const float* noise, const int64_t* t, const float* ca,
+                              const float* cb, const float* w, int num_timesteps, const float* g, float inv_count, float* dout, int B,
+                              int64_t per_sample, vaw_stream stream) {
+    VAW_CHECK_ARG(B > 0 && B <= 65535 && per_sample > 0 && (!t || num_timesteps > 0), "wmse_bwd_t: bad sizes");
+    VAW_CHECK_ARG(model_out && x0 && noise && ca && cb && w && g && dout, "wmse_bwd_t: null pointer");
+    int gx = stream_grid(per_sample / 4 + 1, 256);
+    dim3 grid(gx > 64 ? 64 : gx, B);
+    wmse_bwd_t_kernel<<<grid, 256, 0, (hipStream_t)stream>>>(model_out, x0, noise, ca, cb, w, t, num_timesteps, g, 0, inv_count, dout,
+                                                            per_sample);
+    VAW_CHECK_LAUNCH("wmse_bwd_t");
+    return VAW_OK;
+}
+
+#define CC_U 16
+__global__ void __launch_bounds__(256)
+cast_colsum_kernel(const float* __restrict__ X, int64_t ldx, bf16_t* __restrict__ Y, int64_t ldy, int64_t M, int64_t N,
+                   float* __restrict__ out, float beta) {
+    __shared__ __attribute__((aligned(16))) float part[4][256];
+    const int cg = threadIdx.x & 63, rg = threadIdx.x >> 6;
+    const int64_t col = (int64_t)blockIdx.x * 256 + cg * 4;
+    f32x4 acc = {0, 0, 0, 0};
+    if (col < N) {
+        int64_t r = rg;
+        for (; r + 4 * (CC_U - 1) < M; r += 4 * CC_U) {
+            f32x4 v[CC_U];
+#pragma unroll
+            for (int u = 0; u < CC_U; ++u) v[u] = __builtin_nontemporal_load(reinterpret_cast<const f32x4*>(X + (r + 4 * u) * ldx + col));
+#pragma unroll
+            for (int u = 0; u < CC_U; ++u) {
+                bf16_t* y = Y + (r + 4 * u) * ldy + col;
+                store4(y, v[u]);
+                const bf16x4 q = {(bf16_t)v[u][0], (bf16_t)v[u][1], (bf16_t)v[u][2], (bf16_t)v[u][3]};
+                acc += f32x4{(float)q[0], (float)q[1], (float)q[2], (float)q[3]};
+            }
+        }
+        for (; r < M; r += 4) {
+            const f32x4 v = load4(X + r * ldx + col);
+            store4(Y + r * ldy + col, v);
+            const bf16x4 q = {(bf16_t)v[0], (bf16_t)v[1], (bf16_t)v[2], (bf16_t)v[3]};
+            acc += f32x4{(float)q[0], (float)q[1], (float)q[2], (float)q[3]};
+        }
+    }
+    store4(&part[rg][cg * 4], acc);
+    __syncthreads();
+    const int64_t c = (int64_t)blockIdx.x * 256 + threadIdx.x;
+    if (c < N) {
+        const float p = ((part[0][threadIdx.x] + part[1][threadIdx.x]) + part[2][threadIdx.x]) + part[3][threadIdx.x];
+        float tsum = 0.f;
+        tsum += p;
+        out[c] = (beta != 0.f ? beta * out[c] : 0.f) + tsum;
+    }
+}
+
+extern "C" int vaw_cast_colsum_plan(int64_t M, int64_t N, int64_t ld_src, int64_t ld_dst, int64_t src_addr, int64_t dst_addr,
+                                    int64_t colsum_addr, vaw_cast_colsum_launch* out) {
+    VAW_CHECK_ARG(out != nullptr, "cast_colsum_plan: out is NULL");
+    vaw_cast_colsum_launch p = {};
+    *out = p;
+    VAW_CHECK_ARG(M > 0 && N > 0 && ld_src >= N && ld_dst >= N, "cast_colsum: bad sizes M=%ld N=%ld ld_src=%ld ld_dst=%ld", (long)M, (long)N,
+                  (long)ld_src, (long)ld_dst);
+    VAW_CHECK_ARG(M <= 512, "cast_colsum: M=%ld > 512 rows is left to vaw_cast_bf16 + vaw_colsum", (long)M);
+    VAW_CHECK_ARG(N % 4 == 0 && ld_src % 4 == 0 && ld_dst % 4 == 0, "cast_colsum: N, ld_src and ld_dst must be multiples of 4");
+    VAW_CHECK_ARG((src_addr & 15) == 0 && (dst_addr & 15) == 0 && (colsum_addr & 3) == 0 && src_addr && dst_addr && colsum_addr,
+                  "cast_colsum: src and dst must be 16-byte aligned");
+    VAW_CHECK_ARG((N + 255) / 256 < (1LL << 31), "cast_colsum: N too large");
+    p.grid_x = (int)((N + 255) / 256);
+    p.block = 256;
+    p.rows_per_lane = (int)((M + 3) / 4);
+    p.bytes_read = M * N * 4;
+    p.bytes_written = M * N * 2 + N * 4;
+    *out = p;
+    return VAW_OK;
+}
+
+extern "C" int vaw_cast_colsum_bf16(const float* src, int64_t ld_src, void* dst, int64_t ld_dst, int64_t M, int64_t N, float* colsum,
+                                    float beta, vaw_stream stream) {
+    vaw_cast_colsum_launch p;
+    const int rc = vaw_cast_colsum_plan(M, N, ld_src, ld_dst, (int64_t)(uintptr_t)src, (int64_t)(uintptr_t)dst, (int64_t)(uintptr_t)colsum, &p);
+    if (rc != VAW_OK) return rc;
+    cast_colsum_kernel<<<p.grid_x, p.block, 0, (hipStream_t)stream>>>(src, ld_src, (bf16_t*)dst, ld_dst, M, N, colsum, beta);
+    VAW_CHECK_LAUNCH("cast_colsum_bf16");
+    return VAW_OK;
+}
diff --git a/variance-aware-weight_amd/csrc/gemm.hip b/variance-aware-weight_amd/csrc/gemm.hip
--- a/variance-aware-weight_amd/csrc/gemm.hip
+++ b/variance-aware-weight_amd/csrc/gemm.hip
@@ -519,10 +519,18 @@
                                      void* __restrict__ C, float alpha, float beta, int out_f32,
                                      const float* __restrict__ rowpart = nullptr, float* __restrict__ rowsum_out = nullptr,
                                      float rowsum_beta = 0.f) {
-    if (rowpart && blockIdx.x == gridDim.x - 1) {
-        for (int64_t m = threadIdx.x; m < M; m += blockDim.x) {
+    if (rowpart) {
+        for (int64_t m = blockIdx.x * (int64_t)blockDim.x + threadIdx.x; m < M; m += (int64_t)gridDim.x * blockDim.x) {
             float t = 0.f;
-            for (int sidx = 0; sidx < S; ++sidx) t += rowpart[(int64_t)sidx * M + m];
+            int sidx = 0;
+            for (; sidx + 8 <= S; sidx += 8) {
+                float v[8];
+#pragma unroll
+                for (int u = 0; u < 8; ++u) v[u] = rowpart[(int64_t)(sidx + u) * M + m];
+#pragma unroll
+                for (int u = 0; u < 8; ++u) t += v[u];
+            }
+            for (; sidx < S; ++sidx) t += rowpart[(int64_t)sidx * M + m];
             rowsum_out[m] = (rowsum_beta != 0.f ? rowsum_beta * rowsum_out[m] : 0.f) + t;
         }
     }
diff --git a/variance-aware-weight_amd/csrc/layernorm.hip b/variance-aware-weight_amd/csrc/layernorm.hip
--- a/variance-aware-weight_amd/csrc/layernorm.hip
+++ b/variance-aware-weight_amd/csrc/layernorm.hip
@@ -95,7 +95,8 @@
                const float* __restrict__ dres, const T* __restrict__ y, const float* __restrict__ gate,
                T* __restrict__ dy, float* __restrict__ dgate, float* __restrict__ dy_colpart,
                int rows_per_chunk, float* __restrict__ part,
-               unsigned char* __restrict__ q_out = nullptr, float* __restrict__ q_state = nullptr, int q_e5m2 = 0) {
+               unsigned char* __restrict__ q_out = nullptr, float* __restrict__ q_state = nullptr, int q_e5m2 = 0,
+               T* __restrict__ dx_act = nullptr) {
     static_assert(!(FUSE && GATE_ONLY), "FUSE extends the LayerNorm mode");
     constexpr int NQ = FUSE ? 4 : 2;
     extern __shared__ __attribute__((aligned(16))) float lds[];
@@ -170,6 +171,7 @@
                     f32x4 r = (g[i] - c1 - xh[i] * c2) * rs;
                     if (dres_in) r += load4(dres_in + row * D + c);
                     store4(dx + row * D + c, r);
+                    if (dx_act) store4(dx_act + row * D + c, r);
                     if (FUSE) {
                         const f32x4 yv = load4(y + row * D + c);
                         const f32x4 d = r * load4(gsc_lds + c);
@@ -525,12 +527,12 @@
     return VAW_OK;
 }
 
-extern "C" int vaw_ln_modulate_bwd(vaw_dtype dt, const void* dout, const float* x, const float* mean, const float* rstd,
-                                   const float* scale, int64_t mod_ld, const float* dres_in, float* dx, float* dshift,
-                                   float* dscale, int64_t dmod_ld, int B, int T, int D, float* workspace,
-                                   int64_t workspace_floats, vaw_stream stream) {
+static int ln_modulate_bwd_launch(const char* who, vaw_dtype dt, const void* dout, const float* x, const float* mean, const float* rstd,
+                                  const float* scale, int64_t mod_ld, const float* dres_in, float* dx, float* dshift, float* dscale,
+                                  int64_t dmod_ld, int B, int T, int D, float* workspace, int64_t workspace_floats, void* dx_act,
+                                  vaw_stream stream) {
     VAW_CHECK_ARG(B > 0 && T > 0 && D > 0 && D % 4 == 0 && D <= 2048 && mod_ld % 4 == 0,
-                  "ln_modulate_bwd: need D%%4==0, D<=2048, mod_ld%%4==0 (D=%d)", D);
+                  "%s: need D%%4==0, D<=2048, mod_ld%%4==0 (D=%d)", who, D);
     ROW_PLAN(VAW_ROW_LN_BWD, dt, B, T, D, 0, 0, workspace ? workspace_floats : 0);
     hipStream_t s = (hipStream_t)stream;
     const int nc = plan.nc, rpc = plan.rows_per_chunk, block = plan.block;
@@ -538,13 +540,29 @@
     const size_t lds = plan.lds_bytes;
     dim3 grid(B, nc);
     if (dt == VAW_F32) {
-        DISPATCH_NV(plan.nv, (row_bwd_kernel<float, NV, false><<<grid, block, lds, s>>>((const float*)dout, x, mean, rstd, scale, mod_ld, dres_in, dx, dshift, dscale, dmod_ld, T, D, nullptr, nullptr, nullptr, nullptr, nullptr, nullptr, rpc, part)));
+        DISPATCH_NV(plan.nv, (row_bwd_kernel<float, NV, false><<<grid, block, lds, s>>>((const float*)dout, x, mean, rstd, scale, mod_ld, dres_in, dx, dshift, dscale, dmod_ld, T, D, nullptr, nullptr, nullptr, nullptr, nullptr, nullptr, rpc, part, nullptr, nullptr, 0, (float*)dx_act)));
     } else {
-        DISPATCH_NV(plan.nv, (row_bwd_kernel<bf16_t, NV, false><<<grid, block, lds, s>>>((const bf16_t*)dout, x, mean, rstd, scale, mod_ld, dres_in, dx, dshift, dscale, dmod_ld, T, D, nullptr, nullptr, nullptr, nullptr, nullptr, nullptr, rpc, part)));
+        DISPATCH_NV(plan.nv, (row_bwd_kernel<bf16_t, NV, false><<<grid, block, lds, s>>>((const bf16_t*)dout, x, mean, rstd, scale, mod_ld, dres_in, dx, dshift, dscale, dmod_ld, T, D, nullptr, nullptr, nullptr, nullptr, nullptr, nullptr, rpc, part, nullptr, nullptr, 0, (bf16_t*)dx_act)));
     }
     if (nc > 1) row_bwd_finish_kernel<<<ceil_div((int64_t)B * D, 256), 256, 0, s>>>(part, nc, B, D, dshift, dmod_ld, dscale, dmod_ld);
-    VAW_CHECK_LAUNCH("ln_modulate_bwd");
-    return VAW_OK;
+    VAW_CHECK_LAUNCH(who);
+    return VAW_OK;
+}
+
+extern "C" int vaw_ln_modulate_bwd(vaw_dtype dt, const void* dout, const float* x, const float* mean, const float* rstd,
+                                   const float* scale, int64_t mod_ld, const float* dres_in, float* dx, float* dshift,
+                                   float* dscale, int64_t dmod_ld, int B, int T, int D, float* workspace,
+                                   int64_t workspace_floats, vaw_stream stream) {
+    return ln_modulate_bwd_launch("ln_modulate_bwd", dt, dout, x, mean, rstd, scale, mod_ld, dres_in, dx, dshift, dscale, dmod_ld, B, T, D,
+                                  workspace, workspace_floats, nullptr, stream);
+}
+
+extern "C" int vaw_ln_modulate_bwd_cast(vaw_dtype dt, const void* dout, const float* x, const float* mean, const float* rstd,
+                                        const float* scale, int64_t mod_ld, const float* dres_in, float* dx, float* dshift,
+                                        float* dscale, int64_t dmod_ld, int B, int T, int D, float* workspace,
+                                        int64_t workspace_floats, void* dx_act, vaw_stream stream) {
+    return ln_modulate_bwd_launch("ln_modulate_bwd_cast", dt, dout, x, mean, rstd, scale, mod_ld, dres_in, dx, dshift, dscale, dmod_ld, B, T,
+                                  D, workspace, workspace_floats, dx_act, stream);
 }
 
 extern "C" int vaw_ln_modulate_bwd_gate(vaw_dtype dt, const void* dout, const float* x, const float* mean, const float* rstd,
diff --git a/variance-aware-weight_amd/dit.py b/variance-aware-weight_amd/dit.py
--- a/variance-aware-weight_amd/dit.py
+++ b/variance-aware-weight_amd/dit.py
@@ -191,7 +191,7 @@
             raise L.VawError("DiT backward: activation_checkpointing was switched between this forward and its backward "
                              "(the workspace of the forward was laid out for the other mode)")
         dx = m._backward_impl(dout.contiguous(), ctx.need_dx)
-        return torch.zeros_like(m._anchor), None, dx, None, None
+        return (None if L.STEP_FUSED else torch.zeros_like(m._anchor)), None, dx, None, None
 
 
 class DiT(FlatModule):
@@ -510,14 +510,20 @@
 
     def _adaln_wgrad(self, dt, ws, r0, nrows, B, beta):
         D, ld = self.D, self.mod_cols
+        gw, gb = self._g("blocks.0.adaLN_modulation.1.weight") + 4 * r0 * D, self._g("blocks.0.adaLN_modulation.1.bias") + 4 * r0
+        fused = False
         if dt == BF16:
-            ops.cast_bf16(ws.dmod, ws.dmod_a)
             dmod_a, es = ptr(ws.dmod_a), 2
+            fused = L.STEP_FUSED and ops.cast_colsum_plan(B, nrows, ld, ld, ptr(ws.dmod) + 4 * r0, dmod_a + es * r0, gb) is not None
+            if fused:
+                ops.cast_colsum(ptr(ws.dmod) + 4 * r0, ld, dmod_a + es * r0, ld, B, nrows, gb, beta)
+            else:
+                ops.cast_bf16(ws.dmod, ws.dmod_a)
         else:
             dmod_a, es = ptr(ws.dmod), 4
-        ops.gemm(dt, 0, 0, nrows, D, ws.Bk, dmod_a + es * r0, ld, ptr(ws.cs), D, self._g("blocks.0.adaLN_modulation.1.weight") + 4 * r0 * D,
-                 D, beta=beta, out_f32=True)
-        ops.colsum(dt, dmod_a + es * r0, B, nrows, ld, self._g("blocks.0.adaLN_modulation.1.bias") + 4 * r0, beta)
+        ops.gemm(dt, 0, 0, nrows, D, ws.Bk, dmod_a + es * r0, ld, ptr(ws.cs), D, gw, D, beta=beta, out_f32=True)
+        if not fused:
+            ops.colsum(dt, dmod_a + es * r0, B, nrows, ld, gb, beta)
         return dmod_a
 
     def _backward_impl(self, dout, need_dx):
@@ -538,10 +544,11 @@
         own_dy = defer and not fp8
         ckpt = ws.ckpt
         fuse_rows = fp8 and ws.d_bwd and self.fp8_fuse_epilogue and self.fp8_fuse_rows and M % 64 == 0 and D % 128 == 0
-
-        def ln_bwd_and_gate(dout_p, x_p, mean_p, rstd_p, scale_p, dres_in, dsh, dsc, nxt):
+        fuse_tail = L.STEP_FUSED and dt == BF16
+
+        def ln_bwd_and_gate(dout_p, x_p, mean_p, rstd_p, scale_p, dres_in, dsh, dsc, nxt, dx_act=0):
             if nxt is None:
-                ops.ln_modulate_bwd(dt, dout_p, x_p, mean_p, rstd_p, scale_p, ld, dres_in, dres, dsh, dsc, ld, B, T, D)
+                ops.ln_modulate_bwd(dt, dout_p, x_p, mean_p, rstd_p, scale_p, ld, dres_in, dres, dsh, dsc, ld, B, T, D, dx_act=dx_act)
                 return
             l2, which = nxt
             nb = ws.blk[l2]
@@ -645,8 +652,9 @@
                 else:
                     self._wgrad(dt, pre + "attn.qkv.", dq, ptr(b["xm"]), 3 * D, D, M, beta)
             self._linear_dgrad(ws, b, "f_dqkv", dq, pre + "attn.qkv.", M, 3 * D, D, dD)
+            last_cast = fuse_tail and l == 0
             ln_bwd_and_gate(dD, xin, ptr(b["mean1"]), ptr(b["rstd1"]), mo + 4 * D, dres, dmo, dmo + 4 * D,
-                            (l - 1, "mlp") if (l and not ckpt) else None)
+                            (l - 1, "mlp") if (l and not ckpt) else None, dx_act=ptr(ws.dao) if last_cast else 0)
             if defer:
                 pending.append(l)
                 if ckpt or l == group_cut:
@@ -663,7 +671,9 @@
                     hook("ada_hi")
         pending.reverse()
         flush()
-        if dt == BF16:
+        if dt == BF16 and fuse_tail and Lyr:
+            dx0 = ptr(ws.dao)
+        elif dt == BF16:
             ops.cast_bf16(ws.dres, ws.dD)
             dx0 = dD
         else:
@@ -677,23 +687,19 @@
         rows = ld if ada_half is None else 6 * ada_half * D
         dmod_a = self._adaln_wgrad(dt, ws, 0, rows, B, beta)
         ops.gemm(dt, 1, 0, B, D, ld, dmod_a, ld, self._w("blocks.0.adaLN_modulation.1.weight"), D, ptr(ws.dcs), D, out_f32=True)
-        L.check(lib.vaw_silu_bwd(ptr(ws.c), ptr(ws.dcs), ptr(ws.dc), B * D, st), "silu_bwd")
+        ops.silu_bwd(ws.c, ws.dcs, ws.dc, ws.dc_a[:B] if fuse_tail else None)
         ye = self.y_embedder.embedding_table
         L.check(lib.vaw_embedding_bwd(ptr(ws.dc), ptr(ws.y), self._g("y_embedder.embedding_table.weight"), B, D,
                                       ye.num_embeddings, beta, st), "embedding_bwd")
-        if dt == BF16:
+        if dt == BF16 and not fuse_tail:
             ops.cast_bf16(ws.dc, ws.dc_a)
-            dc_a = ptr(ws.dc_a)
-        else:
-            dc_a = ptr(ws.dc)
+        dc_a = ptr(ws.dc_a) if dt == BF16 else ptr(ws.dc)
         self._wgrad(dt, "t_embedder.mlp.2.", dc_a, ptr(ws.h1s), D, D, ws.Bk, beta)
         ops.gemm(dt, 1, 0, B, D, D, dc_a, D, self._w("t_embedder.mlp.2.weight"), D, ptr(ws.dh1s), D, out_f32=True)
-        L.check(lib.vaw_silu_bwd(ptr(ws.h1), ptr(ws.dh1s), ptr(ws.dh1), B * D, st), "silu_bwd")
-        if dt == BF16:
+        ops.silu_bwd(ws.h1, ws.dh1s, ws.dh1, ws.dh1_a[:B] if fuse_tail else None)
+        if dt == BF16 and not fuse_tail:
             ops.cast_bf16(ws.dh1, ws.dh1_a)
-            dh1_a = ptr(ws.dh1_a)
-        else:
-            dh1_a = ptr(ws.dh1)
+        dh1_a = ptr(ws.dh1_a) if dt == BF16 else ptr(ws.dh1)
         self._wgrad(dt, "t_embedder.mlp.0.", dh1_a, ptr(ws.tfreq), D, 256, ws.Bk, beta)
         self.attach_grads()
         if fp8:
diff --git a/variance-aware-weight_amd/gaussian_diffusion.py b/variance-aware-weight_amd/gaussian_diffusion.py
--- a/variance-aware-weight_amd/gaussian_diffusion.py
+++ b/variance-aware-weight_amd/gaussian_diffusion.py
@@ -482,23 +482,47 @@
             return noise
         return ops.mix_rows(x_start.contiguous(), noise.contiguous(), tb["ca"][t], tb["cb"][t])
 
-    def training_losses(self, model, x_start, features=None, t=None, model_kwargs=None, noise=None):
+    def _check_objective(self):
+        kl_loss = self.loss_type in (LossType.KL, LossType.RESCALED_KL)
+        if not kl_loss and self.loss_type not in (LossType.MSE, LossType.RESCALED_MSE):
+            raise NotImplementedError(self.loss_type)
+        if getattr(self.args, "learn_align", False):
+            raise NotImplementedError("learn_align: feature-alignment teachers are out of scope (SURVEY.md §2.1 row 12)")
+        return kl_loss
+
+    def training_losses(self, model, x_start, features=None, t=None, model_kwargs=None, noise=None, accum=None):
         if model_kwargs is None:
             model_kwargs = {}
         if noise is None:
             noise = torch.randn_like(x_start)
         if t is None:
             t = self.sample_t(x_start)
-        kl_loss = self.loss_type in (LossType.KL, LossType.RESCALED_KL)
-        if not kl_loss and self.loss_type not in (LossType.MSE, LossType.RESCALED_MSE):
-            raise NotImplementedError(self.loss_type)
-        if getattr(self.args, "learn_align", False):
-            raise NotImplementedError("learn_align: feature-alignment teachers are out of scope (SURVEY.md §2.1 row 12)")
+        kl_loss = self._check_objective()
         x_start = x_start.contiguous()
         noise = noise.contiguous()
         tb = self._tables(x_start.device)
         x_t = ops.qsample(x_start, noise, t, tb["a"], tb["s"])
-        raw_output = model(x_t, self._scale_timesteps(t), **model_kwargs)
+        return self._losses_after_qsample(model, x_start, x_t, self._scale_timesteps(t), noise, t, model_kwargs, kl_loss, accum)
+
+    def training_losses_fused(self, model, latent, latent_scale, eps, t=None, model_kwargs=None, noise=None, accum=1):
+        if model_kwargs is None:
+            model_kwargs = {}
+        if noise is None:
+            noise = torch.randn_like(eps)
+        if t is None:
+            t = self.sample_t(eps)
+        kl_loss = self._check_objective()
+        tb = self._tables(latent.device)
+        own_scale = type(self)._scale_timesteps is GaussianDiffusion._scale_timesteps and bool(self.rescale_timesteps)
+        t_scale = 1000.0 / self.num_timesteps if own_scale else None
+        out = ops.latent_qsample(latent.contiguous(), eps.contiguous(), noise.contiguous(), t.contiguous(), tb["a"], tb["s"],
+                                 latent_scale, t_scale)
+        t_model = out[2] if own_scale else self._scale_timesteps(t)
+        return self._losses_after_qsample(model, out[0], out[1], t_model, noise.contiguous(), t, model_kwargs, kl_loss, accum)
+
+    def _losses_after_qsample(self, model, x_start, x_t, t_model, noise, t, model_kwargs, kl_loss, accum):
+        tb = self._tables(x_start.device)
+        raw_output = model(x_t, t_model, **model_kwargs)
         model_output = raw_output[0] if isinstance(raw_output, tuple) else raw_output
         learned = self.model_var_type in (ModelVarType.LEARNED, ModelVarType.LEARNED_RANGE)
         var_values = None
@@ -514,6 +538,9 @@
             scale = self.num_timesteps / 1000.0 if self.loss_type == LossType.RESCALED_MSE else 1.0
             terms["vb"] = self._vb_terms_bpd(model_output.detach(), var_values, x_start, x_t, t, scale)
         assert model_output.shape == x_start.shape
+        if accum is not None and not learned:
+            mse, mean = ops.weighted_mse_mean(model_output, x_start, noise, t.contiguous(), tb["ca"], tb["cb"], tb["w"], accum)
+            return {"mse": mse, "loss": mse, "loss_mean": mean, "mse_mean": mean.detach()}
         terms["mse"] = ops.weighted_mse(model_output, x_start, noise, tb["ca"][t], tb["cb"][t], tb["w"][t])
         terms["loss"] = terms["mse"] + terms["vb"] if "vb" in terms else terms["mse"]
         return terms
@@ -584,7 +611,7 @@
         ca, cb = self._target_coefs(alpha_t, sigma_t, d_alpha_t, d_sigma_t)
         return ops.mix_rows(x_start.contiguous(), noise.contiguous(), ca.float().contiguous(), cb.float().contiguous())
 
-    def training_losses(self, model, x_start, features=None, t=None, model_kwargs=None, noise=None):
+    def training_losses(self, model, x_start, features=None, t=None, model_kwargs=None, noise=None, accum=None):
         if model_kwargs is None:
             model_kwargs = {}
         if noise is None:
@@ -602,6 +629,10 @@
         raw_output = model(x_t, t, **model_kwargs)
         model_output = raw_output[0] if isinstance(raw_output, tuple) else raw_output
         assert model_output.shape == x_start.shape
+        if accum is not None:
+            mse, mean = ops.weighted_mse_mean(model_output, x_start, noise, None, ca.float().contiguous(), cb.float().contiguous(),
+                                              w.float().contiguous(), accum)
+            return {"mse": mse, "loss": mse, "loss_mean": mean, "mse_mean": mean.detach()}
         terms = {"mse": ops.weighted_mse(model_output, x_start, noise, ca.float().contiguous(), cb.float().contiguous(),
                                          w.float().contiguous())}
         terms["loss"] = terms["mse"]
diff --git a/variance-aware-weight_amd/ops.py b/variance-aware-weight_amd/ops.py
--- a/variance-aware-weight_amd/ops.py
+++ b/variance-aware-weight_amd/ops.py
@@ -68,6 +68,71 @@
 
 def weighted_mse(model_out, x0, noise, ca, cb, w):
     return _WeightedMSE.apply(model_out, x0, noise, ca, cb, w)
+
+
+def latent_qsample(latent, eps, noise, t, tab_a, tab_s, latent_scale, t_scale=None):
+    need_cuda(latent, eps, noise, t, tab_a, tab_s)
+    _f32c(latent, eps, noise, tab_a, tab_s)
+    B = latent.shape[0]
+    assert latent.shape[1] % 2 == 0 and eps.shape == noise.shape == (B, latent.shape[1] // 2, *latent.shape[2:])
+    assert t.dtype == torch.int64 and t.shape == (B,) and t.is_contiguous()
+    x0, x_t = torch.empty_like(eps), torch.empty_like(eps)
+    tf = torch.empty(B, device=eps.device, dtype=torch.float32) if t_scale is not None else None
+    check(L.lib().vaw_latent_qsample(ptr(latent), ptr(eps), ptr(noise), ptr(t), ptr(tab_a), ptr(tab_s), tab_a.numel(),
+                                     float(latent_scale), float(t_scale or 0.0), ptr(x0), ptr(x_t), ptr(tf), B, eps.numel() // B,
+                                     stream_ptr()), "vaw_latent_qsample")
+    return (x0, x_t, tf) if t_scale is not None else (x0, x_t)
+
+
+class _WeightedMSEMean(torch.autograd.Function):
+
+    @staticmethod
+    def forward(ctx, model_out, x0, noise, t, ca, cb, w, accum):
+        need_cuda(model_out, x0, noise, t, ca, cb, w)
+        model_out = model_out.contiguous()
+        _f32c(model_out, x0, noise, ca, cb, w)
+        B = x0.shape[0]
+        assert model_out.shape == x0.shape == noise.shape
+        if t is None:
+            assert ca.shape == cb.shape == w.shape == (B,)
+        else:
+            assert t.dtype == torch.int64 and t.shape == (B,) and t.is_contiguous() and ca.shape == cb.shape == w.shape
+        mse = torch.empty(B, device=x0.device, dtype=torch.float32)
+        mean = torch.empty((), device=x0.device, dtype=torch.float32)
+        check(L.lib().vaw_wmse_fwd_t(ptr(model_out), ptr(x0), ptr(noise), ptr(t), ptr(ca), ptr(cb), ptr(w), ca.numel(), ptr(mse),
+                                     ptr(mean), float(accum), B, x0.numel() // B, stream_ptr()), "vaw_wmse_fwd_t")
+        ctx.save_for_backward(model_out, x0, noise, t, ca, cb, w)
+        ctx.inv_count = float((torch.tensor(1.0) / float(accum)) / float(B))
+        ctx.mark_non_differentiable(mse)
+        ctx.set_materialize_grads(False)
+        return mse, mean
+
+    @staticmethod
+    def backward(ctx, _gmse, gmean):
+        if gmean is None:
+            return (None,) * 8
+        model_out, x0, noise, t, ca, cb, w = ctx.saved_tensors
+        need_cuda(gmean)
+        gmean = gmean.contiguous().float()
+        dout = torch.empty_like(model_out)
+        B = x0.shape[0]
+        check(L.lib().vaw_wmse_bwd_t(ptr(model_out), ptr(x0), ptr(noise), ptr(t), ptr(ca), ptr(cb), ptr(w), ca.numel(), ptr(gmean),
+                                     ctx.inv_count, ptr(dout), B, x0.numel() // B, stream_ptr()), "vaw_wmse_bwd_t")
+        return dout, None, None, None, None, None, None, None
+
+
+def weighted_mse_mean(model_out, x0, noise, t, ca, cb, w, accum=1):
+    return _WeightedMSEMean.apply(model_out, x0, noise, t, ca, cb, w, accum)
+
+
+_ones = {}
+
+
+def one_like(x):
+    t = _ones.get(x.device)
+    if t is None:
+        t = _ones[x.device] = torch.ones((), device=x.device, dtype=torch.float32)
+    return t
 
 
 class _VbTerms(torch.autograd.Function):
@@ -691,8 +756,12 @@
     return scratch_f32(torch.device("cuda", torch.cuda.current_device()), L.lib().vaw_row_bwd_workspace_floats(B, T, D))
 
 
-def ln_modulate_bwd(dt, dout, x, mean, rstd, scale, mod_ld, dres_in, dx, dshift, dscale, dmod_ld, B, T, D):
+def ln_modulate_bwd(dt, dout, x, mean, rstd, scale, mod_ld, dres_in, dx, dshift, dscale, dmod_ld, B, T, D, dx_act=0):
     ws = _row_ws(B, T, D)
+    if dx_act:
+        check(L.lib().vaw_ln_modulate_bwd_cast(dt, dout, x, mean, rstd, scale, mod_ld, dres_in or None, dx, dshift, dscale,
+                                               dmod_ld, B, T, D, ws.data_ptr(), ws.numel(), dx_act, stream_ptr()), "vaw_ln_modulate_bwd_cast")
+        return
     check(L.lib().vaw_ln_modulate_bwd(dt, dout, x, mean, rstd, scale, mod_ld, dres_in or None, dx, dshift, dscale,
                                       dmod_ld, B, T, D, ws.data_ptr(), ws.numel(), stream_ptr()), "vaw_ln_modulate_bwd")
 
@@ -837,6 +906,20 @@
     check(L.lib().vaw_cast_bf16(ptr(src), ptr(dst), src.numel(), stream_ptr()), "vaw_cast_bf16")
 
 
+def cast_colsum_plan(M, N, ld_src, ld_dst, src_addr, dst_addr, colsum_addr):
+    p = L.CastColsumLaunch()
+    rc = L.lib().vaw_cast_colsum_plan(M, N, ld_src, ld_dst, src_addr, dst_addr, colsum_addr, C.byref(p))
+    return p if rc == 0 else None
+
+
+def cast_colsum(src, ld_src, dst, ld_dst, M, N, colsum_out, beta=0.0):
+    check(L.lib().vaw_cast_colsum_bf16(src, ld_src, dst, ld_dst, M, N, colsum_out, beta, stream_ptr()), "vaw_cast_colsum_bf16")
+
+
+def silu_bwd(x, dy, dx, dx_bf16=None):
+    check(L.lib().vaw_silu_bwd_cast(ptr(x), ptr(dy), ptr(dx), ptr(dx_bf16), dx.numel(), stream_ptr()), "vaw_silu_bwd_cast")
+
+
 def uncast_bf16(src, dst, scale=1.0):
     check(L.lib().vaw_uncast_bf16(ptr(src), ptr(dst), src.numel(), float(scale), stream_ptr()), "vaw_uncast_bf16")
 
diff --git a/variance-aware-weight_amd/respace.py b/variance-aware-weight_amd/respace.py
--- a/variance-aware-weight_amd/respace.py
+++ b/variance-aware-weight_amd/respace.py
@@ -51,6 +51,9 @@
     def training_losses(self, model, *args, **kwargs):
         return super().training_losses(self._respaced(model), *args, **kwargs)
 
+    def training_losses_fused(self, model, *args, **kwargs):
+        return super().training_losses_fused(self._respaced(model), *args, **kwargs)
+
     def calc_bpd_loop(self, model, *args, **kwargs):
         return super().calc_bpd_loop(self._respaced(model), *args, **kwargs)
 
diff --git a/variance-aware-weight_amd/trainer.py b/variance-aware-weight_amd/trainer.py
--- a/variance-aware-weight_amd/trainer.py
+++ b/variance-aware-weight_amd/trainer.py
@@ -3,7 +3,7 @@
 import torch
 import torch.nn as nn
 
-from . import dist_util, ops
+from . import _lib, dist_util, ops
 from .flat import FlatModule
 from .optim import FusedAdamW
 
@@ -67,6 +67,13 @@
             optimizer.attach_ema(ema_model, args.ema_decay)
         self.last_mse = None
         self._cpu_rng = bool(getattr(args, "cpu_rng", False))
+        self._step_fused = _lib.STEP_FUSED and torch.device(device).type == "cuda"
+        from .gaussian_diffusion import FlowMatching, GaussianDiffusion
+        from .respace import SpacedDiffusion
+        own = getattr(type(diffusion), "training_losses", None) in (GaussianDiffusion.training_losses, SpacedDiffusion.training_losses,
+                                                                   FlowMatching.training_losses)
+        self._fused_means = self._step_fused and own
+        self._fused_latent = self._fused_means and hasattr(diffusion, "training_losses_fused")
         self.schedule_sampler, self._device_sampler = None, False
         name = getattr(args, "schedule_sampler", None)
         if name and name != "uniform":
@@ -101,12 +108,13 @@
         return (images.to(self.device, non_blocking=True),
                 labels.to(self.device, non_blocking=True) if self.args.class_cond else None)
 
-    def _compute_loss(self, images, labels, features):
+    def _compute_loss(self, images, labels, features, accum=None):
         model_kwargs = {"y": labels} if self.args.class_cond else {}
+        extra = {"accum": accum} if accum is not None and self._fused_means else {}
         if self._cpu_rng and not self._device_sampler:
             noise = torch.randn(images.shape).to(images.device)
             t = torch.randint(0, self.diffusion.num_timesteps, (images.shape[0],)).to(images.device)
-            return self.diffusion.training_losses(self.model, images, features, t=t, model_kwargs=model_kwargs, noise=noise)
+            return self.diffusion.training_losses(self.model, images, features, t=t, model_kwargs=model_kwargs, noise=noise, **extra)
         if self.schedule_sampler is not None:
             noise = torch.randn(images.shape).to(images.device) if self._cpu_rng else None
             t, w = self.schedule_sampler.sample(images.shape[0], images.device)
@@ -115,7 +123,39 @@
             terms = dict(terms)
             terms["loss"] = terms["loss"] * w
             return terms
-        return self.diffusion.training_losses(self.model, images, features, model_kwargs=model_kwargs)
+        return self.diffusion.training_losses(self.model, images, features, model_kwargs=model_kwargs, **extra)
+
+    def _micro_step(self, images, labels, accum, cpu_rng, divide):
+        a = self.args
+        fused = self._step_fused and images.is_cuda
+        if fused and a.in_chans == 4 and self.schedule_sampler is None and self._fused_latent:
+            mean, _ = torch.chunk(images, 2, dim=1)
+            model_kwargs = {"y": labels} if a.class_cond else {}
+            if cpu_rng:
+                eps = torch.randn(mean.shape).to(mean.device)
+                model_kwargs = dict(model_kwargs=model_kwargs, noise=torch.randn(mean.shape).to(mean.device),
+                                    t=torch.randint(0, self.diffusion.num_timesteps, (mean.shape[0],)).to(mean.device))
+            else:
+                eps = torch.randn_like(mean)
+                model_kwargs = dict(model_kwargs=model_kwargs)
+            loss_dict = self.diffusion.training_losses_fused(self.model, images, a.latent_scale, eps, accum=accum, **model_kwargs)
+        else:
+            if a.in_chans == 4:
+                images = sample_from_latent(images, a.latent_scale, cpu_rng)
+            loss_dict = self._compute_loss(images, labels, None, accum if fused else None)
+        if "loss_mean" in loss_dict:
+            loss = loss_dict["loss_mean"]
+            torch.autograd.backward(loss, ops.one_like(loss))
+            return loss.detach(), loss_dict["mse_mean"]
+        loss = loss_dict["loss"].mean()
+        if divide:
+            loss = loss / accum
+        loss.backward()
+        ld = loss.detach()
+        if "mse" not in loss_dict:
+            return ld, torch.zeros_like(ld)
+        md = loss_dict["mse"].detach().mean()
+        return ld, (md / accum if divide else md)
 
     def _apply_gradient_clipping(self):
         if self.args.grad_clip:
@@ -139,16 +179,11 @@
             ema(self.model, self.ema_model, self.args.ema_decay)
 
     def _graph_body(self, images, labels):
-        a = self.args
-        if a.in_chans == 4:
-            images = sample_from_latent(images, a.latent_scale, False)
-        loss_dict = self._compute_loss(images, labels, None)
-        loss = loss_dict["loss"].mean()
-        loss.backward()
+        loss, mse = self._micro_step(images, labels, 1, False, False)
         self._apply_gradient_clipping()
         self.optimizer.step()
         self.optimizer.zero_grad()
-        return loss.detach(), (loss_dict["mse"].detach().mean() if "mse" in loss_dict else torch.zeros_like(loss.detach()))
+        return loss, mse
 
     def eager_from_now_on(self):
         if self._use_graph:
@@ -217,18 +252,12 @@
         total, mse_avg = None, None
         for i in range(accum):
             images, labels = self._get_next_batch()
-            if a.in_chans == 4:
-                images = sample_from_latent(images, a.latent_scale, self._cpu_rng)
             if a.parallel and accum > 1 and i < accum - 1:
                 ctx = self.model.no_sync()
             else:
                 ctx = nullcontext()
             with ctx:
-                loss_dict = self._compute_loss(images, labels, None)
-                loss = loss_dict["loss"].mean() / accum
-                loss.backward()
-            ld = loss.detach()
-            md = loss_dict["mse"].detach().mean() / accum if "mse" in loss_dict else torch.zeros_like(ld)
+                ld, md = self._micro_step(images, labels, accum, self._cpu_rng, True)
             total = ld if total is None else total + ld
             mse_avg = md if mse_avg is None else mse_avg + md
             if (i + 1) % accum == 0:
```

Measured after the change: 20670 images/sec (median of 6 runs). 1.2% higher.
